# Tcadart/pyLatticeDSO

Measured on AMD Instinct MI355X. Metric: beams/s assembly+PCG-solve, higher is better.
Workload: dtype f64

## Files before the change

include/pylattice_hip.h:

```cpp
#ifndef PYLATTICE_HIP_H
#define PYLATTICE_HIP_H

#include <stdint.h>

#ifdef __cplusplus
extern "C" {
#endif

typedef struct pl_context *pl_handle;

typedef enum {
  PL_OK = 0,
  PL_ERR_ARG = -1,
  PL_ERR_HIP = -2,
  PL_ERR_STATE = -3,
  PL_ERR_NOCONV = -4,
  PL_ERR_NAN = -5,
  PL_ERR_NODEVICE = -6
} pl_status;

typedef struct {
  int64_t n_nodes;
  int64_t n_beams;
  const double *node_xyz;
// ... 60 lines not shown
  double cg_form_used;
  double kp_form;
  double comm_world;
  double comm_rank;
  double short_iteration_used;
  double reserved[2];
} pl_stats_t;

int pl_default_opts(pl_opts_t *o, uint32_t struct_size);
uint32_t pl_opts_size(void);
uint32_t pl_stats_size(void);
uint32_t pl_abi_version(void);
const char *pl_last_error(void);
const char *pl_version(void);

int pl_lzone(int device, int64_t n_nodes, int64_t n_beams, const double *node_xyz, const int32_t *beam_conn,
             const double *beam_radius, double *lzone);

int pl_create(const pl_mesh_t *mesh, const pl_opts_t *opts, pl_handle *out);
void pl_destroy(pl_handle h);

int pl_create_ddm(int64_t n_nodes, int64_t n_cells, int32_t nb, const int32_t *cell_nodes, int32_t n_S, const double *S,
                  const int32_t *cell_S, const pl_opts_t *opts, pl_handle *out);

#define PL_DDM_DENSE_MAX 16384
int pl_ddm_set_preconditioner(pl_handle h, int32_t n_S, const double *S ,
                              const int32_t *cell_S );

int pl_ddm_update_matrices(pl_handle h, int32_t n_S, const double *S , const int32_t *cell_S );

int pl_ddm_set_geometry(pl_handle h, const double *node_xyz );

int pl_set_bc(pl_handle h, const uint8_t *fixed, const double *ubar, const double *f);

int pl_set_periodic(pl_handle h, const int32_t *master );

int pl_update_radii(pl_handle h, const double *beam_radius);
int pl_set_multiplicity(pl_handle h, const double *beam_mult );
int pl_update_segments(pl_handle h, const double *seg_len, const int32_t *seg_nsub);

int pl_assemble(pl_handle h);

int pl_assemble_bsr(pl_handle h, int with_bc, int64_t *n_block_rows, int64_t *n_blocks);
int pl_get_bsr(pl_handle h, int64_t *rowptr , int32_t *colidx , double *vals );

int pl_spmv(pl_handle h, const double *x, double *y);
int pl_spmv_free(pl_handle h, const double *x, double *y);
int pl_spmv_bsr(pl_handle h, const double *x, double *y);

int pl_solve(pl_handle h, double rtol, int32_t max_iter, double *u, pl_stats_t *stats);

int pl_reactions(pl_handle h, const double *u, double *R);

int pl_sens(pl_handle h, const double *u, const double *lam, double *dCdr);

#define PL_SENS_GRAM_MAX 8
int pl_sens_gram(pl_handle h, int32_t n_rhs, const double *x, double *gram);

int pl_node_mod(pl_handle h, const double *u, double *out);

int pl_stress(pl_handle h, const double *u , int32_t where,
              double *station ,
              double *peak );
int pl_stress_pnorm(pl_handle h, const double *u , int32_t where, double p, double *phi, double *sigma_max,
                    double *dphi_du , double *dphi_dr );

int pl_buckling(pl_handle h, const double *u , int32_t length, double k_eff, int32_t shear,
                double *util , double *n_axial , double *n_crit );
int pl_buckling_pnorm(pl_handle h, const double *u , int32_t length, double k_eff, int32_t shear, double p,
                      double *bp, double *util_max, double *dbp_du , double *dbp_dr );

int pl_energy(pl_handle h, const double *u, double *energy);

int pl_schur(pl_handle h, const int32_t *boundary_nodes, int32_t nb, double rtol, int32_t max_iter, double *S);

#define PL_MULTI_MAX 64
int pl_spmv_multi(pl_handle h, int32_t n_rhs, int masked, const double *x, double *y);
int pl_solve_multi(pl_handle h, int32_t n_rhs, const double *ubar, const double *f, double rtol, int32_t max_iter,
                   double *u, pl_stats_t *stats);
int pl_schur_block(pl_handle h, const int32_t *boundary_nodes, int32_t nb, double rtol, int32_t max_iter,
                   int32_t block, double *S);

int pl_geom_spmv_multi(pl_handle h, const double *u, int32_t n_rhs, int masked, const double *x, double *y);
int pl_buckling_modes(pl_handle h, const double *u , int32_t n_modes, int32_t n_sub,
                      double rtol, int32_t max_iter,
                      double tol, int32_t max_outer,
                      double *load_factor , double *modes ,
                      double *residual ,
                      int32_t *n_found, int32_t *outer_iterations);
int pl_buckling_modes_sens(pl_handle h, const double *u , int32_t n_modes,
                           const double *load_factor , const double *modes ,
                           double rtol, int32_t max_iter,
                           const double *weights ,
                           double *dlam_dr  ,
                           double *dsum_dr  ,
                           double *adj_load );

int pl_set_mass(pl_handle h, double density, int32_t rotary, const double *node_mass );
int pl_mass_spmv_multi(pl_handle h, int32_t n_rhs, int masked, const double *x, double *y);
int pl_vibration_modes(pl_handle h, int32_t n_modes, int32_t n_sub, double rtol, int32_t max_iter, double tol,
                       int32_t max_outer, double *omega2 , double *modes ,
                       double *residual ,
                       int32_t *n_found, int32_t *outer_iterations);
int pl_vibration_modes_sens(pl_handle h, int32_t n_modes, const double *omega2 ,
                            const double *modes , const double *weights ,
                            double *domega2_dr ,
                            double *dsum_dr );

int pl_dyn_spmv_multi(pl_handle h, double c_K, double c_M, int32_t n_rhs, int masked, const double *x, double *y);
int pl_transient(pl_handle h, int32_t n_steps, double dt, double beta, double gamma, double ray_m, double ray_k,
                 int32_t n_pat, const double *pattern , const double *amp ,
                 const double *u0, const double *v0 , double rtol, int32_t max_iter,
                 int32_t n_probe, const int32_t *probe_nodes, double *probe ,
                 double *energy ,
                 int32_t snap_every, double *snaps ,
                 double *state , int32_t *iters );

#define PL_TRANSIENT_SENS_CHUNK 32
int pl_transient_sens(pl_handle h, int32_t n_steps, double dt, double beta, double gamma, double ray_m, double ray_k,
                      int32_t n_pat, const double *pattern , const double *amp ,
                      const double *base_dir , const double *base_acc ,
                      const double *u0, const double *v0 , double rtol, int32_t max_iter,
                      const double *out_vec , int32_t kind, double p, const double *weight ,
                      double *J, double *y , double *dJ_dr ,
                      int32_t *iters );

int pl_schur_cells(const pl_opts_t *o, int32_t n_inst, int32_t n_nodes, int32_t n_beams,
                   const int32_t *beam_conn , int32_t nb,
                   const int32_t *boundary_nodes ,
                   const double *node_xyz , const double *beam_radius ,
                   const double *seg_len , const int32_t *seg_nsub ,
                   double *S , int32_t *info );

int pl_cells_recover(const pl_opts_t *o, int32_t n_inst, int32_t n_nodes, int32_t n_beams,
                     const int32_t *beam_conn , int32_t nb,
                     const int32_t *boundary_nodes ,
                     const double *node_xyz , const double *beam_radius ,
                     const double *seg_len , const int32_t *seg_nsub ,
                     const double *u_b ,
                     const double *lam_b ,
                     double *u_full ,
                     double *lam_full ,
                     double *sens ,
                     int32_t *info );

int pl_get_records(pl_handle h, double *rec);

int pl_debug_partition(pl_handle h, int32_t *tile_of_node, int32_t *agg_of_node, int32_t *local_agg_of_node,
                       uint8_t *eliminated);

int pl_time_kernel(pl_handle h, int which, int reps, double *avg_ms);
int pl_algorithmic_bytes(pl_handle h, double *out3);
int pl_node_words_info(pl_handle h, int *classes_on, int *n_classes, int *bytes_on, int *byte_exp);
int pl_forget_history(pl_handle h);

int pl_debug_spd_solve(int device, int32_t n, const double *A, const double *b, double *x, double *quad,
                       int32_t fp32_factor);

int pl_dist_unique_id_bytes(void);
int pl_dist_unique_id(void *id_out);
int pl_dist_loopback_id(void *id_out);
int pl_dist_abort(pl_handle h);
int pl_dist_init(pl_handle h, int rank, int world, const void *unique_id, const int32_t *shared_local,
                 const int32_t *shared_global, int32_t n_shared, int32_t n_shared_global);

typedef struct pl_lattice pl_lattice;
typedef struct {
  int64_t n_nodes, n_beams, n_cell_beam, n_cell_node, n_created;
} pl_lattice_info_t;
int pl_generate_lattice(int64_t n_cells, const double *cell_coord, const double *cell_size, const double *cell_radii,
                        int32_t n_geom, int32_t n_tmpl, const double *tmpl, const int32_t *tmpl_type,
                        pl_lattice **out, pl_lattice_info_t *info);
int pl_lattice_fetch(const pl_lattice *L, double *node_xyz, int32_t *beam_conn, double *beam_radius, int32_t *beam_type,
                     int32_t *beam_cell0, int64_t *cell_beam_ptr , int64_t *cell_beam_idx,
                     int64_t *cell_node_ptr , int64_t *cell_node_idx, int32_t *created_nodes,
                     int32_t *created_beam);
void pl_lattice_free(pl_lattice *L);

int pl_penalize(int64_t n_beams, const double *node_xyz, const int32_t *beam_conn, const double *lzone ,
                double mesh_size, double *seg_len , int32_t *seg_nsub , double *pen_xyz );

int pl_boundary_index(int64_t n_cells, const int64_t *cell_node_ptr, const int64_t *cell_node_idx, int64_t n_nodes,
                      const double *node_xyz, const double *cell_coord, const double *cell_size, int64_t *index_boundary,
                      int64_t *visit, int64_t *n_visit);

int pl_boundary_index_rows(int64_t n_cells, const int64_t *cell_node_ptr, const int64_t *cell_node_idx, int64_t n_nodes,
                           const double *node_xyz, const double *cell_coord, const double *cell_size,
                           int64_t *index_boundary, int64_t *visit, int64_t *n_visit);

int pl_dist_set_peers(pl_handle h, const int32_t *shared_peer );

#ifdef __cplusplus
}
#endif
#endif
```

pylatticedso_amd/_capi.py:

```python
from __future__ import annotations

import ctypes as C
import os

import numpy as np

from .timing import timing as _timing

_HERE = os.path.dirname(os.path.abspath(__file__))
LIB_PATH = os.environ.get("PYLATTICE_HIP_LIB") or os.path.join(_HERE, "libpylattice_hip.so")

PL_OK, PL_ERR_ARG, PL_ERR_HIP, PL_ERR_STATE, PL_ERR_NOCONV, PL_ERR_NAN, PL_ERR_NODEVICE = 0, -1, -2, -3, -4, -5, -6

EXPORTS = ["pl_default_opts", "pl_opts_size", "pl_stats_size", "pl_abi_version", "pl_last_error", "pl_version", "pl_lzone", "pl_create", "pl_create_ddm",
           "pl_ddm_set_preconditioner", "pl_ddm_set_geometry", "pl_ddm_update_matrices", "pl_destroy", "pl_set_bc", "pl_set_periodic",
           "pl_update_radii", "pl_set_multiplicity", "pl_update_segments", "pl_assemble", "pl_assemble_bsr", "pl_get_bsr", "pl_spmv",
           "pl_spmv_free", "pl_spmv_bsr", "pl_solve", "pl_reactions", "pl_sens", "pl_sens_gram", "pl_energy", "pl_node_mod", "pl_schur",
           "pl_stress", "pl_stress_pnorm", "pl_buckling", "pl_buckling_pnorm",
           "pl_spmv_multi", "pl_solve_multi", "pl_schur_block", "pl_geom_spmv_multi", "pl_buckling_modes", "pl_buckling_modes_sens",
           "pl_set_mass", "pl_mass_spmv_multi", "pl_vibration_modes", "pl_vibration_modes_sens",
           "pl_dyn_spmv_multi", "pl_transient", "pl_transient_sens",
           "pl_schur_cells", "pl_cells_recover", "pl_get_records", "pl_debug_partition", "pl_time_kernel", "pl_algorithmic_bytes", "pl_node_words_info", "pl_forget_history", "pl_debug_spd_solve", "pl_dist_unique_id_bytes",
           "pl_dist_unique_id", "pl_dist_loopback_id", "pl_dist_abort", "pl_dist_init", "pl_dist_set_peers", "pl_generate_lattice", "pl_lattice_fetch",
           "pl_lattice_free", "pl_penalize", "pl_boundary_index", "pl_boundary_index_rows"]


class PlMesh(C.Structure):
    _fields_ = [("n_nodes", C.c_int64), ("n_beams", C.c_int64), ("node_xyz", C.c_void_p),
                ("beam_conn", C.c_void_p), ("beam_radius", C.c_void_p), ("seg_len", C.c_void_p),
                ("seg_nsub", C.c_void_p)]


class PlOpts(C.Structure):
    _fields_ = [("struct_size", C.c_uint32), ("abi_version", C.c_uint32),
                ("young", C.c_double), ("poisson", C.c_double), ("kappa", C.c_double), ("pen_coef", C.c_double),
                ("device", C.c_int32), ("spmv_kernel", C.c_int32), ("precond", C.c_int32), ("reorder", C.c_int32),
                ("check_every", C.c_int32), ("lanes_per_node", C.c_int32),
                ("tile_nodes", C.c_int32), ("coarse_max_dofs", C.c_int32), ("palette", C.c_int32),
                ("local_max_dofs", C.c_int32), ("precision", C.c_int32), ("restart_every", C.c_int32),
                ("alpha_max", C.c_double), ("grid_lo", C.c_double * 3), ("grid_hi", C.c_double * 3),
                ("grid_nodes", C.c_int64), ("mintol", C.c_double), ("compact_records", C.c_int32),
                ("condense", C.c_int32), ("chol_persistent", C.c_int32), ("cg_form", C.c_int32),
                ("tile_modes", C.c_int32), ("coarse_modes", C.c_int32), ("overlap", C.c_int32),
                ("coarse_storage", C.c_int32), ("warm_start", C.c_int32), ("short_iteration", C.c_int32)]


class PlStats(C.Structure):
    _fields_ = [("struct_size", C.c_uint32), ("iterations", C.c_int32), ("converged", C.c_int32),
                ("reserved_i", C.c_int32), ("rel_residual", C.c_double),
                ("b_norm", C.c_double), ("ms_assembly", C.c_double), ("ms_solve", C.c_double),
                ("ms_spmv_avg", C.c_double), ("precond_used", C.c_double), ("restarts", C.c_double),
                ("precision_used", C.c_double), ("info", C.c_double), ("stop_reason", C.c_double),
                ("condensed_nodes", C.c_double), ("cg_form_used", C.c_double), ("kp_form", C.c_double),
                ("comm_world", C.c_double), ("comm_rank", C.c_double), ("short_iteration_used", C.c_double),
                ("reserved", C.c_double * 2)]


class PlError(RuntimeError):
    def __init__(self, code, msg):
        super().__init__(f"libpylattice_hip error {code}: {msg}")
        self.code = code


_lib = None


def load_library(path: str | None = None):
    global _lib
    if _lib is not None and path is None:
        return _lib
    p = path or LIB_PATH
    if not os.path.exists(p):
        raise FileNotFoundError(f"{p} not found - build it with `make -C pylatticedso_amd/csrc` "
                                "(the HIP path has no CPU fallback)")
    lib = C.CDLL(p)
    lib.pl_last_error.restype = C.c_char_p
    lib.pl_version.restype = C.c_char_p
    lib.pl_destroy.restype = None
    for name in ("pl_opts_size", "pl_stats_size", "pl_abi_version"):
        getattr(lib, name).restype = C.c_uint32
    lib.pl_lattice_free.restype = None
    V, I32, I64, D = C.c_void_p, C.c_int32, C.c_int64, C.c_double
    sig = {"pl_default_opts": [V, C.c_uint32], "pl_opts_size": [], "pl_stats_size": [], "pl_abi_version": [], "pl_lzone": [I32, I64, I64, V, V, V, V], "pl_create": [V, V, V], "pl_create_ddm": [I64, I64, I32, V, I32, V, V, V, V],
           "pl_ddm_set_preconditioner": [V, I32, V, V], "pl_ddm_set_geometry": [V, V], "pl_ddm_update_matrices": [V, I32, V, V], "pl_destroy": [V], "pl_set_bc": [V, V, V, V], "pl_set_periodic": [V, V],
           "pl_update_radii": [V, V], "pl_set_multiplicity": [V, V], "pl_update_segments": [V, V, V], "pl_assemble": [V],
           "pl_assemble_bsr": [V, I32, V, V], "pl_get_bsr": [V, V, V, V], "pl_spmv": [V, V, V],
           "pl_spmv_free": [V, V, V], "pl_spmv_bsr": [V, V, V], "pl_solve": [V, D, I32, V, V],
           "pl_reactions": [V, V, V], "pl_sens": [V, V, V, V], "pl_sens_gram": [V, I32, V, V], "pl_energy": [V, V, V], "pl_node_mod": [V, V, V],
           "pl_stress": [V, V, I32, V, V], "pl_stress_pnorm": [V, V, I32, D, V, V, V, V],
           "pl_buckling": [V, V, I32, D, I32, V, V, V], "pl_buckling_pnorm": [V, V, I32, D, I32, D, V, V, V, V],
           "pl_schur": [V, V, I32, D, I32, V], "pl_spmv_multi": [V, I32, I32, V, V],
           "pl_solve_multi": [V, I32, V, V, D, I32, V, V], "pl_schur_block": [V, V, I32, D, I32, I32, V],
           "pl_geom_spmv_multi": [V, V, I32, I32, V, V],
           "pl_buckling_modes": [V, V, I32, I32, D, I32, D, I32, V, V, V, V, V],
           "pl_buckling_modes_sens": [V, V, I32, V, V, D, I32, V, V, V, V],
           "pl_set_mass": [V, D, I32, V], "pl_mass_spmv_multi": [V, I32, I32, V, V],
           "pl_vibration_modes": [V, I32, I32, D, I32, D, I32, V, V, V, V, V],
           "pl_vibration_modes_sens": [V, I32, V, V, V, V, V],
           "pl_dyn_spmv_multi": [V, D, D, I32, I32, V, V],
           "pl_transient": [V, I32, D, D, D, D, D, I32, V, V, V, V, D, I32, I32, V, V, V, I32, V, V, V],
           "pl_transient_sens": [V, I32, D, D, D, D, D, I32, V, V, V, V, V, V, D, I32, V, I32, D, V, V, V, V, V],
           "pl_schur_cells": [V, I32, I32, I32, V, I32, V, V, V, V, V, V, V],
           "pl_cells_recover": [V, I32, I32, I32, V, I32, V, V, V, V, V, V, V, V, V, V, V],
           "pl_get_records": [V, V], "pl_debug_partition": [V, V, V, V, V], "pl_time_kernel": [V, I32, I32, V],
           "pl_algorithmic_bytes": [V, V], "pl_node_words_info": [V, V, V, V, V], "pl_forget_history": [V], "pl_debug_spd_solve": [I32, I32, V, V, V, V, I32], "pl_dist_unique_id_bytes": [], "pl_dist_unique_id": [V], "pl_dist_loopback_id": [V], "pl_dist_abort": [V],
           "pl_dist_init": [V, I32, I32, V, V, V, I32, I32], "pl_dist_set_peers": [V, V],
           "pl_generate_lattice": [I64, V, V, V, I32, I32, V, V, V, V], "pl_lattice_fetch": [V] * 12,
           "pl_lattice_free": [V], "pl_penalize": [I64, V, V, V, D, V, V, V],
           "pl_boundary_index": [I64, V, V, I64, V, V, V, V, V, V],
           "pl_boundary_index_rows": [I64, V, V, I64, V, V, V, V, V, V]}
    for name, args in sig.items():
        getattr(lib, name).argtypes = args
    if lib.pl_opts_size() != C.sizeof(PlOpts) or lib.pl_stats_size() != C.sizeof(PlStats):
        raise ImportError(f"{p}: pl_opts_t / pl_stats_t are {lib.pl_opts_size()} / {lib.pl_stats_size()} bytes in the "
                          f"library, {C.sizeof(PlOpts)} / {C.sizeof(PlStats)} in this binding (ABI version "
                          f"{lib.pl_abi_version()}): rebuild libpylattice_hip.so")
    _lib = lib
    return lib


def default_opts(lib=None) -> "PlOpts":
    lib = lib or load_library()
    opts = PlOpts()
    _check(lib, lib.pl_default_opts(C.byref(opts), C.sizeof(PlOpts)))
    return opts


def _ptr(a):
    return None if a is None else a.ctypes.data_as(C.c_void_p)


def _f64(a, n=None):
    a = np.ascontiguousarray(a, dtype=np.float64)
    if n is not None and a.size != n:
        raise ValueError(f"expected {n} values, got {a.size}")
    return a


def _check(lib, rc, allow=()):
    if rc != PL_OK and rc not in allow:
        raise PlError(rc, lib.pl_last_error().decode())
    return rc


def lzone(node_xyz, beam_conn, beam_radius, device=0):
    lib = load_library()
    xyz = _f64(np.asarray(node_xyz).reshape(-1))
    conn = np.ascontiguousarray(beam_conn, dtype=np.int32).reshape(-1)
    rad = _f64(np.asarray(beam_radius).reshape(-1), len(conn) // 2)
    out = np.empty(len(conn), np.float64)
    _check(lib, lib.pl_lzone(int(device), len(xyz) // 3, len(conn) // 2, _ptr(xyz), _ptr(conn), _ptr(rad), _ptr(out)))
    return out.reshape(-1, 2)


def debug_spd_solve(A, b, device=0, fp32_factor=False):
    lib = load_library()
    A = np.ascontiguousarray(A, np.float64)
    b = np.ascontiguousarray(b, np.float64)
    x = np.empty_like(b)
    q = C.c_double()
    _check(lib, lib.pl_debug_spd_solve(device, len(b), _ptr(A), _ptr(b), _ptr(x), C.byref(q), int(bool(fp32_factor))))
    return x, q.value


MULTI_MAX = 64
SENS_GRAM_MAX = 8
TRANSIENT_SENS_CHUNK = 32

SCHUR_CELLS_MAX_BOUNDARY, SCHUR_CELLS_MAX_INTERIOR, SCHUR_CELLS_MAX_BEAMS = 32, 16, 512


def schur_cells_fits(n_nodes, n_beams, n_boundary):
    return (0 < n_boundary <= SCHUR_CELLS_MAX_BOUNDARY and n_nodes - n_boundary <= SCHUR_CELLS_MAX_INTERIOR
            and 0 < n_beams <= SCHUR_CELLS_MAX_BEAMS)


def _per_instance(name, a, tail, n_inst):
    if a.shape == tail:
        a = np.broadcast_to(a, (n_inst,) + tail)
    elif a.shape != (n_inst,) + tail:
        raise ValueError(f"{name} must have shape {tail} or {(n_inst,) + tail}, got {a.shape}")
    return np.ascontiguousarray(a)


def schur_cells(node_xyz, beam_conn, boundary_nodes, beam_radius, seg_len, seg_nsub, young, poisson, kappa=0.9,
                pen_coef=1.5, device=0, n_inst=None):
    xyz, conn, bn, rad, slen, nsub, n_inst = _cell_batch_arrays(node_xyz, beam_conn, boundary_nodes, beam_radius, seg_len,
                                                                seg_nsub, n_inst)
    B, N = len(conn), xyz.shape[1]
    lib = load_library()
    opts = default_opts(lib)
    opts.young, opts.poisson, opts.kappa, opts.pen_coef, opts.device = young, poisson, kappa, pen_coef, device
    m = 6 * len(bn)
    S = np.empty((n_inst, m, m), np.float64)
    info = np.empty(n_inst, np.int32)
    _check(lib, lib.pl_schur_cells(C.byref(opts), n_inst, N, B, _ptr(conn), len(bn), _ptr(bn), _ptr(xyz), _ptr(rad),
                                   _ptr(slen), _ptr(nsub), _ptr(S), _ptr(info)))
    return S, info


def _cell_batch_arrays(node_xyz, beam_conn, boundary_nodes, beam_radius, seg_len, seg_nsub, n_inst, extra_lead=()):
    conn = np.asarray(beam_conn)
    bn = np.asarray(boundary_nodes)
    if conn.ndim != 2 or conn.shape[1] != 2 or not np.issubdtype(conn.dtype, np.integer):
        raise ValueError("beam_conn must be an integer (B, 2) array")
    if bn.ndim != 1 or not np.issubdtype(bn.dtype, np.integer):
        raise ValueError("boundary_nodes must be a 1-D integer array")
    xyz, rad = np.asarray(node_xyz, dtype=np.float64), np.asarray(beam_radius, dtype=np.float64)
    slen, nsub = np.asarray(seg_len, dtype=np.float64), np.asarray(seg_nsub)
    if not np.issubdtype(nsub.dtype, np.integer):
        raise ValueError("seg_nsub must be an integer array")
    if xyz.ndim not in (2, 3) or xyz.shape[-1] != 3:
        raise ValueError("node_xyz must be (N, 3) or (n_inst, N, 3)")
    B, N = len(conn), xyz.shape[-2]
    lead = [a.shape[0] for a, nd in ((xyz, 3), (rad, 2), (slen, 3), (nsub, 3)) if a.ndim == nd] + list(extra_lead)
    if n_inst is None:
        n_inst = max(lead) if lead else 1
    n_inst = int(n_inst)
    if n_inst < 1:
        raise ValueError("n_inst must be >= 1")
    xyz = _per_instance("node_xyz", xyz, (N, 3), n_inst)
    rad = _per_instance("beam_radius", rad, (B,), n_inst)
    slen = _per_instance("seg_len", slen, (B, 3), n_inst)
    nsub = _per_instance("seg_nsub", nsub.astype(np.int32, copy=False), (B, 3), n_inst)
    conn = np.ascontiguousarray(conn, dtype=np.int32)
    bn = np.ascontiguousarray(bn, dtype=np.int32)
    return xyz, conn, bn, rad, slen, nsub, n_inst


def cells_recover(node_xyz, beam_conn, boundary_nodes, beam_radius, seg_len, seg_nsub, u_b, young, poisson, lam_b=None,
                  want=("u", "lam", "sens"), kappa=0.9, pen_coef=1.5, device=0):
    want = (want,) if isinstance(want, str) else tuple(want)
    if not want or any(w not in ("u", "lam", "sens") for w in want):
        raise ValueError('want must be a non-empty subset of ("u", "lam", "sens")')
    bn = np.asarray(boundary_nodes)
    m = 6 * (len(bn) if bn.ndim == 1 else 0)

    def boundary_values(name, v):
        v = np.asarray(v, dtype=np.float64)
        if v.ndim >= 2 and v.shape[-2:] == (m // 6, 6):
            v = v.reshape(v.shape[:-2] + (m,))
        if v.ndim not in (1, 2) or v.shape[-1] != m:
            raise ValueError(f"{name} must have {m} values per instance, got shape {v.shape}")
        return v

    ub = boundary_values("u_b", u_b)
    lb = None if lam_b is None else boundary_values("lam_b", lam_b)
    lead = [v.shape[0] for v in (ub, lb) if v is not None and v.ndim == 2]
    xyz, conn, bn, rad, slen, nsub, n_inst = _cell_batch_arrays(node_xyz, beam_conn, boundary_nodes, beam_radius, seg_len,
                                                                seg_nsub, None, lead)
    ub = _per_instance("u_b", ub, (m,), n_inst)
    lb = None if lb is None else _per_instance("lam_b", lb, (m,), n_inst)
    B, N = len(conn), xyz.shape[1]
    lib = load_library()
    opts = default_opts(lib)
    opts.young, opts.poisson, opts.kappa, opts.pen_coef, opts.device = young, poisson, kappa, pen_coef, device
    out = {"info": np.empty(n_inst, np.int32)}
    if "u" in want:
# ... 526 lines not shown
            out["dsum_dr"] = dsum
        return out

    def _mass_model(self):
        if getattr(self, "_mass", None) is None:
            raise ValueError("call set_mass first")
        return self._mass

    def mass_spmv_multi_host(self, X, masked=False, fixed=None):
        from . import mass_host as MH
        if masked and fixed is None:
            raise ValueError("the masked product needs the mask given to set_bc")
        rho, rotary, nm = self._mass_model()
        x = self._columns("X", X).reshape(-1, self.n_nodes, 6)
        return MH.mass_apply(self.node_xyz, self.beam_conn, self._radius, rho, x, self._mult, rotary, nm,
                             fixed if masked else None)

    def mass_matrix_host(self):
        from . import mass_host as MH
        rho, rotary, nm = self._mass_model()
        return MH.mass_matrix(self.node_xyz, self.beam_conn, self._radius, rho, self._mult, rotary, nm)

    def vibration_modes_host(self, fixed, n_modes=4, n_sub=0, tol=1e-9, max_outer=200, dense=False):
        from . import geometric_host as GH
        from . import mass_host as MH
        K = GH.elastic_matrix(self.records(), self.beam_conn, self.n_nodes)
        M = self.mass_matrix_host()
        if dense:
            return MH.vibration_modes_dense(K, M, fixed, n_modes)
        return MH.vibration_modes_subspace(K, M, fixed, n_modes, n_sub, tol, max_outer)

    def vibration_modes_sens_host(self, omega2, modes, fixed):
        from . import mass_host as MH
        from . import stress_host as SH
        rho, rotary, nm = self._mass_model()
        E, nu, kappa, pen = self._material
        drec = SH.drecords_dr(self.node_xyz, self.beam_conn, self._radius, self._seg_len, self._seg_nsub, E, nu, kappa, pen,
                              self._mult)
        return MH.vibration_sensitivity(self.node_xyz, self.beam_conn, self._radius, rho, drec, fixed, omega2, modes,
                                        self._mult, rotary, nm)

    def dyn_spmv_multi(self, c_K, c_M, X, masked=False):
        x = self._columns("X", X)
        y = np.empty_like(x)
        _check(self._lib, self._lib.pl_dyn_spmv_multi(self._h, float(c_K), float(c_M), x.shape[0], int(bool(masked)), _ptr(x),
                                                      _ptr(y)))
        return y.reshape(x.shape[0], self.n_nodes, 6)

    def transient(self, dt, n_steps, patterns=None, amp=None, u0=None, v0=None, beta=0.25, gamma=0.5, ray_m=0.0, ray_k=0.0,
                  rtol=1e-10, max_iter=100000, probes=None, snap_every=0, want_state=True):
        n_steps, n6 = int(n_steps), 6 * self.n_nodes
        rows = max(n_steps, 0) + 1
        pat = am = None
        n_pat = 0
        if patterns is not None:
            pat = np.ascontiguousarray(np.asarray(patterns, dtype=np.float64)).reshape(-1, n6)
            n_pat = pat.shape[0]
            am = np.ascontiguousarray(np.asarray(amp, dtype=np.float64).reshape(-1))
            if am.size != rows * n_pat:
                raise ValueError(f"amp must have shape ({rows}, {n_pat})")
        uu = self._opt_vec6(u0)
        vv = self._opt_vec6(v0)
        pr = np.zeros(0, np.int32) if probes is None else np.ascontiguousarray(np.asarray(probes).reshape(-1), dtype=np.int32)
        probe = np.zeros((rows, 3, pr.size, 6), np.float64)
        energy = np.zeros((rows, 3), np.float64)
        iters = np.zeros(rows, np.int32)
        snap_every = int(snap_every)
        snaps = np.zeros((n_steps // snap_every, self.n_nodes, 6), np.float64) if snap_every > 0 and n_steps > 0 else None
        state = np.zeros((3, self.n_nodes, 6), np.float64) if want_state else None
        _check(self._lib, self._lib.pl_transient(self._h, n_steps, float(dt), float(beta), float(gamma), float(ray_m),
                                                 float(ray_k), n_pat, _ptr(pat), _ptr(am), _ptr(uu), _ptr(vv), float(rtol),
                                                 int(max_iter), pr.size, _ptr(pr) if pr.size else None,
                                                 _ptr(probe) if pr.size else None, _ptr(energy), snap_every, _ptr(snaps),
                                                 _ptr(state), _ptr(iters)))
        out = {"time": float(dt) * np.arange(rows), "probe": probe, "energy": energy, "iters": iters}
        if want_state:
            out["state"] = state
        if snaps is not None:
            out["snaps"] = snaps
        return out

    def transient_host(self, fixed, dt, n_steps, patterns=None, amp=None, u0=None, v0=None, beta=0.25, gamma=0.5, ray_m=0.0,
                       ray_k=0.0, solve=None, probes=None, snap_every=0):
        import scipy.sparse as sp
        from . import dynamics_host as DH
        self.assemble_bsr(False)
        rowptr, col, vals = self.get_bsr()
        K = sp.bsr_matrix((vals, col, rowptr), shape=(6 * self.n_nodes, 6 * self.n_nodes)).tocsr()
        K.sum_duplicates()
        return DH.newmark(K, self.mass_matrix_host(), fixed, dt, n_steps, patterns, amp, u0, v0, beta, gamma, ray_m, ray_k,
                          solve, probes, snap_every)

    def transient_sens(self, dt, n_steps, out_vec, kind=2, p=8.0, weight=None, patterns=None, amp=None, base_dir=None,
                       base_acc=None, u0=None, v0=None, beta=0.25, gamma=0.5, ray_m=0.0, ray_k=0.0, rtol=1e-10,
                       max_iter=100000):
        n_steps, n6 = int(n_steps), 6 * self.n_nodes
        rows = max(n_steps, 0) + 1
        pat = am = None
        n_pat = 0
        if patterns is not None:
            pat = np.ascontiguousarray(np.asarray(patterns, dtype=np.float64)).reshape(-1, n6)
            n_pat = pat.shape[0]
            am = np.ascontiguousarray(np.asarray(amp, dtype=np.float64).reshape(-1))
            if am.size != rows * n_pat:
                raise ValueError(f"amp must have shape ({rows}, {n_pat})")
        bd = None if base_dir is None else _f64(np.asarray(base_dir).reshape(-1), 3)
        ba = None if base_acc is None else _f64(np.asarray(base_acc).reshape(-1), rows)
        uu = self._opt_vec6(u0)
        vv = self._opt_vec6(v0)
        lv = _f64(np.asarray(out_vec).reshape(-1), n6)
        wt = None if weight is None else _f64(np.asarray(weight).reshape(-1), rows)
        J = C.c_double()
        y = np.zeros(rows, np.float64)
        grad = np.zeros(self.n_beams, np.float64)
        iters = np.zeros((2, rows), np.int32)
        _check(self._lib, self._lib.pl_transient_sens(self._h, n_steps, float(dt), float(beta), float(gamma), float(ray_m),
                                                      float(ray_k), n_pat, _ptr(pat), _ptr(am), _ptr(bd), _ptr(ba), _ptr(uu),
                                                      _ptr(vv), float(rtol), int(max_iter), _ptr(lv), int(kind), float(p),
                                                      _ptr(wt), C.byref(J), _ptr(y), _ptr(grad), _ptr(iters)))
        return {"J": J.value, "y": y, "dJ_dr": grad, "iters": iters}

    def transient_sens_host(self, fixed, dt, n_steps, out_vec, kind=2, p=8.0, weight=None, patterns=None, amp=None,
                            base_dir=None, base_acc=None, u0=None, v0=None, beta=0.25, gamma=0.5, ray_m=0.0, ray_k=0.0,
                            solve=None):
        import scipy.sparse as sp
        from . import dynamics_host as DH
        from . import mass_host as MH
        from . import stress_host as SH
        self.assemble_bsr(False)
        rowptr, col, vals = self.get_bsr()
        K = sp.bsr_matrix((vals, col, rowptr), shape=(6 * self.n_nodes, 6 * self.n_nodes)).tocsr()
        K.sum_duplicates()
        rho, rotary, nm = self._mass_model()
        E, nu, kappa, pen = self._material
        drec = SH.drecords_dr(self.node_xyz, self.beam_conn, self._radius, self._seg_len, self._seg_nsub, E, nu, kappa, pen,
                              self._mult)
        conn = np.asarray(self.beam_conn).reshape(-1, 2)
        xyz = np.asarray(self.node_xyz, dtype=np.float64).reshape(-1, 3)
        dM = MH.delement_matrix_dr(xyz[conn[:, 1]] - xyz[conn[:, 0]], np.asarray(self._radius, dtype=np.float64).reshape(-1),
                                   rho, self._mult, rotary)
        return DH.newmark_sensitivity(K, self.mass_matrix_host(), fixed, conn, drec, dM, dt, n_steps, out_vec, kind, p, weight,
                                      patterns, amp, base_dir, base_acc, u0, v0, beta, gamma, ray_m, ray_k, solve)

    def time_kernel(self, which, reps=20):
        ms = C.c_double()
        _check(self._lib, self._lib.pl_time_kernel(self._h, int(which), int(reps), C.byref(ms)))
        return ms.value

    def node_words_info(self):
        v = [C.c_int() for _ in range(4)]
        _check(self._lib, self._lib.pl_node_words_info(self._h, *[C.byref(x) for x in v]))
        return {"classes": bool(v[0].value), "n_classes": v[1].value, "bytes": bool(v[2].value), "byte_exp": v[3].value}

    def algorithmic_bytes(self):
        out = (C.c_double * 3)()
        _check(self._lib, self._lib.pl_algorithmic_bytes(self._h, out))
        return {"spmv": out[0], "pcg_iter": out[1], "bsr": out[2]}

    def set_periodic(self, master):
        m = None if master is None else np.ascontiguousarray(master, dtype=np.int32)
        if m is not None and m.size != self.n_nodes:
            raise ValueError(f"expected {self.n_nodes} entries, got {m.size}")
        _check(self._lib, self._lib.pl_set_periodic(self._h, _ptr(m)))

    def forget_history(self):
        _check(self._lib, self._lib.pl_forget_history(self._h))

    @staticmethod
    def dist_unique_id() -> bytes:
        lib = load_library()
        n = lib.pl_dist_unique_id_bytes()
        buf = C.create_string_buffer(n)
        _check(lib, lib.pl_dist_unique_id(buf))
        return buf.raw

    @staticmethod
    def dist_loopback_id() -> bytes:
        lib = load_library()
        buf = C.create_string_buffer(lib.pl_dist_unique_id_bytes())
        _check(lib, lib.pl_dist_loopback_id(buf))
        return buf.raw

    def dist_abort(self):
        if getattr(self, "_h", None) is not None and self._h.value:
            self._lib.pl_dist_abort(self._h)

    def dist_init(self, rank, world, unique_id: bytes, shared_local, shared_global, n_shared_global, shared_peer=None):
        sl = np.ascontiguousarray(shared_local, dtype=np.int32)
        sg = np.ascontiguousarray(shared_global, dtype=np.int32)
        buf = C.create_string_buffer(unique_id, len(unique_id))
        _check(self._lib, self._lib.pl_dist_init(self._h, int(rank), int(world), buf, _ptr(sl), _ptr(sg),
                                                 int(len(sl)), int(n_shared_global)))
        if shared_peer is not None:
            sp = np.ascontiguousarray(shared_peer, dtype=np.int32)
            if sp.shape != sl.shape:
                raise ValueError("one peer rank per shared entry expected")
            _check(self._lib, self._lib.pl_dist_set_peers(self._h, _ptr(sp)))


for _name in ("assemble", "assemble_bsr", "get_bsr", "solve", "set_bc", "spmv", "spmv_free", "spmv_bsr", "reactions",
              "sens", "stress", "stress_pnorm", "buckling", "buckling_pnorm", "energy", "schur", "spmv_multi", "solve_multi", "geom_spmv_multi", "buckling_modes", "buckling_modes_sens", "mass_spmv_multi", "vibration_modes", "vibration_modes_sens", "dyn_spmv_multi", "transient", "update_radii", "update_segments", "records"):
    _f = getattr(HipLattice, _name, None)
    if _f is not None:
        _f._timing_category = "hip"
        setattr(HipLattice, _name, _timing.timeit(_f))
```

pylatticedso_amd/csrc/pl_api.hip:

```cpp
#include <functional>

#include "pl_solver.h"
#include "pl_condense.h"
#include "pl_multi.h"
#include "pl_stress.h"
#include "pl_buckling.h"
#include "pl_geom.h"
#include "pl_mass.h"
#include "pl_dyn.h"
#include "pl_dyn_sens.h"
#include "pl_sensgram.h"


namespace {
template <typename WT>
int debug_spd_solve_t(int device, int32_t n, const double *A, const double *b, double *x, double *quad) {
  if (n <= 0 || !A || !b || !x) return fail(PL_ERR_ARG, "pl_debug_spd_solve: bad argument");
  int ndev = 0;
  if (hipGetDeviceCount(&ndev) != hipSuccess || ndev <= 0) return fail(PL_ERR_NODEVICE, "no HIP device visible");
  PL_HIP(hipSetDevice(device));
  const int np = (n + pl::kNB - 1) / pl::kNB * pl::kNB;
  std::vector<double> Ap((size_t)np * np, 0.0), bp(np, 0.0);
  for (int i = 0; i < np; ++i) {
    if (i < n) {
// ... 24 lines not shown
  PL_HIP(hipMemset(dinfo.p, 0, 2 * sizeof(int)));
  pl::dense_factor_inverse(dA.p, dL.p, dW.p, dWt.p, dD.p, np, np, dinfo.p, 0, nullptr);
  pl::dense_apply(dW.p, dWt.p, np, np, db.p, dt.p, dy.p, dq.p, nullptr, nullptr);
  PL_HIP(hipGetLastError());
  PL_HIP(hipDeviceSynchronize());
  int info[2];
  PL_HIP(hipMemcpy(info, dinfo.p, sizeof(info), hipMemcpyDeviceToHost));
  if (info[0] != 0) return fail(PL_ERR_ARG, "pl_debug_spd_solve: matrix is not positive definite");
  std::vector<double> y(np), q(pl::kSlots);
  PL_HIP(hipMemcpy(y.data(), dy.p, np * sizeof(double), hipMemcpyDeviceToHost));
  PL_HIP(hipMemcpy(q.data(), dq.p, pl::kSlots * sizeof(double), hipMemcpyDeviceToHost));
  std::memcpy(x, y.data(), n * sizeof(double));
  if (quad) {
    *quad = 0.0;
    for (double v : q) *quad += v;
  }
  return PL_OK;
}

}

extern "C" {

const char *pl_last_error(void) { return g_err.c_str(); }
#ifndef PL_KP_HASH
#define PL_KP_HASH "unknown"
#endif
const char *pl_version(void) { return "pylattice_hip 0.2 (gfx950) kp=" PL_KP_HASH; }

uint32_t pl_opts_size(void) { return (uint32_t)sizeof(pl_opts_t); }
uint32_t pl_stats_size(void) { return (uint32_t)sizeof(pl_stats_t); }
uint32_t pl_abi_version(void) { return PL_ABI_VERSION; }

int pl_default_opts(pl_opts_t *o, uint32_t struct_size) {
  if (!o) return fail(PL_ERR_ARG, "pl_default_opts: null argument");
  if (struct_size != sizeof(pl_opts_t))
    return fail(PL_ERR_ARG, "pl_default_opts: the caller's pl_opts_t has " + std::to_string(struct_size) +
                                " bytes, this library's " + std::to_string(sizeof(pl_opts_t)) +
                                " (ABI version " + std::to_string(PL_ABI_VERSION) + "): rebuild the binding against include/pylattice_hip.h");
  std::memset(o, 0, sizeof(*o));
  o->struct_size = (uint32_t)sizeof(pl_opts_t);
  o->abi_version = PL_ABI_VERSION;
  o->young = 1013.0;
  o->poisson = 0.3;
  o->kappa = 0.9;
  o->pen_coef = 1.5;
  o->device = 0;
  o->spmv_kernel = 0;
  o->precond = 1;
  o->reorder = 1;
  o->check_every = 0;
  return PL_OK;
}

namespace {
int check_opts_abi(const pl_opts_t *o, const char *who) {
  if (o->struct_size != sizeof(pl_opts_t) || o->abi_version != PL_ABI_VERSION)
    return fail(PL_ERR_ARG, std::string(who) + ": pl_opts_t was not initialised by pl_default_opts of this library (struct_size " +
                                std::to_string(o->struct_size) + " / abi " + std::to_string(o->abi_version) + ", expected " +
                                std::to_string(sizeof(pl_opts_t)) + " / " + std::to_string(PL_ABI_VERSION) + ")");
  return PL_OK;
}
inline bool multi_rank_handle(const pl_opts_t *o) { return o->grid_nodes > 0; }
inline int coarse_modes_of(const pl_opts_t *o, int64_t N = -1) {
  const bool tile12 = o->precond == 3 && o->tile_modes != 6;
  if (!tile12 || o->coarse_modes == 6) return 6;
  if (multi_rank_handle(o)) N = o->grid_nodes;
  return (o->coarse_modes == 12 || N < 0 || N >= 250000) ? 12 : 6;
}
inline int coarse_budget(const pl_opts_t *o, int64_t N) {
  const bool multi_rank = o->grid_nodes > 0;
  if (o->coarse_max_dofs > 0) return o->coarse_max_dofs;
  if (multi_rank) return (coarse_modes_of(o, N) == 12 && o->grid_nodes >= 2000000) ? 6144 : 3072;
  if (coarse_modes_of(o, N) == 12) return N >= 2000000 ? 6144 : (N >= 1000000 ? 3072 : (N >= 250000 ? 1536 : 768));
  return N >= 1000000 ? 3072 : 2100;
}
}

int pl_create(const pl_mesh_t *m, const pl_opts_t *o, pl_handle *out) {
  if (!m || !o || !out) return fail(PL_ERR_ARG, "pl_create: null argument");
  if (int rc_abi = check_opts_abi(o, "pl_create")) return rc_abi;
  StageTimer stage("pl_create");
  if (m->n_nodes <= 0 || m->n_beams <= 0) return fail(PL_ERR_ARG, "pl_create: empty mesh");
  if (m->n_nodes >= (1LL << 31) - 64 || m->n_beams >= (1LL << 31) - 64)
    return fail(PL_ERR_ARG, "pl_create: more than 2^31 nodes/struts per handle");
  if (!m->node_xyz || !m->beam_conn || !m->beam_radius || !m->seg_len || !m->seg_nsub)
    return fail(PL_ERR_ARG, "pl_create: null mesh array");
  int ndev = 0;
  if (hipGetDeviceCount(&ndev) != hipSuccess || ndev <= 0)
    return fail(PL_ERR_NODEVICE, "pl_create: no HIP device visible (libpylattice_hip has no CPU fallback)");
  if (o->device < 0 || o->device >= ndev) return fail(PL_ERR_ARG, "pl_create: bad device ordinal");
  if (o->precond == 5 && 6 * m->n_nodes > PL_DDM_DENSE_MAX)
    return fail(PL_ERR_ARG, "pl_create: precond = 5 (dense factorisation) serves at most PL_DDM_DENSE_MAX dofs");
  const int64_t N = m->n_nodes, B = m->n_beams;
  {
    std::atomic<int64_t> bad_ends{-1}, bad_radius{-1}, bad_len{-1}, bad_seg{-1};
    pl::parallel_for(B, [&](int64_t b0, int64_t b1, unsigned) {
      for (int64_t b = b0; b < b1; ++b) {
        const int32_t a = m->beam_conn[2 * b], d = m->beam_conn[2 * b + 1];
        if (a < 0 || d < 0 || a >= N || d >= N || a == d) bad_ends = b;
        if (!(m->beam_radius[b] > 0.0)) bad_radius = b;
        const double L = m->seg_len[3 * b] + m->seg_len[3 * b + 1] + m->seg_len[3 * b + 2];
        if (!(L > 0.0)) bad_len = b;
        for (int k = 0; k < 3; ++k)
          if (m->seg_len[3 * b + k] < 0.0 || (m->seg_len[3 * b + k] > 0.0 && m->seg_nsub[3 * b + k] < 1)) bad_seg = b;
      }
    });
    if (bad_ends >= 0)
      return fail(PL_ERR_ARG, "pl_create: strut " + std::to_string(bad_ends.load()) + " has invalid end nodes");
    if (bad_radius >= 0) return fail(PL_ERR_ARG, "pl_create: non-positive radius");
    if (bad_len >= 0) return fail(PL_ERR_ARG, "pl_create: strut with zero length");
    if (bad_seg >= 0) return fail(PL_ERR_ARG, "pl_create: bad segment data on strut " + std::to_string(bad_seg.load()));
  }
  stage.mark("validate");
  PL_HIP(hipSetDevice(o->device));
  pl_context *c = new pl_context();
  c->opt = *o;
  c->N = N;
  c->B = B;
  c->mat = {o->young, o->young / (2.0 * (1.0 + o->poisson)), o->kappa, o->pen_coef};
  c->lpn = o->lanes_per_node > 0 ? o->lanes_per_node : pl::kDefaultLPN;
  if (c->lpn != 1 && c->lpn != 2 && c->lpn != 4 && c->lpn != 8 && c->lpn != 16) {
    delete c;
    return fail(PL_ERR_ARG, "pl_create: lanes_per_node must be 0 (default), 1, 2, 4, 8 or 16");
  }
  auto bail = [&](int rc) {
    delete c;
    return rc;
  };
#define PL_TRY(expr)              \
  do {                            \
    int _rc = (expr);             \
    if (_rc) return bail(_rc);    \
  } while (0)
#define PL_HIPC(expr)                                                                  \
  do {                                                                                 \
    hipError_t _e = (expr);                                                            \
    if (_e != hipSuccess)                                                              \
      return bail(fail(PL_ERR_HIP, std::string(#expr) + ": " + hipGetErrorString(_e))); \
  } while (0)
  {
    int prio_low = 0, prio_high = 0;
    PL_HIPC(hipDeviceGetStreamPriorityRange(&prio_low, &prio_high));
    PL_HIPC(hipStreamCreateWithPriority(&c->stream, hipStreamNonBlocking, prio_high));
    PL_HIPC(hipStreamCreateWithPriority(&c->side, hipStreamNonBlocking, prio_low));
  }
  PL_HIPC(hipEventCreate(&c->ev0));
  PL_HIPC(hipEventCreate(&c->ev1));
  PL_HIPC(hipEventCreateWithFlags(&c->ev_fork, hipEventDisableTiming));
  PL_HIPC(hipEventCreateWithFlags(&c->ev_join, hipEventDisableTiming));
  PL_HIPC(hipEventCreateWithFlags(&c->ev_chol, hipEventDisableTiming));
  PL_HIPC(hipEventCreateWithFlags(&c->ev_t0, hipEventDisableTiming));
  PL_HIPC(hipEventCreateWithFlags(&c->ev_t1, hipEventDisableTiming));
  PL_HIPC(hipEventCreateWithFlags(&c->ev_p0, hipEventDisableTiming));
  PL_HIPC(hipEventCreateWithFlags(&c->ev_p1, hipEventDisableTiming));
  PL_HIPC(hipEventCreateWithFlags(&c->ev_fill1, hipEventDisableTiming));
  PL_HIPC(hipStreamCreateWithFlags(&c->side2, hipStreamNonBlocking));
  {
    const char *e = std::getenv("PL_BSR_CUMASK");
    const int k = e ? std::atoi(e) : 4;
    hipDeviceProp_t prop;
    const bool tuned_layout = hipGetDeviceProperties(&prop, o->device) == hipSuccess && prop.multiProcessorCount == 256;
    if (k > 0 && k < 8 && tuned_layout) {
      uint32_t mask[8];
      for (int w = 0; w < 8; ++w) {
        mask[w] = 0u;
        for (int b = 0; b < 32; ++b) {
          const int i = 32 * w + b;
          if ((i / 8 + i) % 8 >= k) mask[w] |= 1u << b;
        }
      }
      if (hipExtStreamCreateWithCUMask(&c->side_cu, 8, mask) != hipSuccess) {
        (void)hipGetLastError();
        c->side_cu = nullptr;
      }
    }
  }

  const double global_grid[7] = {o->grid_lo[0], o->grid_lo[1], o->grid_lo[2], o->grid_hi[0], o->grid_hi[1],
                                 o->grid_hi[2], (double)o->grid_nodes};
  c->perm.resize(N);
  std::iota(c->perm.begin(), c->perm.end(), 0);
  std::vector<int32_t> tile_start, tile_of;
  std::vector<int64_t> tile_brick;
  pl::BrickGrid grid;
  if (o->reorder == 1) {
    pl::spatial_order(m->node_xyz, N, c->perm, tile_start,
                      (double)(o->tile_nodes > 0 ? std::min(o->tile_nodes, pl::kTileMaxNodes) : 256), tile_brick,
                      grid, o->grid_nodes > 0 ? global_grid : nullptr,
                      (o->precond >= 2 && o->precond <= 4) ? coarse_budget(o, N) * 6 / coarse_modes_of(o, N) : 0);
    c->reordered = true;
    {
      std::vector<uint64_t> kind((size_t)N, 0);
      pl::parallel_for(B, [&](int64_t b0, int64_t b1, unsigned) {
        for (int64_t b = b0; b < b1; ++b) {
          const int32_t u = m->beam_conn[2 * b], v = m->beam_conn[2 * b + 1];
          uint64_t d = 0;
          for (int k = 0; k < 3; ++k) {
            const int64_t q = (int64_t)std::llround((m->node_xyz[3 * (size_t)v + k] - m->node_xyz[3 * (size_t)u + k]) * 4096.0);
            d = d * 0x9E3779B97F4A7C15ull + (uint64_t)(q + (1 << 20));
          }
          auto mix = [](uint64_t h) { h ^= h >> 33; h *= 0xFF51AFD7ED558CCDull; h ^= h >> 33; return h; };
          __atomic_fetch_add(&kind[u], mix(d), __ATOMIC_RELAXED);
          __atomic_fetch_add(&kind[v], mix(~d), __ATOMIC_RELAXED);
        }
      }, 1 << 16);
      const int64_t T = (int64_t)tile_start.size() - 1;
      pl::parallel_for(T, [&](int64_t t0, int64_t t1, unsigned) {
        for (int64_t t = t0; t < t1; ++t)
          std::stable_sort(c->perm.begin() + tile_start[t], c->perm.begin() + tile_start[t + 1],
                           [&](int32_t l, int32_t r) { return kind[l] < kind[r]; });
      }, 16);
    }
  } else {
    pl::chunk_tiles(N, tile_start);
  }
  stage.mark("spatial order");
  c->iperm.resize(N);
  pl::parallel_for(N, [&](int64_t i0, int64_t i1, unsigned) {
    for (int64_t i = i0; i < i1; ++i) c->iperm[c->perm[i]] = (int32_t)i;
  }, 1 << 16);
  if (o->condense >= 0 && o->precond >= 2 && o->precond <= 4 && o->precision != 2 && o->reorder == 1) {
    std::vector<int64_t> aptr((size_t)N + 1, 0);
    pl::parallel_for(2 * B, [&](int64_t k0, int64_t k1, unsigned) {
      for (int64_t k = k0; k < k1; ++k)
        __atomic_fetch_add(&aptr[c->iperm[m->beam_conn[k]] + 1], (int64_t)1, __ATOMIC_RELAXED);
    }, 1 << 16);
    for (int64_t i = 0; i < N; ++i) aptr[i + 1] += aptr[i];
    std::vector<int32_t> adj((size_t)2 * B);
    {
      std::vector<int64_t> fill(aptr.begin(), aptr.end() - 1);
      pl::parallel_for(B, [&](int64_t b0, int64_t b1, unsigned) {
        for (int64_t b = b0; b < b1; ++b) {
          const int32_t u = c->iperm[m->beam_conn[2 * b]], v = c->iperm[m->beam_conn[2 * b + 1]];
          adj[__atomic_fetch_add(&fill[u], (int64_t)1, __ATOMIC_RELAXED)] = v;
          adj[__atomic_fetch_add(&fill[v], (int64_t)1, __ATOMIC_RELAXED)] = u;
        }
      }, 1 << 16);
    }
    double lo[3] = {1e300, 1e300, 1e300}, hi[3] = {-1e300, -1e300, -1e300};
    for (int64_t i = 0; i < N; ++i)
      for (int k = 0; k < 3; ++k) {
        lo[k] = std::min(lo[k], m->node_xyz[3 * i + k]);
        hi[k] = std::max(hi[k], m->node_xyz[3 * i + k]);
      }
    std::vector<uint8_t> state((size_t)N, 0);
    for (int pass = 0; pass < 2; ++pass)
      for (int64_t i = 0; i < N; ++i) {
        if (state[i] || aptr[i + 1] - aptr[i] < 3) continue;
        const double *q3 = m->node_xyz + 3 * (size_t)c->perm[i];
        const bool on_box = q3[0] <= lo[0] || q3[0] >= hi[0] || q3[1] <= lo[1] || q3[1] >= hi[1] || q3[2] <= lo[2] ||
                            q3[2] >= hi[2];
        if (on_box != (pass == 1)) continue;
        state[i] = 1;
        for (int64_t q = aptr[i]; q < aptr[i + 1]; ++q)
          if (!state[adj[q]]) state[adj[q]] = 2;
      }
    int64_t n_cand = 0;
    for (int64_t i = 0; i < N; ++i) n_cand += state[i] == 1;
    const bool use = o->condense > 0 || (double)n_cand >= 0.45 * (double)N;
    const int64_t T = use ? (int64_t)tile_start.size() - 1 : 0;
    std::vector<int32_t> np(c->perm.size());
    if (use) c->h_cand.assign((size_t)N, 0);
    for (int64_t t = 0; t < T; ++t) {
      int64_t w = tile_start[t];
      for (int pass = 0; pass < 2; ++pass)
        for (int64_t i = tile_start[t]; i < tile_start[t + 1]; ++i)
          if ((state[i] == 1) == (pass == 1)) {
            c->h_cand[w] = (uint8_t)pass;
            np[w++] = c->perm[i];
          }
    }
    if (use) {
      c->perm.swap(np);
      for (int64_t i = 0; i < N; ++i) c->iperm[c->perm[i]] = (int32_t)i;
    }
  }

  stage.mark("candidates");
  std::vector<double> xyz((size_t)N * 3);
  pl::parallel_for(N, [&](int64_t i0, int64_t i1, unsigned) {
    for (int64_t i = i0; i < i1; ++i)
      std::memcpy(&xyz[3 * i], m->node_xyz + 3 * (size_t)c->perm[i], 3 * sizeof(double));
  });
  std::vector<int32_t> conn((size_t)B * 2);
  {
    std::vector<int32_t> conn0((size_t)B * 2);
    pl::parallel_for(2 * B, [&](int64_t k0, int64_t k1, unsigned) {
      for (int64_t k = k0; k < k1; ++k) conn0[k] = c->iperm[m->beam_conn[k]];
    });
    pl::tile_strut_order(conn0, N, B, tile_start, tile_of, c->bperm, xyz.data());
    pl::parallel_for(B, [&](int64_t b0, int64_t b1, unsigned) {
      for (int64_t b = b0; b < b1; ++b) {
        conn[2 * b] = conn0[2 * (size_t)c->bperm[b]];
        conn[2 * b + 1] = conn0[2 * (size_t)c->bperm[b] + 1];
      }
    });
  }
  stage.mark("strut order");
  std::vector<double> radius(B), seg_len((size_t)B * 3);
  std::vector<int32_t> seg_nsub((size_t)B * 3);
  pl::parallel_for(B, [&](int64_t b0, int64_t b1, unsigned) {
    for (int64_t b = b0; b < b1; ++b) {
      const size_t ob = (size_t)c->bperm[b];
      radius[b] = m->beam_radius[ob];
      for (int k = 0; k < 3; ++k) {
// ... 64 lines not shown
  PL_HIPC(c->f.alloc(n6));
  const size_t vpad = o->precond == 5 ? (size_t)pl::kNB : 0;
  for (DevBuf<double> *v : {&c->diag, &c->dinv, &c->x, &c->r, &c->z, &c->p, &c->Ap, &c->tmp, &c->tmp2}) {
    PL_HIPC(v->alloc(n6 + vpad));
    if (vpad) PL_HIPC(hipMemset(v->p, 0, (n6 + vpad) * sizeof(double)));
  }
  PL_HIPC(c->scal.alloc(2 * pl::S_COUNT * pl::kSlots));
  PL_HIPC(hipMemset(c->fixed.p, 0, n6));
  PL_HIPC(hipMemset(c->fixedbits.p, 0, N));
  PL_HIPC(hipMemset(c->ubar.p, 0, n6 * sizeof(double)));
  PL_HIPC(hipMemset(c->f.p, 0, n6 * sizeof(double)));
  PL_HIPC(hipDeviceSynchronize());
#undef PL_TRY
#undef PL_HIPC
  stage.mark("vector buffers");
  *out = c;
  return PL_OK;
}

static int ddm_build_classes(pl_context *c) {
  const int64_t n_cells = c->ddm_cells;
  const int nb = c->ddm_nb, m = 6 * nb;
  const int32_t *cell_S = c->h_ddm_cell_S.data(), *cell_nodes = c->h_ddm_cell_nodes.data();
  std::vector<int32_t> order((size_t)n_cells);
  std::iota(order.begin(), order.end(), 0);
  std::stable_sort(order.begin(), order.end(), [&](int32_t l, int32_t r) { return cell_S[l] < cell_S[r]; });
  PL_HIP(c->ddm_order.alloc(order.size()));
  PL_HIP(hipMemcpy(c->ddm_order.p, order.data(), order.size() * sizeof(int32_t), hipMemcpyHostToDevice));
  std::vector<int32_t> tiles, tile_S;
  for (size_t q = 0; q < order.size();) {
    const int32_t id = cell_S[order[q]];
    size_t e = q;
    while (e < order.size() && cell_S[order[e]] == id) ++e;
    for (size_t a = q; a < e; a += 16) {
      for (size_t k = 0; k < 16; ++k) tiles.push_back(a + k < e ? order[a + k] : -1);
      tile_S.push_back(id);
    }
    q = e;
  }
  c->ddm_n_tiles = (int64_t)tile_S.size();
  if (m <= 192) {
    const int KS = pl::ddm_mfma_ks(m);
    std::vector<int32_t> gidx((size_t)c->ddm_n_tiles * KS * 64, -1);
    for (int64_t t = 0; t < c->ddm_n_tiles; ++t)
      for (int kk = 0; kk < KS; ++kk)
        for (int lane = 0; lane < 64; ++lane) {
          const int32_t cell = tiles[16 * t + (lane & 15)];
          const int k = 4 * kk + (lane >> 4);
          if (cell >= 0 && k < m)
            gidx[((size_t)t * KS + kk) * 64 + lane] = 6 * cell_nodes[(int64_t)cell * nb + k / 6] + k % 6;
        }
    PL_HIP(c->ddm_tile_gidx.alloc(std::max<size_t>(1, gidx.size())));
    if (!gidx.empty())
      PL_HIP(hipMemcpy(c->ddm_tile_gidx.p, gidx.data(), gidx.size() * sizeof(int32_t), hipMemcpyHostToDevice));
  }
  PL_HIP(c->ddm_tiles.alloc(std::max<size_t>(1, tiles.size())));
  PL_HIP(c->ddm_tile_S.alloc(std::max<size_t>(1, tile_S.size())));
  if (!tiles.empty()) {
    PL_HIP(hipMemcpy(c->ddm_tiles.p, tiles.data(), tiles.size() * sizeof(int32_t), hipMemcpyHostToDevice));
    PL_HIP(hipMemcpy(c->ddm_tile_S.p, tile_S.data(), tile_S.size() * sizeof(int32_t), hipMemcpyHostToDevice));
  }
  return PL_OK;
}

int pl_ddm_update_matrices(pl_handle h, int32_t n_S, const double *S, const int32_t *cell_S) {
  if (!valid(h) || !S || !cell_S || n_S <= 0) return fail(PL_ERR_ARG, "pl_ddm_update_matrices: bad argument");
  if (h->opkind != 1) return fail(PL_ERR_STATE, "pl_ddm_update_matrices: not a DDM handle");
  for (int64_t c = 0; c < h->ddm_cells; ++c)
    if (cell_S[c] < 0 || cell_S[c] >= n_S) return fail(PL_ERR_ARG, "pl_ddm_update_matrices: matrix id out of range");
  PL_HIP(hipSetDevice(h->opt.device));
  PL_HIP(hipStreamSynchronize(h->stream));
  const int m = 6 * h->ddm_nb;
  const size_t cnt = (size_t)n_S * m * m;
  if (h->ddm_St.n != cnt) PL_HIP(h->ddm_St.alloc(cnt));
  if (h->ddm_Sraw.n < cnt) PL_HIP(h->ddm_Sraw.alloc(cnt));
  PL_HIP(hipMemcpyAsync(h->ddm_Sraw.p, S, cnt * sizeof(double), hipMemcpyHostToDevice, h->stream));
  hipLaunchKernelGGL(pl::k_ddm_transpose_palette, dim3(grid_for((int64_t)cnt)), dim3(pl::kBlock), 0, h->stream, (int64_t)n_S, m,
                     (const double *)h->ddm_Sraw.p, h->ddm_St.p);
  PL_HIP(hipStreamSynchronize(h->stream));
  PL_HIP(hipGetLastError());
  h->ddm_n_S = n_S;
  if (!std::equal(h->h_ddm_cell_S.begin(), h->h_ddm_cell_S.end(), cell_S)) {
    h->h_ddm_cell_S.assign(cell_S, cell_S + h->ddm_cells);
    PL_HIP(hipMemcpy(h->ddm_cell_S.p, cell_S, h->ddm_cells * sizeof(int32_t), hipMemcpyHostToDevice));
    int rc = ddm_build_classes(h);
    if (rc) return rc;
  }
  h->assembled = false;
  h->dd_ready = false;
  h->dd_blocks = false;
  h->dd2_ready = false;
  return PL_OK;
}

int pl_create_ddm(int64_t n_nodes, int64_t n_cells, int32_t nb, const int32_t *cell_nodes, int32_t n_S,
                  const double *S, const int32_t *cell_S, const pl_opts_t *o, pl_handle *out) {
  if (!cell_nodes || !S || !cell_S || !o || !out) return fail(PL_ERR_ARG, "pl_create_ddm: null argument");
  if (int rc_abi = check_opts_abi(o, "pl_create_ddm")) return rc_abi;
  if (n_nodes <= 0 || n_cells <= 0 || nb <= 0 || n_S <= 0) return fail(PL_ERR_ARG, "pl_create_ddm: empty problem");
  if (6 * nb > pl::kDdmMaxM) return fail(PL_ERR_ARG, "pl_create_ddm: more than 27 boundary nodes per cell");
  int ndev = 0;
  if (hipGetDeviceCount(&ndev) != hipSuccess || ndev <= 0)
    return fail(PL_ERR_NODEVICE, "pl_create_ddm: no HIP device visible (libpylattice_hip has no CPU fallback)");
  if (o->device < 0 || o->device >= ndev) return fail(PL_ERR_ARG, "pl_create_ddm: bad device ordinal");
  for (int64_t k = 0; k < n_cells * nb; ++k)
    if (cell_nodes[k] < 0 || cell_nodes[k] >= n_nodes) return fail(PL_ERR_ARG, "pl_create_ddm: node id out of range");
  for (int64_t c = 0; c < n_cells; ++c)
    if (cell_S[c] < 0 || cell_S[c] >= n_S) return fail(PL_ERR_ARG, "pl_create_ddm: matrix id out of range");
  PL_HIP(hipSetDevice(o->device));
  pl_context *c = new pl_context();
  c->opt = *o;
  c->opt.precond = (o->precond >= 1 && o->precond <= 4) ? o->precond : 0;
  if (c->opt.precond == 2 && 6 * n_nodes > PL_DDM_DENSE_MAX) {
    delete c;
    return fail(PL_ERR_ARG, "pl_create_ddm: precond = 2 factorises a dense (6 n_nodes)^2 matrix; limit is " +
                                std::to_string(PL_DDM_DENSE_MAX) + " dofs (use precond = 3 or 1)");
  }
  c->opkind = 1;
  c->N = n_nodes;
  c->B = 0;
  c->ddm_cells = n_cells;
  c->ddm_nb = nb;
  {
    int64_t span = 0;
    for (int64_t cc = 0; cc < n_cells; ++cc) {
      const int32_t *nd = cell_nodes + cc * nb;
      span = std::max<int64_t>(span, *std::max_element(nd, nd + nb) - *std::min_element(nd, nd + nb));
    }
    c->dd_bw = (int)((6 * span + 5) / pl::kNB + 1);
  }
  auto bail = [&](int rc) {
    delete c;
    return rc;
  };
#define PL_HIPC(expr)                                                                  \
  do {                                                                                 \
    hipError_t _e = (expr);                                                            \
    if (_e != hipSuccess)                                                              \
      return bail(fail(PL_ERR_HIP, std::string(#expr) + ": " + hipGetErrorString(_e))); \
  } while (0)
  {
    int prio_low = 0, prio_high = 0;
    PL_HIPC(hipDeviceGetStreamPriorityRange(&prio_low, &prio_high));
    PL_HIPC(hipStreamCreateWithPriority(&c->stream, hipStreamNonBlocking, prio_high));
    PL_HIPC(hipStreamCreateWithPriority(&c->side, hipStreamNonBlocking, prio_low));
  }
  PL_HIPC(hipEventCreate(&c->ev0));
  PL_HIPC(hipEventCreate(&c->ev1));
  PL_HIPC(hipEventCreateWithFlags(&c->ev_fork, hipEventDisableTiming));
  PL_HIPC(hipEventCreateWithFlags(&c->ev_join, hipEventDisableTiming));
  PL_HIPC(hipEventCreateWithFlags(&c->ev_chol, hipEventDisableTiming));
  PL_HIPC(hipEventCreateWithFlags(&c->ev_t0, hipEventDisableTiming));
  PL_HIPC(hipEventCreateWithFlags(&c->ev_t1, hipEventDisableTiming));
  PL_HIPC(hipStreamCreateWithFlags(&c->side2, hipStreamNonBlocking));
  c->perm.resize(n_nodes);
  std::iota(c->perm.begin(), c->perm.end(), 0);
  c->iperm = c->perm;
  const int m = 6 * nb;
  std::vector<double> St((size_t)n_S * m * m);
  for (int s = 0; s < n_S; ++s)
    for (int i = 0; i < m; ++i)
      for (int j = 0; j < m; ++j) St[((size_t)s * m + j) * m + i] = S[((size_t)s * m + i) * m + j];
  PL_HIPC(c->ddm_cell_nodes.alloc((size_t)n_cells * nb));
  PL_HIPC(c->ddm_cell_S.alloc(n_cells));
  PL_HIPC(c->ddm_St.alloc(St.size()));
  PL_HIPC(hipMemcpy(c->ddm_cell_nodes.p, cell_nodes, (size_t)n_cells * nb * sizeof(int32_t), hipMemcpyHostToDevice));
  PL_HIPC(hipMemcpy(c->ddm_cell_S.p, cell_S, n_cells * sizeof(int32_t), hipMemcpyHostToDevice));
  PL_HIPC(hipMemcpy(c->ddm_St.p, St.data(), St.size() * sizeof(double), hipMemcpyHostToDevice));
  {
    if (n_cells * nb >= (1LL << 31)) return bail(fail(PL_ERR_ARG, "pl_create_ddm: more than 2^31 cell-node entries"));
    std::vector<int64_t> nptr((size_t)n_nodes + 1, 0);
    for (int64_t k = 0; k < n_cells * nb; ++k) nptr[cell_nodes[k] + 1]++;
    for (int64_t i = 0; i < n_nodes; ++i) nptr[i + 1] += nptr[i];
    std::vector<int32_t> nent((size_t)n_cells * nb);
    std::vector<int64_t> fill(nptr.begin(), nptr.end() - 1);
    for (int64_t k = 0; k < n_cells * nb; ++k) nent[fill[cell_nodes[k]]++] = (int32_t)k;
    PL_HIPC(c->ddm_node_ptr.alloc(nptr.size()));
    PL_HIPC(c->ddm_node_ent.alloc(nent.size()));
    PL_HIPC(c->ddm_stage.alloc((size_t)n_cells * m));
    PL_HIPC(hipMemcpy(c->ddm_node_ptr.p, nptr.data(), nptr.size() * sizeof(int64_t), hipMemcpyHostToDevice));
    PL_HIPC(hipMemcpy(c->ddm_node_ent.p, nent.data(), nent.size() * sizeof(int32_t), hipMemcpyHostToDevice));
    c->h_ddm_cell_nodes.assign(cell_nodes, cell_nodes + n_cells * nb);
    c->h_ddm_cell_S.assign(cell_S, cell_S + n_cells);
    c->ddm_n_S = n_S;
    {
      int rcc = ddm_build_classes(c);
      if (rcc) return bail(rcc);
    }
  }
  const size_t n6 = (size_t)n_nodes * 6;
  PL_HIPC(c->fixed.alloc(n6));
  PL_HIPC(c->fixedbits.alloc(n_nodes));
  PL_HIPC(c->ubar.alloc(n6));
  PL_HIPC(c->f.alloc(n6));
  for (DevBuf<double> *v : {&c->diag, &c->dinv, &c->x, &c->r, &c->z, &c->p, &c->Ap, &c->tmp, &c->tmp2}) {
    PL_HIPC(v->alloc(n6 + pl::kNB));
    PL_HIPC(hipMemset(v->p, 0, (n6 + pl::kNB) * sizeof(double)));
  }
  PL_HIPC(c->scal.alloc(2 * pl::S_COUNT * pl::kSlots));
  PL_HIPC(hipMemset(c->fixed.p, 0, n6));
  PL_HIPC(hipMemset(c->fixedbits.p, 0, n_nodes));
  PL_HIPC(hipMemset(c->ubar.p, 0, n6 * sizeof(double)));
  PL_HIPC(hipMemset(c->f.p, 0, n6 * sizeof(double)));
  PL_HIPC(hipDeviceSynchronize());
#undef PL_HIPC
  *out = c;
  return PL_OK;
}

int pl_ddm_set_geometry(pl_handle h, const double *node_xyz) {
  if (!valid(h) || !node_xyz) return fail(PL_ERR_ARG, "pl_ddm_set_geometry: null argument");
  if (h->opkind != 1) return fail(PL_ERR_STATE, "pl_ddm_set_geometry: not a DDM handle");
  PL_HIP(hipSetDevice(h->opt.device));
  const int64_t N = h->N;
  h->dd2_plan = false;
  h->dd2_ready = false;
  h->assembled = false;
  double lo[3], hi[3];
  for (int k = 0; k < 3; ++k) lo[k] = hi[k] = node_xyz[k];
  for (int64_t i = 0; i < N; ++i)
    for (int k = 0; k < 3; ++k) {
      const double v = node_xyz[3 * i + k];
      if (!std::isfinite(v)) return fail(PL_ERR_ARG, "pl_ddm_set_geometry: non-finite coordinate");
      lo[k] = std::min(lo[k], v);
      hi[k] = std::max(hi[k], v);
    }
  const int budget = h->opt.coarse_max_dofs > 0 ? h->opt.coarse_max_dofs : 1536;
  const int64_t n_target = std::max<int64_t>(1, std::min<int64_t>(budget / pl::kDdmModes, N / 27));
  double ext[3];
  for (int k = 0; k < 3; ++k) ext[k] = hi[k] - lo[k];
  const double emax = std::max(ext[0], std::max(ext[1], ext[2]));
  int64_t na[3] = {1, 1, 1};
  if (emax > 0.0) {
    double side = emax;
    for (int it = 0; it < 200; ++it) {
      int64_t t[3];
      for (int k = 0; k < 3; ++k) t[k] = std::max<int64_t>(1, (int64_t)std::floor(ext[k] / (side * 0.96) + 0.5));
      if (t[0] * t[1] * t[2] > n_target) break;
      for (int k = 0; k < 3; ++k) na[k] = t[k];
      side *= 0.96;
    }
  }
  const int n_agg = (int)(na[0] * na[1] * na[2]);
  int ax[3] = {0, 1, 2};
  std::stable_sort(ax, ax + 3, [&](int l, int r) { return na[l] > na[r]; });
  std::vector<int32_t> agg((size_t)N), ptr((size_t)n_agg + 1, 0), nodes((size_t)N);
  for (int64_t i = 0; i < N; ++i) {
    int64_t b[3];
    for (int k = 0; k < 3; ++k) {
      b[k] = ext[k] > 0.0 ? (int64_t)std::floor((node_xyz[3 * i + k] - lo[k]) / ext[k] * (double)na[k]) : 0;
      b[k] = std::min<int64_t>(std::max<int64_t>(b[k], 0), na[k] - 1);
    }
    agg[(size_t)i] = (int32_t)((b[ax[0]] * na[ax[1]] + b[ax[1]]) * na[ax[2]] + b[ax[2]]);
    ptr[(size_t)agg[(size_t)i] + 1]++;
  }
  for (int a = 0; a < n_agg; ++a) ptr[(size_t)a + 1] += ptr[(size_t)a];
  {
    std::vector<int32_t> fill(ptr.begin(), ptr.end() - 1);
    for (int64_t i = 0; i < N; ++i) nodes[(size_t)fill[(size_t)agg[(size_t)i]]++] = (int32_t)i;
  }
  std::vector<double> cen((size_t)n_agg * 3);
  for (int a = 0; a < n_agg; ++a) {
    int64_t b[3];
    b[ax[0]] = a / (na[ax[1]] * na[ax[2]]);
    b[ax[1]] = (a / na[ax[2]]) % na[ax[1]];
    b[ax[2]] = a % na[ax[2]];
    for (int k = 0; k < 3; ++k) cen[3 * (size_t)a + k] = lo[k] + ((double)b[k] + 0.5) * ext[k] / (double)na[k];
  }
  std::vector<int32_t> cn((size_t)h->ddm_cells * h->ddm_nb);
  PL_HIP(hipMemcpy(cn.data(), h->ddm_cell_nodes.p, cn.size() * sizeof(int32_t), hipMemcpyDeviceToHost));
  int64_t max_diff = 0;
  for (int64_t c = 0; c < h->ddm_cells; ++c) {
    int32_t amin = n_agg, amax = -1;
    for (int i = 0; i < h->ddm_nb; ++i) {
      const int32_t a = agg[(size_t)cn[(size_t)c * h->ddm_nb + i]];
      amin = std::min(amin, a);
      amax = std::max(amax, a);
    }
    max_diff = std::max<int64_t>(max_diff, amax - amin);
  }
  pl::Coarse &cs = h->dd2;
  const int nc = pl::kDdmModes * n_agg, ncp = (nc + pl::kNB - 1) / pl::kNB * pl::kNB;
  if (cs.ncp != ncp) {
    for (void **q : {(void **)&cs.Ac, (void **)&cs.Lf, (void **)&cs.W, (void **)&cs.Wt, (void **)&cs.Dinv, (void **)&cs.rc,
                     (void **)&cs.yc, (void **)&cs.tv, (void **)&cs.info, (void **)&cs.bar, (void **)&cs.Ainv})
      if (*q) {
        (void)hipFree(*q);
        *q = nullptr;
      }
    const size_t n2 = (size_t)ncp * ncp;
    PL_HIP(hipMalloc((void **)&cs.Ac, n2 * sizeof(double)));
    PL_HIP(hipMalloc((void **)&cs.Lf, n2 * sizeof(double)));
    PL_HIP(hipMalloc((void **)&cs.W, n2 * sizeof(float)));
    PL_HIP(hipMalloc((void **)&cs.Wt, n2 * sizeof(float)));
    PL_HIP(hipMalloc((void **)&cs.Dinv, (size_t)ncp * pl::kNB * sizeof(double)));
    PL_HIP(hipMalloc((void **)&cs.rc, (size_t)(ncp + 2 * pl::kSlots) * sizeof(double)));
    PL_HIP(hipMalloc((void **)&cs.yc, (size_t)ncp * sizeof(double)));
    PL_HIP(hipMalloc((void **)&cs.tv, (size_t)ncp * sizeof(double)));
    PL_HIP(hipMalloc((void **)&cs.info, 2 * sizeof(int)));
    PL_HIP(hipMalloc((void **)&cs.bar, sizeof(unsigned)));
    if (ncp <= pl::kOneGemvMaxDofs) PL_HIP(hipMalloc((void **)&cs.Ainv, n2 * sizeof(float)));
    PL_HIP(hipMemset(cs.Lf, 0, n2 * sizeof(double)));
    PL_HIP(hipMemset(cs.W, 0, n2 * sizeof(float)));
    PL_HIP(hipMemset(cs.Wt, 0, n2 * sizeof(float)));
    PL_HIP(hipMemset(cs.rc, 0, (size_t)(ncp + 2 * pl::kSlots) * sizeof(double)));
    PL_HIP(hipMemset(cs.yc, 0, (size_t)ncp * sizeof(double)));
// ... 2142 lines not shown
  if (!valid(h)) return fail(PL_ERR_ARG, "pl_debug_partition: null handle");
  PL_HIP(hipSetDevice(h->opt.device));
  const int64_t N = h->N;
  std::vector<int32_t> tmp((size_t)N);
  auto fetch = [&](const int32_t *dev, int32_t *out) -> int {
    if (!out) return PL_OK;
    if (!dev) {
      std::fill(out, out + N, -1);
      return PL_OK;
    }
    PL_HIP(hipMemcpy(tmp.data(), dev, (size_t)N * sizeof(int32_t), hipMemcpyDeviceToHost));
    for (int64_t i = 0; i < N; ++i) out[h->perm[i]] = tmp[(size_t)i];
    return PL_OK;
  };
  if (tile_of_node) {
    std::fill(tile_of_node, tile_of_node + N, -1);
    if (h->opkind == 0)
      for (size_t t = 0; t + 1 < h->h_tile_start.size(); ++t)
        for (int32_t i = h->h_tile_start[t]; i < h->h_tile_start[t + 1]; ++i) tile_of_node[h->perm[i]] = (int32_t)t;
  }
  int rc = fetch(h->opkind == 1 ? (h->dd2_plan ? (const int32_t *)h->dd2_agg.p : (const int32_t *)nullptr)
                                : (h->coarse.enabled ? (const int32_t *)h->coarse.agg_of_node.p : (const int32_t *)nullptr),
                 agg_of_node);
  if (rc) return rc;
  rc = fetch(h->coarseL.enabled ? (const int32_t *)h->coarseL.agg_of_node.p : (const int32_t *)nullptr, local_agg_of_node);
  if (rc) return rc;
  if (eliminated) {
    std::fill(eliminated, eliminated + N, (uint8_t)0);
    if (h->n_cond > 0 && h->cond_ready && h->cflag.p) {
      std::vector<uint8_t> flag((size_t)N);
      PL_HIP(hipMemcpy(flag.data(), h->cflag.p, (size_t)N, hipMemcpyDeviceToHost));
      for (int64_t i = 0; i < N; ++i) eliminated[h->perm[i]] = flag[(size_t)i];
    }
  }
  return PL_OK;
}

int pl_algorithmic_bytes(pl_handle h, double *out3) {
  if (!valid(h) || !out3) return fail(PL_ERR_ARG, "pl_algorithmic_bytes: null argument");
  const double w = 8.0, B = (double)h->B, N = (double)h->N;
  const bool mp = h->assembled && mp_applies(h);
  const double wv = mp ? 4.0 : 8.0;
  const double wx = (mp && h->opt.precision == 1) ? 4.0 : 8.0;
  out3[0] = B * (8.0 + 8.0 * w) + N * 6.0 * wv * 2.0;
  out3[1] = out3[0] + 10.0 * (6.0 * N * wx);
  out3[2] = B * (8.0 + 8.0 * w) + (N + 2.0 * B) * (36.0 * w + 4.0);
  return PL_OK;
}

int pl_forget_history(pl_handle h) {
  if (!valid(h)) return fail(PL_ERR_ARG, "pl_forget_history: null handle");
  h->last_iterations = 0;
  h->xprev_valid = false;
  h->xprev2_valid = false;
  h->xprev3_valid = false;
  h->gh_count = 0;
  return PL_OK;
}

int pl_time_kernel(pl_handle h, int which, int reps, double *avg_ms) {
  if (!valid(h) || !avg_ms || reps <= 0) return fail(PL_ERR_ARG, "pl_time_kernel: bad argument");
  if (h->opkind != 0 && which != 0 && which != 3 && which != 10 && which != 11) return fail(PL_ERR_STATE, "pl_time_kernel: DDM handles time K*p / PCG only");
  if (!h->assembled) return fail(PL_ERR_STATE, "pl_time_kernel: call pl_assemble first");
  if ((which == 0 || which == 3 || which == 10 || which == 11) && !h->have_bc) return fail(PL_ERR_STATE, "pl_time_kernel: call pl_set_bc first");
  if ((which == 2 || which == 4) && !h->have_bsr) return fail(PL_ERR_STATE, "pl_time_kernel: needs pl_assemble_bsr");
  PL_HIP(hipSetDevice(h->opt.device));
  const int64_t n6 = h->N * 6;
  int rc = ensure_hist(h, reps + 1);
  if (rc) return rc;
  solver_plan(h);
  h->stop_use = false;
  if (h->small_use && (which == 3 || which == 11)) {
    rc = small_prepare(h);
    if (rc) return rc;
  }
  PL_HIP(hipMemcpyAsync(h->p.p, h->dinv.p, n6 * sizeof(double), hipMemcpyDeviceToDevice, h->stream));
  if (which >= 7 && which <= 11) {
    hipLaunchKernelGGL(pl::k_to_float, dim3(grid_for(n6)), dim3(pl::kBlock), 0, h->stream, n6, h->dinv.p,
                       reinterpret_cast<float *>(h->z.p));
    PL_HIP(hipMemsetAsync(h->tmp.p, 0, n6 * sizeof(double), h->stream));
  }
  float *p32 = reinterpret_cast<float *>(h->z.p), *Ap32 = p32 + n6;
  float *x32 = reinterpret_cast<float *>(h->tmp.p), *r32 = x32 + n6;
  auto one = [&](int k) -> int {
    switch (which) {
      case 0: return launch_spmv(h, h->p.p, h->Ap.p, true, h->scal.p + pl::S_PAP * pl::kSlots);
      case 1: {
        int r1 = launch_records(h);
        return r1 ? r1 : build_palette(h);
      }
      case 2: return launch_bsr_fill(h, 0, h->stream);
      case 3: return pcg_iteration(h, k);
      case 4:
        hipLaunchKernelGGL(pl::k_bsr_spmv, dim3(grid_for(h->N)), dim3(pl::kBlock), 0, h->stream, h->N,
                           h->bsr_rowptr.p, h->bsr_col.p, h->bsr_vals.p, h->p.p, h->Ap.p);
        return PL_OK;
      case 5:
        if (!h->dist.active) return fail(PL_ERR_STATE, "pl_time_kernel: 5/6 need pl_dist_init");
        return pl::dist_sum_shared(h->dist, h->Ap.p, h->stream, h->scal.p + pl::S_PAP * pl::kSlots, pl::kSlots)
                   ? fail(PL_ERR_HIP, "RCCL all-reduce failed") : PL_OK;
      case 6:
        if (!h->dist.active || !h->coarse.ready) return fail(PL_ERR_STATE, "pl_time_kernel: 6 needs a coarse level");
        return pl::dist_sum_scalars(h->dist, h->coarse.tv, h->coarse.ncp, h->stream)
                   ? fail(PL_ERR_HIP, "RCCL all-reduce failed") : PL_OK;
      case 7:
      case 8:
      case 9:
        if (!(h->coarse.ready && h->tile.ready && choose_kernel(h) == 3))
          return fail(PL_ERR_STATE, "pl_time_kernel: 7/8/9 need the multi-level PCG on the tile kernel");
        if (which == 7) return launch_spmv_f32(h, p32, Ap32, true, h->scal.p + pl::S_PAP * pl::kSlots);
        return which == 8 ? mp_iteration<float>(h, k, k, p32, Ap32, x32, r32)
                          : mp_iteration<double>(h, k, k, p32, Ap32, h->x.p, h->r.p);
      case 10:
        return mp_applies(h) ? apply_operator<float>(h, p32, Ap32, h->scal.p + pl::S_PAP * pl::kSlots)
                             : apply_operator<double>(h, h->p.p, h->Ap.p, h->scal.p + pl::S_PAP * pl::kSlots);
      case 11:
        return mp_applies(h) && h->opt.precision == 1 ? mp_iteration<float>(h, k, k, p32, Ap32, x32, r32) : pcg_iteration(h, k);
      case 12:
        if (h->gram_cols < 1) return fail(PL_ERR_STATE, "pl_time_kernel: 12 needs a pl_sens_gram call on this handle first");
        return launch_sens_gram(h, h->gram_cols, h->gram_x.p, h->gram_out.p);
      default: return fail(PL_ERR_ARG, "pl_time_kernel: unknown kernel id");
    }
  };
  for (int k = 0; k < 3; ++k) {
    rc = one(0);
    if (rc) return rc;
  }
  PL_HIP(hipEventRecord(h->ev0, h->stream));
  for (int k = 0; k < reps; ++k) {
    rc = one(k);
    if (rc) return rc;
  }
  PL_HIP(hipEventRecord(h->ev1, h->stream));
  PL_HIP(hipStreamSynchronize(h->stream));
  float ms = 0.f;
  PL_HIP(hipEventElapsedTime(&ms, h->ev0, h->ev1));
  *avg_ms = (double)ms / reps;
  return PL_OK;
}

int pl_node_words_info(pl_handle h, int *classes_on, int *n_classes, int *bytes_on, int *byte_exp) {
  if (!valid(h)) return fail(PL_ERR_ARG, "pl_node_words_info: null handle");
  const pl::Coarse &cs = h->coarse;
  const bool words = node_words_apply(h);
  const bool cls = words && h->assembled && cs.dcl_ready;
  const bool bytes = words && cs.rel_e >= 0;
  if (classes_on) *classes_on = cls ? 1 : 0;
  if (n_classes) *n_classes = h->assembled ? cs.dcl_classes : 0;
  if (bytes_on) *bytes_on = bytes ? 1 : 0;
  if (byte_exp) *byte_exp = bytes ? cs.rel_e : -1;
  return PL_OK;
}

int pl_debug_spd_solve(int device, int32_t n, const double *A, const double *b, double *x, double *quad,
                       int32_t fp32_factor) {
  return fp32_factor ? debug_spd_solve_t<float>(device, n, A, b, x, quad)
                     : debug_spd_solve_t<double>(device, n, A, b, x, quad);
}

int pl_lzone(int device, int64_t n_nodes, int64_t n_beams, const double *node_xyz, const int32_t *beam_conn,
             const double *beam_radius, double *lzone) {
  if (n_nodes <= 0 || n_beams <= 0 || !node_xyz || !beam_conn || !beam_radius || !lzone)
    return fail(PL_ERR_ARG, "pl_lzone: bad argument");
  int ndev = 0;
  if (hipGetDeviceCount(&ndev) != hipSuccess || ndev <= 0)
    return fail(PL_ERR_NODEVICE, "pl_lzone: no HIP device visible (libpylattice_hip has no CPU fallback)");
  if (device < 0 || device >= ndev) return fail(PL_ERR_ARG, "pl_lzone: bad device ordinal");
  const int64_t nh = 2 * n_beams;
  std::vector<int64_t> ptr((size_t)n_nodes + 1, 0);
  for (int64_t h = 0; h < nh; ++h) {
    const int32_t v = beam_conn[h];
    if (v < 0 || v >= n_nodes) return fail(PL_ERR_ARG, "pl_lzone: node id out of range");
    ptr[(size_t)v + 1]++;
  }
  for (int64_t i = 0; i < n_nodes; ++i) ptr[i + 1] += ptr[i];
  std::vector<int32_t> half((size_t)nh);
  {
    std::vector<int64_t> fill(ptr.begin(), ptr.end() - 1);
    for (int64_t h = 0; h < nh; ++h) half[(size_t)fill[beam_conn[h]]++] = (int32_t)h;
  }
  PL_HIP(hipSetDevice(device));
  DevBuf<double> dx, dr, dl;
  DevBuf<int32_t> dc, dh;
  DevBuf<int64_t> dp;
  PL_HIP(dx.alloc((size_t)n_nodes * 3));
  PL_HIP(dr.alloc(n_beams));
  PL_HIP(dl.alloc(nh));
  PL_HIP(dc.alloc(nh));
  PL_HIP(dh.alloc(nh));
  PL_HIP(dp.alloc(n_nodes + 1));
  PL_HIP(hipMemcpy(dx.p, node_xyz, (size_t)n_nodes * 3 * sizeof(double), hipMemcpyHostToDevice));
  PL_HIP(hipMemcpy(dr.p, beam_radius, n_beams * sizeof(double), hipMemcpyHostToDevice));
  PL_HIP(hipMemcpy(dc.p, beam_conn, nh * sizeof(int32_t), hipMemcpyHostToDevice));
  PL_HIP(hipMemcpy(dh.p, half.data(), nh * sizeof(int32_t), hipMemcpyHostToDevice));
  PL_HIP(hipMemcpy(dp.p, ptr.data(), (n_nodes + 1) * sizeof(int64_t), hipMemcpyHostToDevice));
  hipLaunchKernelGGL(pl::k_lzone, dim3(grid_for(nh)), dim3(pl::kBlock), 0, nullptr, nh, dx.p, dc.p, dr.p, dp.p, dh.p,
                     dl.p);
  PL_HIP(hipGetLastError());
  PL_HIP(hipMemcpy(lzone, dl.p, nh * sizeof(double), hipMemcpyDeviceToHost));
  return PL_OK;
}

#ifdef PL_TILE_STAMPS
int pl_debug_tile_stamps(unsigned long long *out) {
  return hipMemcpyFromSymbol(out, HIP_SYMBOL(pl::g_tile_stamps), sizeof(unsigned long long) * 8 * 4096) == hipSuccess ? 0 : -2;
}
#endif

int pl_dist_unique_id_bytes(void) { return pl::dist_unique_id_bytes(); }
int pl_dist_unique_id(void *id_out) {
  if (!id_out) return fail(PL_ERR_ARG, "pl_dist_unique_id: null argument");
  return pl::dist_unique_id(id_out) ? fail(PL_ERR_HIP, "ncclGetUniqueId failed") : PL_OK;
}
int pl_dist_loopback_id(void *id_out) {
  if (!id_out) return fail(PL_ERR_ARG, "pl_dist_loopback_id: null argument");
  pl::dist_loopback_id(id_out);
  return PL_OK;
}
int pl_dist_init(pl_handle h, int rank, int world, const void *unique_id, const int32_t *shared_local,
                 const int32_t *shared_global, int32_t n_shared, int32_t n_shared_global) {
  if (!valid(h) || !unique_id || world < 1 || rank < 0 || rank >= world || n_shared < 0)
    return fail(PL_ERR_ARG, "pl_dist_init: bad argument");
  if (n_shared > 0 && (!shared_local || !shared_global)) return fail(PL_ERR_ARG, "pl_dist_init: null index array");
  PL_HIP(hipSetDevice(h->opt.device));
  std::vector<int32_t> loc(n_shared);
  for (int i = 0; i < n_shared; ++i) {
    if (shared_local[i] < 0 || shared_local[i] >= h->N || shared_global[i] < 0 || shared_global[i] >= n_shared_global)
      return fail(PL_ERR_ARG, "pl_dist_init: shared node index out of range");
    loc[i] = h->iperm[shared_local[i]];
  }
  int rc = pl::dist_init(h->dist, rank, world, unique_id, loc.data(), shared_global, n_shared, n_shared_global, h->N,
                         h->stream);
  if (rc == 6)
    return fail(PL_ERR_ARG, "pl_dist_init: loopback group mismatch (all ranks of a loopback id must share one device and one "
                            "world size <= " + std::to_string(pl::kLoopMaxWorld) + ", each rank attaches once)");
  if (rc) return fail(PL_ERR_HIP, "pl_dist_init: communicator setup failed (" + std::to_string(rc) + ")");
  h->h_shared.assign((size_t)h->N, 0);
  for (int i = 0; i < n_shared; ++i) h->h_shared[loc[i]] = 1;
  h->ov_ready = false;
  if (h->coarse.enabled) {
    h->cond_ready = false;
    h->n_cond = 0;
    h->cond_agree = -1;
    PL_HIP(hipMemcpy(h->sharedbits.p, h->h_shared.data(), h->h_shared.size(), hipMemcpyHostToDevice));
    h->coarseL.n_fix = -1;
  }
  h->assembled = false;
  return PL_OK;
}

int pl_dist_abort(pl_handle h) {
  if (!valid(h)) return fail(PL_ERR_ARG, "pl_dist_abort: null handle");
  if (h->dist.loop) {
    std::lock_guard<std::mutex> lk(h->dist.loop->m);
    h->dist.loop->broken = true;
    h->dist.loop->cv.notify_all();
  }
  return PL_OK;
}

int pl_dist_set_peers(pl_handle h, const int32_t *shared_peer) {
  if (!valid(h) || !shared_peer) return fail(PL_ERR_ARG, "pl_dist_set_peers: null argument");
  if (!h->dist.active) return fail(PL_ERR_STATE, "pl_dist_set_peers: call pl_dist_init first");
  PL_HIP(hipSetDevice(h->opt.device));
  int rc = pl::dist_set_peers(h->dist, shared_peer);
  if (rc) return fail(rc == 2 ? PL_ERR_ARG : PL_ERR_HIP, "pl_dist_set_peers: setup failed (" + std::to_string(rc) + ")");
  h->assembled = false;
  h->ov_ready = false;
  if (h->opt.overlap >= 0 && h->tile.ready && h->opkind == 0 && !h->h_tile_start.empty()) {
    const int64_t T = (int64_t)h->h_tile_start.size() - 1;
    std::vector<int32_t> iface, inner;
    for (int64_t t = 0; t < T; ++t) {
      bool has = false;
      for (int32_t i = h->h_tile_start[t]; i < h->h_tile_start[t + 1] && !has; ++i) has = h->h_shared[i] != 0;
      (has ? iface : inner).push_back((int32_t)t);
    }
    if (!iface.empty() && !inner.empty()) {
      PL_HIP(h->ov_iface.alloc(iface.size()));
      PL_HIP(h->ov_inner.alloc(inner.size()));
      PL_HIP(hipMemcpy(h->ov_iface.p, iface.data(), iface.size() * sizeof(int32_t), hipMemcpyHostToDevice));
      PL_HIP(hipMemcpy(h->ov_inner.p, inner.data(), inner.size() * sizeof(int32_t), hipMemcpyHostToDevice));
      h->n_ov_iface = (int64_t)iface.size();
      h->n_ov_inner = (int64_t)inner.size();
      if (!h->comm_stream) {
        int prio_low = 0, prio_high = 0;
        PL_HIP(hipDeviceGetStreamPriorityRange(&prio_low, &prio_high));
        PL_HIP(hipStreamCreateWithPriority(&h->comm_stream, hipStreamNonBlocking, prio_high));
        PL_HIP(hipEventCreateWithFlags(&h->ev_ov_a, hipEventDisableTiming));
        PL_HIP(hipEventCreateWithFlags(&h->ev_ov_x, hipEventDisableTiming));
      }
      h->ov_ready = true;
    }
  }
  return PL_OK;
}

}
```

pylatticedso_amd/csrc/pl_assembly.h:

```cpp
#pragma once
#include "pl_ops.h"

namespace {

inline bool small_wanted(const pl_context *c) {
  const pl::Coarse &cs = c->coarse;
  if (c->opt.short_iteration < 0 || c->opkind != 0 || c->dist.active || c->coarseL.enabled || c->opt.precision != 0 ||
      c->opt.cg_form == 1 || !cs.enabled || !c->tile.ready || choose_kernel(c) != 3 || c->opt.mintol > 0.0 ||
      c->opt.restart_every > 0)
    return false;
  if (c->opt.short_iteration == 1) return true;
  static const double auto_mb = [] { const char *e = std::getenv("PL_SHORT_ITERATION_MB"); return e ? std::atof(e) : 16.0; }();
  return (double)cs.n_tiles * cs.cm * cs.ncp * 4.0 <= auto_mb * 1048576.0;
}


int launch_records(pl_context *c) {
  hipLaunchKernelGGL(pl::k_build_records, dim3(grid_for(c->B)), dim3(pl::kBlock), 0, c->stream, c->B, c->xyz.p,
                     c->conn.p, c->radius.p, c->seg_len.p, c->seg_nsub.p, c->mult.p, c->mat, c->rec.p, c->rec5.p);
  PL_HIP(hipGetLastError());
  return PL_OK;
}

void refresh_visit_words(pl_context *c, hipStream_t st) {
// ... 58 lines not shown
  const dim3 g(grid_for(c->B)), blk(pl::kBlock);
  hipLaunchKernelGGL(pl::k_pal_insert, g, blk, 0, st, c->B, c->rec.p, c->pal_keys.p, c->pal_owner.p, c->pal_id.p,
                     c->pal_flags.p);
  hipLaunchKernelGGL(pl::k_pal_publish, g, blk, 0, st, c->B, c->rec.p, c->pal_owner.p, c->pal_id.p, c->palette.p);
  hipLaunchKernelGGL(pl::k_pal_verify, g, blk, 0, st, c->B, c->rec.p, c->pal_id.p, c->palette.p, c->pal_owner.p,
                     c->pal_flags.p, c->pal_dense_of_slot.p, c->pal_dense.p, pl::kPalDenseMax);
  refresh_visit_words(c, st);
  if (c->pal_dense2.p)
    hipLaunchKernelGGL(pl::k_pal_orient, dim3(1), dim3(pl::kPalDenseMax), 0, st, pl::kPalDenseMax, c->pal_dense.p,
                       c->pal_dense2.p);
  PL_HIP(hipGetLastError());
  PL_HIP(hipMemcpyAsync(c->pal_host_flags, c->pal_flags.p, 2 * sizeof(int), hipMemcpyDeviceToHost, st));
  return PL_OK;
}
void finish_palette(pl_context *c) {
  if (!c->opt.palette) return;
  if (c->pal_skipped) {
    c->pal_entries = 0;
    c->pal_ready = false;
    c->pal_lds = false;
    c->pal_rows = false;
    return;
  }
  c->pal_entries = c->pal_host_flags[1];
  c->pal_ready = (c->pal_host_flags[0] == 0);
  static const bool lds_off = [] { const char *e = std::getenv("PL_TILE_LDS"); return e && e[0] == '0'; }();
  c->pal_lds = c->pal_ready && c->vword.p && c->pal_entries > 0 && c->pal_entries <= pl::kPalDenseMax && !lds_off;
  if (c->pal_ready && !c->pal_lds && !lds_off && small_wanted(c) && c->rec5.p && c->vword_dir.p && c->tile.n_dir > 0 &&
      c->tile.n_dir <= pl::kPalDenseMax)
    c->pal_ready = false;
  if (c->pal_ready) {
    c->pal_fail_streak = 0;
  } else {
    c->pal_fail_streak = std::min(c->pal_fail_streak + 1, 4);
    c->pal_skip_left = (1 << c->pal_fail_streak) - 1;
  }
  const char *re = std::getenv("PL_ROWS");
  c->pal_rows = c->pal_lds && c->rword.p && c->pal_dense2.p && re && re[0] == '1';
}
int build_palette(pl_context *c) {
  int rc = launch_palette(c, c->stream);
  if (rc) return rc;
  PL_HIP(hipStreamSynchronize(c->stream));
  finish_palette(c);
  return PL_OK;
}

int launch_diag(pl_context *c, hipStream_t st) {
  const unsigned g = grid_for(c->n_slices, pl::kBlock / pl::kWave);
  const uint8_t *fb = c->have_bc ? c->fixedbits.p : (const uint8_t *)nullptr;
#define PL_D(L)                                                                                                  \
  hipLaunchKernelGGL((pl::k_diag_gather<L>), dim3(g), dim3(pl::kBlock), 0, st, c->N, c->slice_ptr.p, c->ent.p, \
                     c->rec.p, fb, c->diag.p, c->dinv.p)
  switch (c->lpn) { case 1: PL_D(1); break; case 2: PL_D(2); break; case 4: PL_D(4); break; case 8: PL_D(8); break;
                    default: PL_D(16); }
#undef PL_D
  PL_HIP(hipGetLastError());
  return PL_OK;
}
int finish_diag_dist(pl_context *c) {
  if (!c->dist.active) return PL_OK;
  int rc = pl::dist_sum_shared(c->dist, c->diag.p, c->stream);
  if (rc) return fail(PL_ERR_HIP, "RCCL all-reduce of the Jacobi diagonal failed");
  pl::launch_invert_diag(c->N * 6, c->diag.p, c->have_bc ? c->fixed.p : nullptr, c->dinv.p, c->stream);
  return PL_OK;
}

__global__ void k_local_mask(int64_t N, const uint8_t *__restrict__ fixedbits, const uint8_t *__restrict__ shared,
                             uint8_t *__restrict__ mask) {
  const int64_t i = (int64_t)blockIdx.x * blockDim.x + threadIdx.x;
  if (i < N) mask[i] = (uint8_t)(fixedbits[i] | (shared[i] ? 0x3f : 0));
}

int launch_dinv32(pl_context *c) {
  if (!c->coarse.enabled) return PL_OK;
  hipLaunchKernelGGL(pl::k_to_float, dim3(grid_for(c->N * 6)), dim3(pl::kBlock), 0, c->stream, c->N * 6, c->dinv.p,
                     c->coarse.dinv32);
  PL_HIP(hipGetLastError());
  return PL_OK;
}

inline bool node_words_apply(const pl_context *c) {
  return c->coarse.enabled && c->coarse.nword.p && !c->dist.active && !c->coarseL.ready;
}
int launch_node_classes(pl_context *c, hipStream_t st, bool convert) {
  pl::Coarse &cs = c->coarse;
  cs.dcl_ready = false;
  cs.dcl_classes = 0;
  c->dcl_pending = false;
  if (!cs.enabled || !cs.nword.p || !cs.dcl_table || !c->have_bc || c->dist.active || c->coarseL.enabled)
    return PL_OK;
  if (c->dcl_skip_left > 0) {
    c->dcl_skip_left--;
    return PL_OK;
  }
  if (!c->dcl_keys.p) {
    PL_HIP(c->dcl_keys.alloc(pl::kDclSlots));
    PL_HIP(c->dcl_owner.alloc(pl::kDclSlots));
    PL_HIP(c->dcl_dense_of_slot.alloc(pl::kDclSlots));
    PL_HIP(c->dcl_flags.alloc(2));
    PL_HIP(c->dcl_slot.alloc((size_t)c->N));
    void *pinned = nullptr;
    PL_HIP(hipHostMalloc(&pinned, 2 * sizeof(int), hipHostMallocDefault));
    c->dcl_host_flags = static_cast<int *>(pinned);
  }
  c->dcl_host_flags[0] = 1;
  c->dcl_host_flags[1] = 0;
  PL_HIP(hipMemsetAsync(c->dcl_keys.p, 0xFF, pl::kDclSlots * sizeof(unsigned long long), st));
  PL_HIP(hipMemsetAsync(c->dcl_owner.p, 0x7F, pl::kDclSlots * sizeof(int), st));
  PL_HIP(hipMemsetAsync(c->dcl_dense_of_slot.p, 0xFF, pl::kDclSlots * sizeof(int), st));
  PL_HIP(hipMemsetAsync(c->dcl_flags.p, 0, 2 * sizeof(int), st));
  const dim3 g(grid_for(c->N)), blk(pl::kBlock);
  if (convert)
    hipLaunchKernelGGL(pl::k_to_float, dim3(grid_for(c->N * 6)), blk, 0, st, c->N * 6, c->dinv.p, cs.dinv32);
  hipLaunchKernelGGL(pl::k_dcl_insert, g, blk, 0, st, c->N, (const float *)cs.dinv32, (const uint8_t *)c->fixedbits.p,
                     c->dcl_keys.p, c->dcl_owner.p, c->dcl_slot.p, c->dcl_flags.p);
  hipLaunchKernelGGL(pl::k_dcl_publish, g, blk, 0, st, c->N, (const float *)cs.dinv32, (const uint8_t *)c->fixedbits.p,
                     (const int *)c->dcl_owner.p, (const uint16_t *)c->dcl_slot.p, c->dcl_dense_of_slot.p, cs.dcl_table,
                     c->dcl_flags.p);
  hipLaunchKernelGGL(pl::k_dcl_verify, g, blk, 0, st, c->N, (const float *)cs.dinv32, (const uint8_t *)c->fixedbits.p,
                     (const uint16_t *)c->dcl_slot.p, (const int *)c->dcl_dense_of_slot.p, (const uint32_t *)cs.dcl_table,
                     cs.nword.p, c->dcl_flags.p);
  PL_HIP(hipGetLastError());
  PL_HIP(hipMemcpyAsync(c->dcl_host_flags, c->dcl_flags.p, 2 * sizeof(int), hipMemcpyDeviceToHost, st));
  c->dcl_pending = true;
  return PL_OK;
}
void finish_node_classes(pl_context *c) {
  if (!c->dcl_pending) return;
  c->dcl_pending = false;
  pl::Coarse &cs = c->coarse;
  cs.dcl_classes = c->dcl_host_flags[1];
  cs.dcl_ready = c->dcl_host_flags[0] == 0 && cs.dcl_classes > 0 && cs.dcl_classes <= pl::kDclMax;
  if (cs.dcl_ready) {
    c->dcl_fail_streak = 0;
  } else {
    c->dcl_fail_streak = std::min(c->dcl_fail_streak + 1, 4);
    c->dcl_skip_left = (1 << c->dcl_fail_streak) - 1;
  }
}

int launch_local_mask(pl_context *c) {
  if (!c->coarse.enabled || !(c->dist.active || c->coarseL.enabled)) return PL_OK;
  hipLaunchKernelGGL(k_local_mask, dim3(grid_for(c->N)), dim3(pl::kBlock), 0, c->stream, c->N, c->fixedbits.p,
                     c->sharedbits.p, c->maskL.p);
  PL_HIP(hipGetLastError());
  return PL_OK;
}

inline int tile_modes_now(const pl_context *c) {
  return (c->coarse.tile_level && c->coarse.tile_modes == 12 && !c->coarseL.enabled) ? 12 : 6;
}

int launch_tile_blocks(pl_context *c, hipStream_t st) {
  pl::Coarse &cs = c->coarse;
  if (!cs.enabled || !c->have_bc || !cs.tile_level) return PL_OK;
  if (cs.cm == 12) return PL_OK;
  const uint8_t *fb = c->dist.active ? c->maskL.p : c->fixedbits.p;
  const bool twelve = tile_modes_now(c) == 12;
  if (!twelve)
    hipLaunchKernelGGL(pl::k_tile_blocks, dim3((unsigned)cs.n_tiles), dim3(pl::kBlock), 0, st, c->tile.tile_start.p,
                       c->tile.home_ptr.p, c->tile.foreign_ptr.p, c->tile.foreign_idx.p,
                       reinterpret_cast<const int2 *>(c->conn.p), c->rec.p, cs.agg_of_tile.p, cs.cen.p, c->xyz.p,
                       fb, cs.Bt_inv, (double *)nullptr);
  if (twelve) {
    hipLaunchKernelGGL(pl::k_tile_blocks_strain<true>, dim3((unsigned)cs.n_tiles), dim3(pl::kBlock), 0, st,
                       c->tile.tile_start.p, c->tile.home_ptr.p, c->tile.foreign_ptr.p, c->tile.foreign_idx.p,
                       reinterpret_cast<const int2 *>(c->conn.p), c->rec.p, cs.agg_of_tile.p, cs.cen.p, c->xyz.p, fb,
                       cs.Bt_raw);
    hipLaunchKernelGGL(pl::k_tile_blocks_strain<false>, dim3((unsigned)cs.n_tiles), dim3(pl::kBlock), 0, st,
                       c->tile.tile_start.p, c->tile.home_ptr.p, c->tile.foreign_ptr.p, c->tile.foreign_idx.p,
                       reinterpret_cast<const int2 *>(c->conn.p), c->rec.p, cs.agg_of_tile.p, cs.cen.p, c->xyz.p, fb,
                       cs.Bt_raw);
    hipLaunchKernelGGL(pl::k_tile_invert12, dim3((unsigned)cs.n_tiles), dim3(pl::kInv12Block), 0, st, cs.n_tiles,
                       (const double *)cs.Bt_raw, cs.Bt_inv);
  }
  PL_HIP(hipGetLastError());
  return PL_OK;
}

int build_coarse_level(pl_context *c, pl::Coarse &cs, const uint8_t *mask, bool reduce,
                       const std::function<void(int)> &after_chol = nullptr) {
  cs.ready = false;
  if (!cs.enabled || !c->have_bc) {
    if (after_chol) after_chol(1);
    return PL_OK;
  }
  bool tile_invert_pending = false;
  const int n = cs.ncp;
  if (!cs.ac_clean) PL_HIP(hipMemsetAsync(cs.Ac, 0, (size_t)n * n * sizeof(double), c->stream));
  cs.ac_clean = false;
  PL_HIP(hipMemsetAsync(cs.info, 0, 2 * sizeof(int), c->stream));
  if (cs.cm == 12) {
    const dim3 gt((unsigned)cs.n_tiles), blk(pl::kBlock);
    const int2 *conn2 = reinterpret_cast<const int2 *>(c->conn.p);
    const bool two_sets = c->dist.active;
    if (two_sets) {
      if (!cs.Bt_rawA && hipMalloc((void **)&cs.Bt_rawA, (size_t)cs.n_tiles * 144 * sizeof(double)) != hipSuccess)
        return fail(PL_ERR_HIP, "pl_assemble: out of device memory for the tile blocks");
      hipLaunchKernelGGL(pl::k_tile_blocks_strain<true>, gt, blk, 0, c->stream, c->tile.tile_start.p, c->tile.home_ptr.p,
                         c->tile.foreign_ptr.p, c->tile.foreign_idx.p, conn2, c->rec.p, cs.agg_of_tile.p, cs.cen.p,
                         c->xyz.p, (const uint8_t *)c->maskL.p, cs.Bt_raw);
      hipLaunchKernelGGL(pl::k_tile_blocks_strain<false>, gt, blk, 0, c->stream, c->tile.tile_start.p, c->tile.home_ptr.p,
                         c->tile.foreign_ptr.p, c->tile.foreign_idx.p, conn2, c->rec.p, cs.agg_of_tile.p, cs.cen.p,
                         c->xyz.p, (const uint8_t *)c->maskL.p, cs.Bt_raw);
    }
    double *rawA = two_sets ? cs.Bt_rawA : cs.Bt_raw;
    PL_HIP(hipEventRecord(c->ev_t0, c->stream));
    PL_HIP(hipStreamWaitEvent(c->side2, c->ev_t0, 0));
    hipLaunchKernelGGL(pl::k_tile_blocks_strain<true>, gt, blk, 0, c->side2, c->tile.tile_start.p, c->tile.home_ptr.p,
                       c->tile.foreign_ptr.p, c->tile.foreign_idx.p, conn2, c->rec.p, cs.agg_of_tile.p, cs.cen.p, c->xyz.p,
                       mask, rawA);
    if (cs.n_cross > 0)
      hipLaunchKernelGGL(pl::k_coarse_cross12, dim3(grid_for(cs.n_cross)), blk, 0, c->side2, cs.n_cross,
                         cs.cross_idx.p, c->conn.p, c->rec.p, cs.agg_of_node.p, cs.cen.p, c->xyz.p, mask, n, cs.Ac);
    PL_HIP(hipEventRecord(c->ev_t1, c->side2));
    hipLaunchKernelGGL(pl::k_tile_blocks_strain<false>, gt, blk, 0, c->stream, c->tile.tile_start.p, c->tile.home_ptr.p,
                       c->tile.foreign_ptr.p, c->tile.foreign_idx.p, conn2, c->rec.p, cs.agg_of_tile.p, cs.cen.p, c->xyz.p,
                       mask, rawA);
    PL_HIP(hipStreamWaitEvent(c->stream, c->ev_t1, 0));
    hipLaunchKernelGGL(pl::k_agg_add_tiles, dim3(grid_for(cs.n_tiles * 144)), blk, 0, c->stream, cs.n_tiles,
                       cs.agg_of_tile.p, (const double *)rawA, n, cs.Ac);
    PL_HIP(hipEventRecord(c->ev_t0, c->stream));
    PL_HIP(hipStreamWaitEvent(c->side2, c->ev_t0, 0));
    hipLaunchKernelGGL(pl::k_tile_invert12, dim3((unsigned)cs.n_tiles), dim3(pl::kInv12Block), 0,
                       c->side2, cs.n_tiles, (const double *)cs.Bt_raw, cs.Bt_inv);
    PL_HIP(hipEventRecord(c->ev_t1, c->side2));
    tile_invert_pending = true;
  } else {
  if (cs.n_fix < 0) {
    if (!cs.fix_count) PL_HIP(hipMalloc((void **)&cs.fix_count, sizeof(int)));
    int cnt = 0;
    DevBuf<int64_t> keys;
    for (int pass = 0; pass < 2; ++pass) {
      PL_HIP(hipMemsetAsync(cs.fix_count, 0, sizeof(int), c->stream));
      hipLaunchKernelGGL(pl::k_list_fixed_struts, dim3(grid_for(c->B)), dim3(pl::kBlock), 0, c->stream, c->B,
                         c->conn.p, cs.agg_of_node.p, mask, pass ? keys.p : (int64_t *)nullptr, cs.fix_count);
      if (pass == 0) {
        PL_HIP(hipMemcpyAsync(&cnt, cs.fix_count, sizeof(int), hipMemcpyDeviceToHost, c->stream));
        PL_HIP(hipStreamSynchronize(c->stream));
        if (cnt == 0) break;
        PL_HIP(keys.alloc((size_t)cnt));
      }
    }
    std::vector<int32_t> list;
    if (cnt > 0) {
      std::vector<int64_t> hk((size_t)cnt);
      PL_HIP(hipMemcpyAsync(hk.data(), keys.p, hk.size() * sizeof(int64_t), hipMemcpyDeviceToHost, c->stream));
      PL_HIP(hipStreamSynchronize(c->stream));
      std::sort(hk.begin(), hk.end());
      list.reserve(hk.size() + hk.size() / 4 + pl::kWave);
      for (size_t q = 0; q < hk.size(); ++q) {
        if (q > 0 && (hk[q] >> 32) != (hk[q - 1] >> 32))
          while (list.size() % pl::kWave) list.push_back(-1);
        list.push_back((int32_t)(hk[q] & 0xffffffffLL));
      }
      while (list.size() % pl::kWave) list.push_back(-1);
      PL_HIP(cs.fix_list.upload(list));
    }
    cs.n_fix = (int64_t)list.size();
  }
  if (cs.n_fix > 0)
    hipLaunchKernelGGL(pl::k_coarse_assemble, dim3(grid_for(cs.n_fix)), dim3(pl::kBlock), 0, c->stream, cs.n_fix,
                       cs.fix_list.p, c->conn.p, c->rec.p, cs.agg_of_node.p, cs.cen.p, c->xyz.p, mask, n,
                       cs.Ac);
  if (cs.n_cross > 0)
    hipLaunchKernelGGL(pl::k_coarse_assemble_cross, dim3(grid_for(cs.n_cross)), dim3(pl::kBlock), 0, c->stream,
                       cs.n_cross, cs.cross_idx.p, c->conn.p, c->rec.p, cs.agg_of_node.p, cs.cen.p, c->xyz.p,
                       mask, n, cs.Ac);
  }
  if (reduce && c->dist.active) {
    const int nb = n / pl::kNB;
    if (cs.bw_blocks > 0 && cs.bw_blocks + 1 < nb) {
      const int64_t cnt = (int64_t)n * (cs.bw_blocks + 1) * pl::kNB;
      hipLaunchKernelGGL(pl::k_band_pack, dim3((unsigned)((cnt + 255) / 256)), dim3(256), 0, c->stream, n, n,
                         cs.bw_blocks, cs.Ac, cs.Lf);
      if (pl::dist_sum_scalars(c->dist, cs.Lf, (int)cnt, c->stream))
        return fail(PL_ERR_HIP, "RCCL all-reduce of the coarse operator failed");
      hipLaunchKernelGGL(pl::k_band_unpack, dim3((unsigned)((cnt + 255) / 256)), dim3(256), 0, c->stream, n, n,
                         cs.bw_blocks, cs.Lf, cs.Ac);
    } else if (pl::dist_sum_scalars(c->dist, cs.Ac, n * n, c->stream)) {
      return fail(PL_ERR_HIP, "RCCL all-reduce of the coarse operator failed");
    }
  }
  hipLaunchKernelGGL(pl::k_coarse_regularize, dim3((n + 255) / 256), dim3(256), 0, c->stream, n, cs.Ac);
  pl::TrtriPhases ph;
  {
    const char *e = std::getenv("PL_TRTRI_ROWS");
    ph.rows = e ? std::atoi(e) : 3;
    ph.stream = c->side2;
    ph.ev_go = c->ev_p0;
    ph.ev_done = c->ev_p1;
  }
  pl::coarse_factor(cs, n, c->stream, after_chol, c->opt.chol_persistent ? cs.bar : (unsigned *)nullptr, ph);
  cs.ainv_ready = false;
  if (&cs == &c->coarse && (small_wanted(c) || (n <= pl::kOneGemvMaxDofs && c->opkind == 0))) {
    if (!cs.Ainv && hipMalloc((void **)&cs.Ainv, (size_t)n * n * sizeof(float)) != hipSuccess)
      return fail(PL_ERR_HIP, "pl_assemble: out of device memory for the explicit inverse of the dense level");
    const long tiles = (long)(n / 32) * (n / 32 + 1) / 2;
    if (cs.w16)
      hipLaunchKernelGGL(pl::k_dense_explicit_inverse<pl::bf16_t>, dim3((unsigned)((tiles + 3) / 4)), dim3(256), 0, c->stream, n,
                         reinterpret_cast<const pl::bf16_t *>(cs.W), n, cs.Ainv);
    else
      hipLaunchKernelGGL(pl::k_dense_explicit_inverse<float>, dim3((unsigned)((tiles + 3) / 4)), dim3(256), 0, c->stream, n,
                         (const float *)cs.W, n, cs.Ainv);
    cs.ainv_ready = true;
  }
  if (tile_invert_pending) PL_HIP(hipStreamWaitEvent(c->stream, c->ev_t1, 0));
  PL_HIP(hipGetLastError());
  int info[2] = {0, 0};
  PL_HIP(hipMemcpyAsync(info, cs.info, sizeof(info), hipMemcpyDeviceToHost, c->stream));
  PL_HIP(hipStreamSynchronize(c->stream));
  if (&cs == &c->coarse) c->coarse_info = info[0];
  cs.ready = (info[0] == 0);
  return PL_OK;
}

int build_coarse(pl_context *c, const std::function<void(int)> &after_chol = nullptr) {
  int rc = build_coarse_level(c, c->coarse, c->fixedbits.p, true, after_chol);
  if (rc || !c->coarseL.enabled) return rc;
  return build_coarse_level(c, c->coarseL, c->maskL.p, false);
}

inline const double *cinv(const pl_context *c) { return c->cls_ready ? c->cls_table.p : c->kcc_inv.p; }
inline const uint16_t *ccls(const pl_context *c) { return c->cls_ready ? c->cls_id.p : (const uint16_t *)nullptr; }

int select_condensed(pl_context *c, const std::vector<uint8_t> &bits) {
  c->cond_ready = false;
  c->n_cond = 0;
  c->cond_agree = -1;
  const bool wanted = c->opt.condense >= 0 && c->opkind == 0 && c->coarse.enabled && c->opt.precision != 2 &&
                      !c->h_cand.empty();
  if (!wanted) return PL_OK;
  const int64_t N = c->N;
  std::vector<int32_t> picked;
  for (int64_t i = 0; i < N; ++i)
    if (c->h_cand[i] && !bits[i] && (c->h_shared.empty() || !c->h_shared[i])) picked.push_back((int32_t)i);
  if (picked.empty()) return PL_OK;
  std::vector<uint8_t> flag((size_t)N, 0), mask(bits);
  for (int32_t i : picked) {
    flag[i] = 1;
    mask[i] = 0x3f;
  }
  PL_HIP(c->cnodes.alloc(picked.size()));
  PL_HIP(c->kcc_inv.alloc(picked.size() * 36));
  if (!c->maskC.p) {
    PL_HIP(c->maskC.alloc(N));
    PL_HIP(c->cflag.alloc(N));
  }
  PL_HIP(hipMemcpy(c->cnodes.p, picked.data(), picked.size() * sizeof(int32_t), hipMemcpyHostToDevice));
  {
    std::vector<int32_t> keep;
    keep.reserve((size_t)N - picked.size());
    for (int64_t i = 0; i < N; ++i)
      if (!flag[i]) keep.push_back((int32_t)i);
    PL_HIP(c->ckeep.alloc(std::max<size_t>(1, keep.size())));
    if (!keep.empty()) PL_HIP(hipMemcpy(c->ckeep.p, keep.data(), keep.size() * sizeof(int32_t), hipMemcpyHostToDevice));
  }
  if (!c->cbase.p) PL_HIP(c->cbase.alloc(N));
  c->cbase_state = -1;
  PL_HIP(hipMemcpy(c->maskC.p, mask.data(), N, hipMemcpyHostToDevice));
  PL_HIP(hipMemcpy(c->cflag.p, flag.data(), N, hipMemcpyHostToDevice));
  if (!c->cend.p) PL_HIP(c->cend.alloc(c->B));
  hipLaunchKernelGGL(k_cond_ends, dim3(grid_for(c->B)), dim3(pl::kBlock), 0, c->stream, c->B,
                     reinterpret_cast<const int2 *>(c->conn.p), (const uint8_t *)c->cflag.p, c->cend.p);
  refresh_visit_words(c, c->stream);
  if (refresh_visit_words_dir(c, c->stream)) return PL_ERR_HIP;
  PL_HIP(hipGetLastError());
  c->n_cond = (int64_t)picked.size();
  return PL_OK;
}
int agree_condensed(pl_context *c) {
// ... 175 lines not shown
```

pylatticedso_amd/csrc/pl_coarse.h:

```cpp
#pragma once
#include <hip/hip_runtime.h>

#include <algorithm>
#include <cstdint>
#include <cstdlib>
#include <vector>

#include "pl_dense.h"
#include "pl_kernels.h"
#include "pl_nodeword.h"
#include "pl_tile.h"

namespace pl {

constexpr int kDclMax = 256;
constexpr int kDclSlots = 4096;
inline bool node_words_enabled() {
  const char *e = std::getenv("PL_NODE_WORDS");
  return !(e && e[0] == '0');
}

struct Coarse {
  bool enabled = false;
  bool ready = false;
  int n_agg = 0, nc = 0, ncp = 0;
  int cm = 6;
  int bw_blocks = 0;
  int64_t n_tiles = 0;
  int vblock = kBlock;
  TBuf<int32_t> agg_of_node, agg_of_tile;
  TBuf<int32_t> tile_of_node;
  TBuf<double> cen;
  TBuf<int32_t> cross_idx;
  int64_t n_cross = 0;
  float *Ainv = nullptr;
  bool ainv_ready = false;
  float *W = nullptr, *Wt = nullptr;
  bool w16 = false;
  double *Ac = nullptr, *Lf = nullptr, *Dinv = nullptr, *rc = nullptr, *yc = nullptr, *tv = nullptr;
  int *info = nullptr;
  unsigned *bar = nullptr;
  bool ac_clean = false;
  bool tile_level = true;
  std::vector<int32_t> h_tile_start;
  double *Bt_inv = nullptr, *yt = nullptr;
  int tile_modes = 6;
  double *Bt_raw = nullptr;
  double *Bt_rawA = nullptr;
  float *dinv32 = nullptr;
  TBuf<float> rel32;
  bool rel_exact = false;
  TBuf<uint32_t> nword;
  int rel_e = -1;
  bool dcl_ready = false;
  int dcl_classes = 0;
  uint32_t *dcl_table = nullptr;
  TBuf<int32_t> fix_list;
  int *fix_count = nullptr;
  int64_t n_fix = -1;
  ~Coarse() {
    for (void *q : {(void *)Ac, (void *)Lf, (void *)W, (void *)Wt, (void *)Dinv, (void *)rc, (void *)yc, (void *)tv,
                    (void *)info, (void *)Bt_inv, (void *)yt, (void *)fix_count, (void *)dinv32, (void *)bar,
                    (void *)Bt_raw, (void *)Bt_rawA, (void *)Ainv, (void *)dcl_table})
      if (q) (void)hipFree(q);
  }
};

inline int coarse_setup(Coarse &c, const std::vector<int32_t> &tile_start, const std::vector<int64_t> &tile_brick,
                        const BrickGrid &grid, const double *xyz_dev_order, int64_t N, int max_dofs,
                        const std::vector<int32_t> &conn, bool local = false, bool multi_rank = false, int modes = 6) {
  const int64_t T = (int64_t)tile_start.size() - 1;
  c.cm = modes;
  const int64_t *nbrick = grid.nb;
  int ax[3] = {0, 1, 2};
  std::stable_sort(ax, ax + 3, [&](int l, int r) { return nbrick[l] > nbrick[r]; });
  auto grid_agg = [&](int64_t key, int , const int64_t *na) {
    const int64_t b[3] = {key / (nbrick[2] * nbrick[1]), (key / nbrick[2]) % nbrick[1], key % nbrick[2]};
    const int64_t a0 = b[ax[0]] * na[ax[0]] / nbrick[ax[0]], a1 = b[ax[1]] * na[ax[1]] / nbrick[ax[1]],
                  a2 = b[ax[2]] * na[ax[2]] / nbrick[ax[2]];
    return (a0 * na[ax[1]] + a1) * na[ax[2]] + a2;
  };
  int g = 2;
  int64_t na[3];
  std::vector<int64_t> used;
  for (int step = 0;; ++step) {
    const double scale = 1.5 + 0.125 * step;
    for (int k = 0; k < 3; ++k) na[k] = std::max<int64_t>(1, (int64_t)std::floor((double)nbrick[k] / scale));
    if (!local && step == 0 && grid.na[0] > 0 && modes * grid.na[0] * grid.na[1] * grid.na[2] <= max_dofs)
      for (int k = 0; k < 3; ++k) na[k] = grid.na[k];
    int64_t count = na[0] * na[1] * na[2];
    if (local) {
      used.clear();
      for (int64_t t = 0; t < T; ++t) used.push_back(grid_agg(tile_brick[t], g, na));
      std::sort(used.begin(), used.end());
      used.erase(std::unique(used.begin(), used.end()), used.end());
      count = (int64_t)used.size();
    }
    if (count * modes <= max_dofs || scale > 64.0) break;
  }
  const int n_agg = local ? (int)used.size() : (int)(na[0] * na[1] * na[2]);
  std::vector<int32_t> agg_of_tile(T), agg_of_node(N);
  std::vector<double> cen((size_t)n_agg * 3, 0.0);
  for (int a = 0; a < n_agg; ++a) {
    const int64_t ga = local ? used[a] : a;
    int64_t ai[3];
    ai[ax[0]] = ga / (na[ax[1]] * na[ax[2]]);
    ai[ax[1]] = (ga / na[ax[2]]) % na[ax[1]];
    ai[ax[2]] = ga % na[ax[2]];
    for (int k = 0; k < 3; ++k) {
      const int64_t b_lo = (ai[k] * nbrick[k] + na[k] - 1) / na[k], b_hi = ((ai[k] + 1) * nbrick[k] + na[k] - 1) / na[k];
      cen[3 * a + k] = grid.lo[k] + 0.5 * (double)(b_lo + b_hi) * grid.side[k];
    }
  }
  for (int64_t t = 0; t < T; ++t) {
    const int64_t ga = grid_agg(tile_brick[t], g, na);
    const int a = local ? (int)(std::lower_bound(used.begin(), used.end(), ga) - used.begin()) : (int)ga;
    agg_of_tile[t] = a;
    for (int32_t i = tile_start[t]; i < tile_start[t + 1]; ++i) agg_of_node[i] = a;
  }
  {
    if (hipMalloc((void **)&c.dinv32, (size_t)N * 6 * sizeof(float)) != hipSuccess) return 2;
    c.rel_exact = false;
    if (!local && xyz_dev_order && !std::getenv("PL_NO_REL32")) {
      std::vector<float> rel((size_t)N * 3);
      bool exact = true;
      for (int64_t i = 0; i < N && exact; ++i)
        for (int k = 0; k < 3; ++k) {
          const double d = xyz_dev_order[3 * i + k] - cen[3 * (size_t)agg_of_node[i] + k];
          const float f = (float)d;
          if ((double)f != d) {
            exact = false;
            break;
          }
          rel[3 * (size_t)i + k] = f;
        }
      if (exact) {
        if (c.rel32.upload(rel) != hipSuccess) return 1;
        c.rel_exact = true;
      }
    }
    c.rel_e = -1;
    if (!local && xyz_dev_order && node_words_enabled()) {
      std::vector<double> d((size_t)N * 3);
      for (int64_t i = 0; i < N; ++i)
        for (int k = 0; k < 3; ++k) d[3 * (size_t)i + k] = xyz_dev_order[3 * i + k] - cen[3 * (size_t)agg_of_node[i] + k];
      std::vector<uint32_t> words;
      int e = -1;
      if (pack_rel_bytes(d.data(), (size_t)N, words, e)) c.rel_e = e;
      else words.assign((size_t)N, 0u);
      if (c.nword.upload(words) != hipSuccess) return 1;
      if (hipMalloc((void **)&c.dcl_table, (size_t)kDclMax * 8 * sizeof(uint32_t)) != hipSuccess) return 2;
    }
  }
  c.n_agg = n_agg;
  c.nc = modes * n_agg;
  c.n_tiles = T;
  {
    int longest = 1;
    for (int64_t t = 0; t < T; ++t) longest = std::max(longest, (int)(tile_start[t + 1] - tile_start[t]));
    c.vblock = std::min(kBlock, (longest + kWave - 1) / kWave * kWave);
  }
  {
    const int64_t B = (int64_t)conn.size() / 2;
    std::vector<std::pair<int64_t, int32_t>> cross;
    std::vector<int32_t> tile_of_node(N);
    for (int64_t t = 0; t < T; ++t)
      for (int32_t i = tile_start[t]; i < tile_start[t + 1]; ++i) tile_of_node[i] = (int32_t)t;
    if (c.tile_of_node.upload(tile_of_node) != hipSuccess) return 1;
    for (int64_t b = 0; b < B; ++b) {
      const int I = agg_of_node[conn[2 * b]], J = agg_of_node[conn[2 * b + 1]];
      if (I != J || (modes == 12 && tile_of_node[conn[2 * b]] != tile_of_node[conn[2 * b + 1]]))
        cross.push_back({(int64_t)I * n_agg + J, (int32_t)b});
    }
    int64_t max_diff = std::min<int64_t>(n_agg - 1, na[ax[1]] * na[ax[2]] + na[ax[2]] + 1);
    if (local) {
      max_diff = 0;
      for (const auto &pr : cross) max_diff = std::max<int64_t>(max_diff, std::abs(pr.first / n_agg - pr.first % n_agg));
    }
    c.bw_blocks = (int)((modes * (max_diff + 1) + kNB - 1) / kNB + 1);
    for (const auto &pr : cross)
      if (std::abs(pr.first / n_agg - pr.first % n_agg) > max_diff) {
        if (multi_rank && !local) return 4;
        c.bw_blocks = 0;
      }
    std::sort(cross.begin(), cross.end());
    std::vector<int32_t> idx2;
    idx2.reserve(cross.size() + cross.size() / 2);
    for (size_t q = 0; q < cross.size(); ++q) {
      if (q > 0 && cross[q].first != cross[q - 1].first)
        while (idx2.size() % kWave) idx2.push_back(-1);
      idx2.push_back(cross[q].second);
    }
    while (idx2.size() % kWave) idx2.push_back(-1);
    c.n_cross = (int64_t)idx2.size();
    if (c.cross_idx.upload(idx2) != hipSuccess) return 1;
  }
  if (c.agg_of_node.upload(agg_of_node) != hipSuccess || c.agg_of_tile.upload(agg_of_tile) != hipSuccess ||
      c.cen.upload(cen) != hipSuccess)
    return 1;
  c.ncp = (c.nc + kNB - 1) / kNB * kNB;
  const size_t n2 = (size_t)c.ncp * c.ncp;
  if (hipMalloc((void **)&c.Ac, n2 * sizeof(double)) != hipSuccess) return 2;
  c.ac_clean = false;
  if (hipMalloc((void **)&c.W, n2 * sizeof(float)) != hipSuccess) return 2;
  if (hipMalloc((void **)&c.Lf, n2 * sizeof(double)) != hipSuccess) return 2;
  if (hipMemset(c.Lf, 0, n2 * sizeof(double)) != hipSuccess) return 2;
  if (hipMalloc((void **)&c.Wt, n2 * sizeof(float)) != hipSuccess) return 2;
  if (hipMalloc((void **)&c.Dinv, (size_t)c.ncp * kNB * sizeof(double)) != hipSuccess) return 2;
  if (hipMalloc((void **)&c.rc, (size_t)(c.ncp + 2 * kSlots) * sizeof(double)) != hipSuccess) return 2;
  if (hipMalloc((void **)&c.yc, (size_t)c.ncp * sizeof(double)) != hipSuccess) return 2;
  if (hipMalloc((void **)&c.tv, (size_t)c.ncp * sizeof(double)) != hipSuccess) return 2;
  if (hipMalloc((void **)&c.info, 2 * sizeof(int)) != hipSuccess) return 2;
  if (hipMalloc((void **)&c.bar, sizeof(unsigned)) != hipSuccess) return 2;
  {
    c.h_tile_start = tile_start;
    if (hipMalloc((void **)&c.Bt_inv, (size_t)T * 144 * sizeof(double)) != hipSuccess) return 2;
    if (hipMalloc((void **)&c.Bt_raw, (size_t)T * 144 * sizeof(double)) != hipSuccess) return 2;
    if (hipMalloc((void **)&c.yt, (size_t)T * 12 * sizeof(double)) != hipSuccess) return 2;
    if (hipMemset(c.Bt_inv, 0, (size_t)T * 144 * sizeof(double)) != hipSuccess) return 2;
    if (hipMemset(c.Bt_raw, 0, (size_t)T * 144 * sizeof(double)) != hipSuccess) return 2;
    if (hipMemset(c.yt, 0, (size_t)T * 12 * sizeof(double)) != hipSuccess) return 2;
  }
  if (hipMemset(c.rc, 0, (size_t)(c.ncp + 2 * kSlots) * sizeof(double)) != hipSuccess) return 2;
  if (hipMemset(c.W, 0, n2 * sizeof(float)) != hipSuccess) return 2;
  if (hipMemset(c.Wt, 0, n2 * sizeof(float)) != hipSuccess) return 2;
  c.enabled = true;
  return 0;
}

__global__ __launch_bounds__(kBlock) void k_list_fixed_struts(int64_t B, const int32_t *__restrict__ conn,
                                                              const int32_t *__restrict__ agg,
                                                              const uint8_t *__restrict__ fixedbits,
                                                              int64_t *__restrict__ keys, int *__restrict__ count) {
  const int64_t b = (int64_t)blockIdx.x * kBlock + threadIdx.x;
  if (b >= B) return;
  const int ia = conn[2 * b], ib = conn[2 * b + 1];
  const int I = agg[ia];
  if (I != agg[ib]) return;
  if ((fixedbits[ia] | fixedbits[ib]) == 0u) return;
  const int slot = atomicAdd(count, 1);
  if (keys) keys[slot] = ((int64_t)I << 32) | (int64_t)b;
}

__device__ __forceinline__ void coarse_block(const double *K, unsigned frow, unsigned fcol, const double *relp,
                                             const double *relq, double *C) {
  double Km[36];
#pragma unroll
  for (int i = 0; i < 6; ++i)
#pragma unroll
    for (int j = 0; j < 6; ++j) Km[i * 6 + j] = (((frow >> i) & 1u) || ((fcol >> j) & 1u)) ? 0.0 : K[i * 6 + j];
  const double Sq[3][3] = {{0, -relq[2], relq[1]}, {relq[2], 0, -relq[0]}, {-relq[1], relq[0], 0}};
  const double Sp[3][3] = {{0, -relp[2], relp[1]}, {relp[2], 0, -relp[0]}, {-relp[1], relp[0], 0}};
  double M[36];
#pragma unroll
  for (int i = 0; i < 6; ++i) {
#pragma unroll
    for (int j = 0; j < 3; ++j) M[i * 6 + j] = Km[i * 6 + j];
#pragma unroll
    for (int j = 0; j < 3; ++j) {
      double acc = Km[i * 6 + 3 + j];
#pragma unroll
      for (int k = 0; k < 3; ++k) acc -= Km[i * 6 + k] * Sq[k][j];
      M[i * 6 + 3 + j] = acc;
    }
  }
#pragma unroll
  for (int j = 0; j < 6; ++j) {
#pragma unroll
    for (int i = 0; i < 3; ++i) C[i * 6 + j] = M[i * 6 + j];
#pragma unroll
    for (int i = 0; i < 3; ++i) {
      double acc = M[(3 + i) * 6 + j];
#pragma unroll
      for (int k = 0; k < 3; ++k) acc += Sp[i][k] * M[k * 6 + j];
      C[(3 + i) * 6 + j] = acc;
    }
  }
}

__global__ __launch_bounds__(kBlock) void k_coarse_assemble(int64_t n_list, const int32_t *__restrict__ list,
                                                            const int32_t *__restrict__ conn,
                                                            const Record *__restrict__ rec,
                                                            const int32_t *__restrict__ agg,
                                                            const double *__restrict__ cen,
                                                            const double *__restrict__ xyz,
                                                            const uint8_t *__restrict__ fixedbits, int nc,
                                                            double *__restrict__ Ac) {
  const int64_t q = (int64_t)blockIdx.x * kBlock + threadIdx.x;
  if ((q & ~(int64_t)(kWave - 1)) >= n_list) return;
  const bool live = list[q] >= 0;
  const int64_t b = live ? list[q] : list[q & ~(int64_t)(kWave - 1)];
  const int ia = conn[2 * b], ib = conn[2 * b + 1];
  const int I = agg[ia];
  const unsigned fa = fixedbits[ia], fb = fixedbits[ib];
  const Record r = load_record(rec, b);
  double rela[3], relb[3];
#pragma unroll
  for (int k = 0; k < 3; ++k) {
    rela[k] = xyz[3 * (int64_t)ia + k] - cen[3 * I + k];
    relb[k] = xyz[3 * (int64_t)ib + k] - cen[3 * I + k];
  }
  double Kss[36], Kso[36], C[36], T[36];
  tip_blocks(r, Kss, Kso);
  coarse_block(Kss, fb, fb, relb, relb, T);
  coarse_block(Kso, fb, fa, relb, rela, C);
#pragma unroll
  for (int e = 0; e < 36; ++e) T[e] += C[e];
  tip_blocks(reversed(r), Kss, Kso);
  coarse_block(Kss, fa, fa, rela, rela, C);
#pragma unroll
  for (int e = 0; e < 36; ++e) T[e] += C[e];
  coarse_block(Kso, fa, fb, rela, relb, C);
#pragma unroll
  for (int e = 0; e < 36; ++e) T[e] += C[e];
  double *dII = Ac + ((size_t)6 * I) * nc + 6 * I;
  const bool uniform = __all(I == __shfl(I, 0, 64));
  if (uniform) {
#pragma unroll
    for (int e = 0; e < 36; ++e) {
      const double v = wave_sum(live ? T[e] : 0.0);
      if ((threadIdx.x & 63) == 0) unsafeAtomicAdd(dII + (size_t)(e / 6) * nc + e % 6, v);
    }
  } else if (live) {
#pragma unroll
    for (int e = 0; e < 36; ++e) unsafeAtomicAdd(dII + (size_t)(e / 6) * nc + e % 6, T[e]);
  }
}

__global__ __launch_bounds__(kBlock) void k_coarse_assemble_cross(int64_t n_cross, const int32_t *__restrict__ cross,
                                                                  const int32_t *__restrict__ conn,
                                                                  const Record *__restrict__ rec,
                                                                  const int32_t *__restrict__ agg,
                                                                  const double *__restrict__ cen,
                                                                  const double *__restrict__ xyz,
                                                                  const uint8_t *__restrict__ fixedbits, int nc,
                                                                  double *__restrict__ Ac) {
  const int64_t q = (int64_t)blockIdx.x * kBlock + threadIdx.x;
  if ((q & ~(int64_t)(kWave - 1)) >= n_cross) return;
  const bool live = cross[q] >= 0;
  const int64_t b = live ? cross[q] : cross[q & ~(int64_t)(kWave - 1)];
  const int ia = conn[2 * b], ib = conn[2 * b + 1];
  const int I = agg[ia], J = agg[ib];
  const unsigned fa = fixedbits ? fixedbits[ia] : 0u, fb = fixedbits ? fixedbits[ib] : 0u;
  const Record r = load_record(rec, b);
  double rela[3], relb[3];
#pragma unroll
  for (int k = 0; k < 3; ++k) {
    rela[k] = xyz[3 * (int64_t)ia + k] - cen[3 * I + k];
    relb[k] = xyz[3 * (int64_t)ib + k] - cen[3 * J + k];
  }
  double Kss[36], Kso[36], Cjj[36], Cii[36], Cx[36];
  tip_blocks(r, Kss, Kso);
  coarse_block(Kss, fb, fb, relb, relb, Cjj);
  if (J > I) coarse_block(Kso, fb, fa, relb, rela, Cx);
  tip_blocks(reversed(r), Kss, Kso);
  coarse_block(Kss, fa, fa, rela, rela, Cii);
  if (I > J) coarse_block(Kso, fa, fb, rela, relb, Cx);
  const int hi = I > J ? I : J, lo = I > J ? J : I;
  double *dII = Ac + ((size_t)6 * I) * nc + 6 * I, *dJJ = Ac + ((size_t)6 * J) * nc + 6 * J;
  double *dX = Ac + ((size_t)6 * hi) * nc + 6 * lo;
  const int I0 = __shfl(I, 0, 64), J0 = __shfl(J, 0, 64);
  const bool uniform = __all(I == I0 && J == J0);
  if (uniform) {
#pragma unroll
    for (int e = 0; e < 36; ++e) {
      const double a = wave_sum(live ? Cii[e] : 0.0), c = wave_sum(live ? Cjj[e] : 0.0), x = wave_sum(live ? Cx[e] : 0.0);
      if ((threadIdx.x & 63) == 0) {
        const int i = e / 6, j = e - 6 * i;
        unsafeAtomicAdd(dII + (size_t)i * nc + j, a);
        unsafeAtomicAdd(dJJ + (size_t)i * nc + j, c);
        unsafeAtomicAdd(dX + (size_t)i * nc + j, x);
      }
    }
  } else if (live) {
#pragma unroll
    for (int e = 0; e < 36; ++e) {
      const int i = e / 6, j = e - 6 * i;
      unsafeAtomicAdd(dII + (size_t)i * nc + j, Cii[e]);
      unsafeAtomicAdd(dJJ + (size_t)i * nc + j, Cjj[e]);
      unsafeAtomicAdd(dX + (size_t)i * nc + j, Cx[e]);
    }
  }
}

__device__ __forceinline__ V3 strain_disp(int q, const double *r) {
  switch (q) {
    case 0: return {r[0], 0.0, 0.0};
    case 1: return {0.0, r[1], 0.0};
    case 2: return {0.0, 0.0, r[2]};
    case 3: return {0.5 * r[1], 0.5 * r[0], 0.0};
    case 4: return {0.0, 0.5 * r[2], 0.5 * r[1]};
    default: return {0.5 * r[2], 0.0, 0.5 * r[0]};
  }
}
__device__ __forceinline__ void strain_restrict(const V3 &F, const double *r, double *s6, double sign) {
  s6[0] += sign * r[0] * F.x;
  s6[1] += sign * r[1] * F.y;
  s6[2] += sign * r[2] * F.z;
  s6[3] += sign * 0.5 * (r[1] * F.x + r[0] * F.y);
  s6[4] += sign * 0.5 * (r[2] * F.y + r[1] * F.z);
  s6[5] += sign * 0.5 * (r[2] * F.x + r[0] * F.z);
}
__device__ __forceinline__ V3 mask3(V3 v, unsigned bits) {
  return {(bits & 1u) ? 0.0 : v.x, (bits & 2u) ? 0.0 : v.y, (bits & 4u) ? 0.0 : v.z};
}
__global__ __launch_bounds__(kBlock) void k_agg_add_tiles(int64_t T, const int32_t *__restrict__ agg_of_tile,
                                                          const double *__restrict__ raw, int nc,
                                                          double *__restrict__ Ac) {
  const int64_t q = (int64_t)blockIdx.x * kBlock + threadIdx.x;
  const int64_t t = q / 144;
  if (t >= T) return;
  const int e = (int)(q - 144 * t), i = e / 12, j = e - 12 * i;
  if (j > i) return;
  const int a = agg_of_tile[t];
  const double v = 0.5 * (raw[t * 144 + i * 12 + j] + raw[t * 144 + j * 12 + i]);
  if (v != 0.0) unsafeAtomicAdd(Ac + ((size_t)12 * a + i) * nc + 12 * a + j, v);
}
__device__ __forceinline__ void mode_disp(int n, const double *r, V3 &u, V3 &th) {
  th = {0.0, 0.0, 0.0};
  if (n >= 6) {
    u = strain_disp(n - 6, r);
    return;
  }
  switch (n) {
    case 0: u = {1.0, 0.0, 0.0}; break;
    case 1: u = {0.0, 1.0, 0.0}; break;
    case 2: u = {0.0, 0.0, 1.0}; break;
    case 3: u = {0.0, -r[2], r[1]}; th = {1.0, 0.0, 0.0}; break;
    case 4: u = {r[2], 0.0, -r[0]}; th = {0.0, 1.0, 0.0}; break;
    default: u = {-r[1], r[0], 0.0}; th = {0.0, 0.0, 1.0}; break;
  }
}
__global__ __launch_bounds__(kBlock) void k_coarse_cross12(int64_t n_cross, const int32_t *__restrict__ list,
                                                           const int32_t *__restrict__ conn,
                                                           const Record *__restrict__ rec,
                                                           const int32_t *__restrict__ agg,
                                                           const double *__restrict__ cen,
                                                           const double *__restrict__ xyz,
                                                           const uint8_t *__restrict__ fixedbits, int nc,
                                                           double *__restrict__ Ac) {
  const int64_t q = (int64_t)blockIdx.x * kBlock + threadIdx.x;
  if ((q & ~(int64_t)(kWave - 1)) >= n_cross) return;
  const bool live = list[q] >= 0;
  const int64_t b = live ? list[q] : list[q & ~(int64_t)(kWave - 1)];
  const int ia = conn[2 * b], ib = conn[2 * b + 1];
  const int I = agg[ia], J = agg[ib];
  const unsigned fa = fixedbits ? fixedbits[ia] : 0u, fb = fixedbits ? fixedbits[ib] : 0u;
  const Record r = load_record(rec, b);
  double rela[3], relb[3];
#pragma unroll
  for (int k = 0; k < 3; ++k) {
    rela[k] = xyz[3 * (int64_t)ia + k] - cen[3 * I + k];
    relb[k] = xyz[3 * (int64_t)ib + k] - cen[3 * J + k];
  }
  const V3 d = {r.dx, r.dy, r.dz}, zero = {0.0, 0.0, 0.0};
  const int lane = threadIdx.x & 63;
  for (int n = 0; n < 12; ++n) {
    V3 uB, tB;
    mode_disp(n, relb, uB, tB);
    uB = mask3(uB, fb);
    tB = mask3(tB, fb >> 3);
    V3 F, M;
    tip_force(r, zero, zero, uB, tB, F, M);
    const V3 FA = mask3((-1.0) * F, fa), MA = mask3((-1.0) * M - cross(d, F), fa >> 3);
    double x[12] = {FA.x, FA.y, FA.z,
                    MA.x + (rela[1] * FA.z - rela[2] * FA.y), MA.y + (rela[2] * FA.x - rela[0] * FA.z),
                    MA.z + (rela[0] * FA.y - rela[1] * FA.x), 0, 0, 0, 0, 0, 0};
    strain_restrict(FA, rela, x + 6, 1.0);
#pragma unroll
    for (int m = 0; m < 12; ++m) {
      const double v = wave_sum(live ? x[m] : 0.0);
      if (lane == 0 && v != 0.0) {
        const size_t ri = (size_t)12 * I + m, cj = (size_t)12 * J + n;
        if (ri > cj) unsafeAtomicAdd(Ac + ri * nc + cj, v);
        else if (cj > ri) unsafeAtomicAdd(Ac + cj * nc + ri, v);
        else unsafeAtomicAdd(Ac + ri * nc + cj, 2.0 * v);
      }
    }
  }
}

__global__ void k_coarse_regularize(int nc, double *__restrict__ Ac) {
  const int i = blockIdx.x * blockDim.x + threadIdx.x;
  if (i >= nc) return;
  if (!(Ac[(size_t)i * nc + i] > 0.0)) Ac[(size_t)i * nc + i] = 1.0;
}
__device__ __forceinline__ void spd6_inverse(double *A ) {
  double dmax = 0.0;
#pragma unroll
  for (int i = 0; i < 6; ++i) dmax = fmax(dmax, A[i * 6 + i]);
  double L[36];
  bool keep[6];
#pragma unroll
  for (int e = 0; e < 36; ++e) L[e] = 0.0;
#pragma unroll
  for (int j = 0; j < 6; ++j) {
    double s = A[j * 6 + j];
#pragma unroll
    for (int k = 0; k < 6; ++k)
      if (k < j) s -= L[j * 6 + k] * L[j * 6 + k];
    keep[j] = s > 1e-12 * dmax;
    if (!keep[j]) {
#pragma unroll
      for (int k = 0; k < 6; ++k) L[j * 6 + k] = 0.0;
      L[j * 6 + j] = 1.0;
      continue;
    }
    const double d = sqrt(s);
    L[j * 6 + j] = d;
#pragma unroll
    for (int i = 0; i < 6; ++i)
      if (i > j) {
        double v = 0.5 * (A[i * 6 + j] + A[j * 6 + i]);
#pragma unroll
        for (int k = 0; k < 6; ++k)
          if (k < j) v -= L[i * 6 + k] * L[j * 6 + k];
        L[i * 6 + j] = v / d;
      }
  }
  double W[36];
#pragma unroll
  for (int e = 0; e < 36; ++e) W[e] = 0.0;
#pragma unroll
  for (int j = 0; j < 6; ++j) {
    W[j * 6 + j] = 1.0 / L[j * 6 + j];
#pragma unroll
    for (int i = 0; i < 6; ++i)
      if (i > j) {
        double v = 0.0;
#pragma unroll
        for (int k = 0; k < 6; ++k)
          if (k >= j && k < i) v -= L[i * 6 + k] * W[k * 6 + j];
        W[i * 6 + j] = v / L[i * 6 + i];
      }
  }
#pragma unroll
  for (int i = 0; i < 6; ++i)
#pragma unroll
    for (int j = 0; j < 6; ++j) {
      double v = 0.0;
#pragma unroll
      for (int k = 0; k < 6; ++k)
        if (k >= i && k >= j) v += W[k * 6 + i] * W[k * 6 + j];
      A[i * 6 + j] = (keep[i] && keep[j]) ? v : 0.0;
    }
}

__global__ void k_band_pack(int n, int ld, int bwb, double *__restrict__ A, double *__restrict__ P) {
  const int W = (bwb + 1) * kNB;
  const int64_t e = (int64_t)blockIdx.x * blockDim.x + threadIdx.x;
  if (e >= (int64_t)n * W) return;
  const int i = (int)(e / W), j = (i / kNB - bwb) * kNB + (int)(e % W);
  double v = 0.0;
  if (j >= 0) {
    v = A[(size_t)i * ld + j];
    A[(size_t)i * ld + j] = 0.0;
  }
  P[e] = v;
}
__global__ void k_band_unpack(int n, int ld, int bwb, const double *__restrict__ P, double *__restrict__ A) {
  const int W = (bwb + 1) * kNB;
  const int64_t e = (int64_t)blockIdx.x * blockDim.x + threadIdx.x;
  if (e >= (int64_t)n * W) return;
  const int i = (int)(e / W), j = (i / kNB - bwb) * kNB + (int)(e % W);
  if (j >= 0) A[(size_t)i * ld + j] = P[e];
}

__global__ __launch_bounds__(kBlock) void k_tile_blocks(const int32_t *__restrict__ tile_start,
                                                        const int64_t *__restrict__ home_ptr,
                                                        const int64_t *__restrict__ foreign_ptr,
                                                        const int32_t *__restrict__ foreign_idx,
                                                        const int2 *__restrict__ conn2, const Record *__restrict__ rec,
                                                        const int32_t *__restrict__ agg_of_tile,
                                                        const double *__restrict__ cen, const double *__restrict__ xyz,
                                                        const uint8_t *__restrict__ fixedbits,
                                                        double *__restrict__ Bt_inv,
                                                        double *__restrict__ raw ) {
  __shared__ double red[36][kBlock / kWave];
  __shared__ double A[36];
  const int t = blockIdx.x;
  const int n0 = tile_start[t], n1 = tile_start[t + 1];
  const int a = agg_of_tile[t];
  const double c0 = cen[3 * a], c1 = cen[3 * a + 1], c2 = cen[3 * a + 2];
  double acc[36];
#pragma unroll
  for (int e = 0; e < 36; ++e) acc[e] = 0.0;
  const int64_t h0 = home_ptr[t], h1 = home_ptr[t + 1], f0 = foreign_ptr[t], f1 = foreign_ptr[t + 1];
  const int64_t total = (h1 - h0) + (f1 - f0);
  for (int64_t q = threadIdx.x; q < total; q += kBlock) {
    const int64_t b = q < (h1 - h0) ? h0 + q : (int64_t)foreign_idx[f0 + (q - (h1 - h0))];
    const int2 cn = conn2[b];
    const bool ina = cn.x >= n0 && cn.x < n1, inb = cn.y >= n0 && cn.y < n1;
    const unsigned fa = fixedbits ? fixedbits[cn.x] : 0u, fb = fixedbits ? fixedbits[cn.y] : 0u;
    if (ina && inb && fa == 0u && fb == 0u) continue;
    const Record r = load_record(rec, b);
    const double rela[3] = {xyz[3 * (int64_t)cn.x] - c0, xyz[3 * (int64_t)cn.x + 1] - c1, xyz[3 * (int64_t)cn.x + 2] - c2};
    const double relb[3] = {xyz[3 * (int64_t)cn.y] - c0, xyz[3 * (int64_t)cn.y + 1] - c1, xyz[3 * (int64_t)cn.y + 2] - c2};
    double Kss[36], Kso[36], C[36];
    if (inb) {
      tip_blocks(r, Kss, Kso);
      coarse_block(Kss, fb, fb, relb, relb, C);
#pragma unroll
      for (int e = 0; e < 36; ++e) acc[e] += C[e];
      if (ina) {
        coarse_block(Kso, fb, fa, relb, rela, C);
#pragma unroll
        for (int e = 0; e < 36; ++e) acc[e] += C[e];
      }
    }
    if (ina) {
      tip_blocks(reversed(r), Kss, Kso);
      coarse_block(Kss, fa, fa, rela, rela, C);
#pragma unroll
      for (int e = 0; e < 36; ++e) acc[e] += C[e];
      if (inb) {
        coarse_block(Kso, fa, fb, rela, relb, C);
#pragma unroll
        for (int e = 0; e < 36; ++e) acc[e] += C[e];
      }
    }
  }
  const int lane = threadIdx.x & 63, wv = threadIdx.x >> 6;
#pragma unroll
  for (int e = 0; e < 36; ++e) {
    const double s = wave_sum(acc[e]);
    if (lane == 0) red[e][wv] = s;
  }
  __syncthreads();
  if (threadIdx.x < 36) {
    double s = 0.0;
#pragma unroll
    for (int q = 0; q < kBlock / kWave; ++q) s += red[threadIdx.x][q];
    A[threadIdx.x] = s;
  }
  __syncthreads();
  if (raw) {
    if (threadIdx.x < 36) raw[(size_t)t * 144 + (threadIdx.x / 6) * 12 + threadIdx.x % 6] = A[threadIdx.x];
    return;
  }
  if (threadIdx.x == 0) {
    double M[36];
#pragma unroll
    for (int e = 0; e < 36; ++e) M[e] = A[e];
    spd6_inverse(M);
#pragma unroll
    for (int e = 0; e < 36; ++e) Bt_inv[(size_t)t * 36 + e] = M[e];
  }
}

template <bool RIGID>
__global__ __launch_bounds__(kBlock) void k_tile_blocks_strain(const int32_t *__restrict__ tile_start,
                                                               const int64_t *__restrict__ home_ptr,
                                                               const int64_t *__restrict__ foreign_ptr,
                                                               const int32_t *__restrict__ foreign_idx,
                                                               const int2 *__restrict__ conn2,
                                                               const Record *__restrict__ rec,
                                                               const int32_t *__restrict__ agg_of_tile,
                                                               const double *__restrict__ cen,
                                                               const double *__restrict__ xyz,
                                                               const uint8_t *__restrict__ fixedbits,
                                                               double *__restrict__ raw) {
  __shared__ double red[57][kBlock / kWave];
  const int t = blockIdx.x;
  const int n0 = tile_start[t], n1 = tile_start[t + 1];
  const int a = agg_of_tile[t];
  const double c0 = cen[3 * a], c1 = cen[3 * a + 1], c2 = cen[3 * a + 2];
  double SS[21], RS[RIGID ? 1 : 36];
  double RR[RIGID ? 21 : 1];
#pragma unroll
  for (int e = 0; e < (RIGID ? 21 : 1); ++e) RR[e] = 0.0;
#pragma unroll
  for (int e = 0; e < 21; ++e) SS[e] = 0.0;
#pragma unroll
  for (int e = 0; e < (RIGID ? 1 : 36); ++e) RS[e] = 0.0;
  const int64_t h0 = home_ptr[t], h1 = home_ptr[t + 1], f0 = foreign_ptr[t], f1 = foreign_ptr[t + 1];
  const int64_t total = (h1 - h0) + (f1 - f0);
  for (int64_t v = threadIdx.x; v < total; v += kBlock) {
    const int64_t b = v < (h1 - h0) ? h0 + v : (int64_t)foreign_idx[f0 + (v - (h1 - h0))];
    const int2 cn = conn2[b];
    const bool ina = cn.x >= n0 && cn.x < n1, inb = cn.y >= n0 && cn.y < n1;
    if (!ina && !inb) continue;
    const unsigned fa = fixedbits ? fixedbits[cn.x] : 0u, fb = fixedbits ? fixedbits[cn.y] : 0u;
    const bool free_inside = ina && inb && fa == 0u && fb == 0u;
    if (RIGID && free_inside) continue;
    const Record r = load_record(rec, b);
    const double rela[3] = {xyz[3 * (int64_t)cn.x] - c0, xyz[3 * (int64_t)cn.x + 1] - c1, xyz[3 * (int64_t)cn.x + 2] - c2};
    const double relb[3] = {xyz[3 * (int64_t)cn.y] - c0, xyz[3 * (int64_t)cn.y + 1] - c1, xyz[3 * (int64_t)cn.y + 2] - c2};
    const V3 d = {r.dx, r.dy, r.dz}, zero = {0.0, 0.0, 0.0};
#pragma unroll
    for (int q = 0; q < (RIGID ? 0 : 6); ++q) {
      const V3 uA = ina ? mask3(strain_disp(q, rela), fa) : zero, uB = inb ? mask3(strain_disp(q, relb), fb) : zero;
      V3 F, M;
      tip_force(r, uA, zero, uB, zero, F, M);
      const V3 FB = mask3(F, fb), MB = mask3(M, fb >> 3);
      const V3 FA = mask3((-1.0) * F, fa), MA = mask3((-1.0) * M - cross(d, F), fa >> 3);
      double s6[6] = {0, 0, 0, 0, 0, 0};
      if (inb) strain_restrict(FB, relb, s6, 1.0);
      if (ina) strain_restrict(FA, rela, s6, 1.0);
#pragma unroll
      for (int p = 0; p <= q; ++p) SS[q * (q + 1) / 2 + p] += s6[p];
      if (!free_inside) {
        if (inb) {
          RS[0 * 6 + q] += FB.x;
          RS[1 * 6 + q] += FB.y;
          RS[2 * 6 + q] += FB.z;
          RS[3 * 6 + q] += MB.x + (relb[1] * FB.z - relb[2] * FB.y);
          RS[4 * 6 + q] += MB.y + (relb[2] * FB.x - relb[0] * FB.z);
          RS[5 * 6 + q] += MB.z + (relb[0] * FB.y - relb[1] * FB.x);
        }
        if (ina) {
          RS[0 * 6 + q] += FA.x;
          RS[1 * 6 + q] += FA.y;
          RS[2 * 6 + q] += FA.z;
          RS[3 * 6 + q] += MA.x + (rela[1] * FA.z - rela[2] * FA.y);
          RS[4 * 6 + q] += MA.y + (rela[2] * FA.x - rela[0] * FA.z);
          RS[5 * 6 + q] += MA.z + (rela[0] * FA.y - rela[1] * FA.x);
        }
      }
    }
    if (RIGID && !free_inside) {
#pragma unroll
      for (int q = 0; q < 6; ++q) {
        V3 uA = zero, tA = zero, uB = zero, tB = zero;
        if (ina) {
          mode_disp(q, rela, uA, tA);
          uA = mask3(uA, fa);
          tA = mask3(tA, fa >> 3);
        }
        if (inb) {
          mode_disp(q, relb, uB, tB);
          uB = mask3(uB, fb);
          tB = mask3(tB, fb >> 3);
        }
        V3 F, M;
        tip_force(r, uA, tA, uB, tB, F, M);
        double x6[6] = {0, 0, 0, 0, 0, 0};
        if (inb) {
          const V3 FB = mask3(F, fb), MB = mask3(M, fb >> 3);
          x6[0] += FB.x;
          x6[1] += FB.y;
          x6[2] += FB.z;
          x6[3] += MB.x + (relb[1] * FB.z - relb[2] * FB.y);
          x6[4] += MB.y + (relb[2] * FB.x - relb[0] * FB.z);
          x6[5] += MB.z + (relb[0] * FB.y - relb[1] * FB.x);
        }
        if (ina) {
          const V3 FA = mask3((-1.0) * F, fa), MA = mask3((-1.0) * M - cross(d, F), fa >> 3);
          x6[0] += FA.x;
          x6[1] += FA.y;
          x6[2] += FA.z;
          x6[3] += MA.x + (rela[1] * FA.z - rela[2] * FA.y);
          x6[4] += MA.y + (rela[2] * FA.x - rela[0] * FA.z);
          x6[5] += MA.z + (rela[0] * FA.y - rela[1] * FA.x);
        }
#pragma unroll
        for (int p = 0; p <= q; ++p) RR[q * (q + 1) / 2 + p] += x6[p];
      }
    }
  }
  const int lane = threadIdx.x & 63, wv = threadIdx.x >> 6;
  double *B = raw + (size_t)t * 144;
  if (RIGID) {
#pragma unroll
    for (int e = 0; e < 21; ++e) {
      const double s0 = wave_sum(RR[e]);
      if (lane == 0) red[e][wv] = s0;
    }
    __syncthreads();
    if (threadIdx.x < 21) {
      double v = 0.0;
#pragma unroll
      for (int q = 0; q < kBlock / kWave; ++q) v += red[threadIdx.x][q];
      int q = 0;
      while ((q + 1) * (q + 2) / 2 <= (int)threadIdx.x) ++q;
      const int p = (int)threadIdx.x - q * (q + 1) / 2;
      B[p * 12 + q] = v;
      B[q * 12 + p] = v;
    }
    return;
  }
#pragma unroll
  for (int e = 0; e < 21; ++e) {
    const double s1 = wave_sum(SS[e]);
    if (lane == 0) red[e][wv] = s1;
  }
#pragma unroll
  for (int e = 0; e < (RIGID ? 1 : 36); ++e) {
    const double s2 = wave_sum(RS[e]);
    if (lane == 0) red[21 + e][wv] = s2;
  }
  __syncthreads();
  if (threadIdx.x < 57) {
    double v = 0.0;
#pragma unroll
    for (int q = 0; q < kBlock / kWave; ++q) v += red[threadIdx.x][q];
    if (threadIdx.x < 21) {
      int q = 0;
      while ((q + 1) * (q + 2) / 2 <= (int)threadIdx.x) ++q;
      const int p = (int)threadIdx.x - q * (q + 1) / 2;
      B[(6 + p) * 12 + 6 + q] = v;
      B[(6 + q) * 12 + 6 + p] = v;
    } else {
      const int e = (int)threadIdx.x - 21, p = e / 6, q = e % 6;
      B[p * 12 + 6 + q] = v;
      B[(6 + q) * 12 + p] = v;
    }
  }
}
constexpr int kInv12Block = 192;
__global__ __launch_bounds__(kInv12Block) void k_tile_invert12(int64_t T, const double *__restrict__ raw,
                                                              double *__restrict__ Bt_inv) {
  constexpr int n = 12;
  __shared__ double A[n][n + 1];
  __shared__ double diag0[n];
  const int64_t t = blockIdx.x;
  if (t >= T) return;
  const int e = threadIdx.x, i = e / n, j = e - n * i;
  const bool act = e < n * n;
  if (act) A[i][j] = 0.5 * (raw[t * 144 + i * n + j] + raw[t * 144 + j * n + i]);
  __syncthreads();
  if (e < n) diag0[e] = A[e][e];
  __syncthreads();
  unsigned dropped = 0u;
  for (int k = 0; k < n; ++k) {
    const double d = A[k][k];
    if (!(d > 1e-10 * diag0[k]) || !(diag0[k] > 0.0)) {
      dropped |= 1u << k;
      continue;
    }
    const double inv = 1.0 / d;
    double v = 0.0;
    if (act) {
      const bool di = (dropped >> i) & 1u, dj = (dropped >> j) & 1u;
      if (i == k && j == k) v = -inv;
      else if (i == k) v = A[k][j] * inv;
      else if (j == k) v = A[k][i] * inv;
      else if (di || dj) v = A[i][j];
      else v = A[i][j] - (A[i][k] * inv) * A[k][j];
    }
    __syncthreads();
    if (act) A[i][j] = v;
    __syncthreads();
  }
  if (act) {
    const bool out = ((dropped >> i) & 1u) || ((dropped >> j) & 1u);
    Bt_inv[t * 144 + i * n + j] = out ? 0.0 : -A[i][j];
  }
}
inline void coarse_factor(Coarse &cs, int n, hipStream_t s, const std::function<void(int)> &after_chol, unsigned *bar,
                          TrtriPhases ph = TrtriPhases()) {
  if (cs.w16)
    dense_factor_inverse(cs.Ac, cs.Lf, reinterpret_cast<bf16_t *>(cs.W), reinterpret_cast<bf16_t *>(cs.Wt), cs.Dinv, n, n,
                         cs.info, cs.bw_blocks, s, after_chol, bar, ph);
  else
    dense_factor_inverse(cs.Ac, cs.Lf, cs.W, cs.Wt, cs.Dinv, n, n, cs.info, cs.bw_blocks, s, after_chol, bar, ph);
}
constexpr int kOneGemvMaxDofs = 2048;
inline void coarse_apply(const Coarse &cs, const double *r, double *t, double *y, double *dot_out, const double *add0,
                         hipStream_t s) {
  static const bool one_off = [] { const char *e = std::getenv("PL_ONE_GEMV"); return e && e[0] == '0'; }();
  if (cs.ainv_ready && cs.Ainv && cs.ncp <= kOneGemvMaxDofs && !one_off) {
    hipLaunchKernelGGL(k_full_gemv, dim3((cs.ncp + 3) / 4), dim3(kBlock), 0, s, cs.ncp, (const float *)cs.Ainv, cs.ncp, r, y,
                       dot_out, add0);
    return;
  }
  if (cs.w16)
    dense_apply(reinterpret_cast<const bf16_t *>(cs.W), reinterpret_cast<const bf16_t *>(cs.Wt), cs.ncp, cs.ncp, r, t, y,
                dot_out, add0, s);
  else
    dense_apply(cs.W, cs.Wt, cs.ncp, cs.ncp, r, t, y, dot_out, add0, s);
}

__global__ __launch_bounds__(kBlock) void k_to_float(int64_t n, const double *__restrict__ x, float *__restrict__ y) {
  const int64_t i = (int64_t)blockIdx.x * kBlock + threadIdx.x;
  if (i < n) y[i] = (float)x[i];
}

__device__ __forceinline__ void nword_rel(uint32_t w, double rscale, double &rx, double &ry, double &rz) {
  rx = (double)((int)(w << 24) >> 24) * rscale;
  ry = (double)((int)(w << 16) >> 24) * rscale;
  rz = (double)((int)(w << 8) >> 24) * rscale;
}

template <typename PT, typename RT, int TM = 6, bool MULTI = true, bool LOCAL = true>
__global__ __launch_bounds__(kBlock) void k_pcg_update_tile(const int32_t *__restrict__ tile_start,
                                                            const int32_t *__restrict__ agg_of_tile,
                                                            const double *__restrict__ cen,
                                                            const double *__restrict__ xyz,
                                                            const PT *__restrict__ Ap,
                                                            const float *__restrict__ dinv32,
                                                            const double *__restrict__ w ,
                                                            RT *__restrict__ r,
                                                            double *__restrict__ scal, double *__restrict__ rc,
                                                            const double *__restrict__ Bt_inv ,
                                                            double *__restrict__ yt,
                                                            const int32_t *__restrict__ aggL_of_tile ,
                                                            const double *__restrict__ cenL,
                                                            const uint8_t *__restrict__ shared ,
                                                            double *__restrict__ rcL, int ncp,
                                                            const uint8_t *__restrict__ skip_rows ,
                                                            int cm = 6 ,
                                                            const float *__restrict__ rel32 = nullptr ,
                                                            const uint32_t *__restrict__ nword = nullptr ,
                                                            const uint32_t *__restrict__ dtab = nullptr ,
                                                            double rscale = 0.0 ) {
  __shared__ double red[32][4 * kBlock / kWave];
  if constexpr (!MULTI) {
    w = nullptr;
    shared = nullptr;
  }
  if constexpr (!MULTI || !LOCAL) aggL_of_tile = nullptr;
  double *rr_slot = rc + ncp + (blockIdx.x & (kSlots - 1)), *rdr_slot = rr_slot + kSlots;
  const int t = blockIdx.x;
  double pap, old_rz;
  scalar_read2(scal, S_PAP, S_RZ_OLD, pap, old_rz);
  const double alpha = (pap != 0.0) ? old_rz / pap : 0.0;
  const int n0 = tile_start[t], n1 = tile_start[t + 1];
  const int a = agg_of_tile[t];
  const double c0 = cen[3 * a], c1 = cen[3 * a + 1], c2 = cen[3 * a + 2];
  __shared__ double sbi[16][TM];
  double bi[TM];
#pragma unroll
  for (int j = 0; j < TM; ++j) bi[j] = 0.0;
  const int my_mode = (TM == 12) ? ((int)threadIdx.x < 6 ? (int)threadIdx.x : ((int)threadIdx.x >= 8 && (int)threadIdx.x < 14
                                                                                   ? (int)threadIdx.x - 2 : -1))
                                 : ((int)threadIdx.x < 6 ? (int)threadIdx.x : -1);
  if (Bt_inv && my_mode >= 0) {
#pragma unroll
    for (int j = 0; j < TM; ++j) bi[j] = Bt_inv[(size_t)t * (TM * TM) + TM * my_mode + j];
  }
  if (threadIdx.x < 16) {
#pragma unroll
    for (int j = 0; j < TM; ++j) sbi[threadIdx.x][j] = bi[j];
  }
  double accS[6] = {0, 0, 0, 0, 0, 0};
  double accD[6] = {0, 0, 0, 0, 0, 0};
  double acc[8] = {0, 0, 0, 0, 0, 0, 0, 0};
  const int aL = aggL_of_tile ? aggL_of_tile[t] : 0;
  double l0 = 0.0, l1 = 0.0, l2 = 0.0;
  if (aggL_of_tile) {
    l0 = cenL[3 * aL];
    l1 = cenL[3 * aL + 1];
    l2 = cenL[3 * aL + 2];
  }
  double accL[6] = {0, 0, 0, 0, 0, 0};
  double accT[6] = {0, 0, 0, 0, 0, 0};
  const bool own_t = Bt_inv && shared;
  for (int i = n0 + threadIdx.x; i < n1; i += blockDim.x) {
    if (skip_rows && skip_rows[i]) continue;
// ... 714 lines not shown
```

pylatticedso_amd/csrc/pl_context.h:

```cpp
#pragma once
#include <hip/hip_runtime.h>

#include <algorithm>
#include <atomic>
#include <chrono>
#include <cmath>
#include <cstdlib>
#include <cstdio>
#include <cstring>
#include <functional>
#include <memory>
#include <numeric>
#include <string>
#include <vector>

#include "../../include/pylattice_hip.h"
#include "pl_kernels.h"
#include "pl_parallel.h"
#include "pl_tile.h"
#include "pl_rows.h"
#include "pl_dist.h"
#include "pl_coarse.h"
#include "pl_cg1.h"
#include "pl_small.h"
#include "pl_persist.h"
#include "pl_palette.h"
#include "pl_ddm.h"
#include "pl_lzone.h"

namespace {

thread_local std::string g_err;

int fail(int code, const std::string &msg) {
  g_err = msg;
  return code;
}

#define PL_HIP(expr)                                                                                   \
  do {                                                                                                 \
    hipError_t _e = (expr);                                                                            \
    if (_e != hipSuccess)                                                                              \
      return fail(PL_ERR_HIP, std::string(#expr) + ": " + hipGetErrorString(_e));                     \
  } while (0)

template <typename T>
struct DevBuf {
  T *p = nullptr;
  size_t n = 0;
  ~DevBuf() { release(); }
  void release() {
    if (p) (void)hipFree(p);
    p = nullptr;
    n = 0;
  }
  hipError_t alloc(size_t count) {
    release();
    n = count;
    if (count == 0) return hipSuccess;
    return hipMalloc(reinterpret_cast<void **>(&p), count * sizeof(T));
  }
};

inline unsigned grid_for(int64_t n, int block = pl::kBlock) { return (unsigned)((n + block - 1) / block); }
inline unsigned grid_stream(int64_t n) {
  return (unsigned)std::max<int64_t>(1, std::min<int64_t>((n + pl::kBlock - 1) / pl::kBlock, 2048));
}

}

struct pl_context {
  pl_opts_t opt{};
  pl::Material mat{};
  int64_t N = 0, B = 0;
  hipStream_t stream = nullptr;
  hipEvent_t ev0 = nullptr, ev1 = nullptr;
  hipStream_t side = nullptr;
  hipEvent_t ev_fork = nullptr, ev_join = nullptr, ev_chol = nullptr, ev_t0 = nullptr, ev_t1 = nullptr;
  hipEvent_t ev_p0 = nullptr, ev_p1 = nullptr;
  hipEvent_t ev_fill1 = nullptr;
  hipStream_t side2 = nullptr;
  hipStream_t side_cu = nullptr;
  bool assembled = false, have_bc = false, have_bsr = false;
  int pal_fallback_flags[2] = {1, 0};
  int *pal_host_flags = pal_fallback_flags;
  bool want_bsr = false;
  int bsr_with_bc = 0;

  std::vector<int32_t> perm, iperm;
  bool reordered = false;
  std::vector<int32_t> bperm;

  DevBuf<double> xyz, radius, seg_len;
  DevBuf<double> mult;
  DevBuf<int32_t> conn, seg_nsub;
  DevBuf<pl::Record> rec;
  DevBuf<double> rec5;
  DevBuf<int64_t> slice_ptr;
  DevBuf<int2> ent;
  int64_t n_slices = 0, n_ent = 0;
  int lpn = pl::kDefaultLPN;
  DevBuf<int64_t> bsr_rowptr;
  DevBuf<int32_t> bsr_col, ent_slot, diag_slot;
  DevBuf<double> bsr_vals;
  int64_t nblk = 0;
  std::vector<int64_t> h_rowptr;
  std::vector<int32_t> h_col;
  DevBuf<uint8_t> fixed;
  DevBuf<uint8_t> fixedbits;
  std::vector<uint8_t> h_fixedbits;
  DevBuf<double> ubar, f;
  DevBuf<double> diag, dinv, x, r, z, p, Ap, tmp, tmp2, scal, hist;
  DevBuf<double> xprev;
  bool xprev_valid = false;
  int pal_fail_streak = 0, pal_skip_left = 0;
  bool pal_skipped = false;
  DevBuf<double> xprev2;
  bool xprev2_valid = false;
  DevBuf<double> xprev3;
  bool xprev3_valid = false;
  static constexpr int kWarmMax = 8;
  DevBuf<double> gh[kWarmMax - 1];
  int gh_head = 0, gh_count = 0;
  DevBuf<double> gw[kWarmMax];
  DevBuf<double> gw_dots;
  DevBuf<double> cg1;
  int hist_cap = 0;
  pl::TilePlan tile;
  int opkind = 0;
  int64_t ddm_cells = 0;
  int ddm_nb = 0;
  int ddm_n_S = 0;
  std::vector<int32_t> h_ddm_cell_nodes, h_ddm_cell_S;
  DevBuf<int32_t> ddm_cell_nodes, ddm_cell_S;
  DevBuf<double> ddm_St;
  DevBuf<double> ddm_Sraw;
  DevBuf<int64_t> ddm_node_ptr;
  DevBuf<int32_t> ddm_node_ent;
  DevBuf<double> ddm_stage;
  DevBuf<int32_t> ddm_order;
  DevBuf<int32_t> ddm_tiles, ddm_tile_S;
  int64_t ddm_n_tiles = 0;
  DevBuf<int32_t> ddm_tile_gidx;
  DevBuf<int32_t> ddm_cell_P;
  DevBuf<double> ddm_Pt;
  bool ddm_have_P = false;
  DevBuf<double> dd_A, dd_Lf, dd_W, dd_Wt, dd_Dinv, dd_tv;
  DevBuf<int> dd_info;
  int dd_n = 0;
  int dd_bw = 0;
  bool dd_ready = false;
  DevBuf<double> dd_B;
  bool dd_blocks = false;
  DevBuf<double> dd2_xyz, dd2_cen;
  DevBuf<int32_t> dd2_agg, dd2_ptr, dd2_nodes;
  pl::Coarse dd2;
  int dd2_n_agg = 0;
  bool dd2_plan = false, dd2_ready = false;
  DevBuf<int> stop_flag;
  bool stop_use = false;
  double stop_thresh = 0.0;
  DevBuf<unsigned long long> pal_keys;
  DevBuf<int> pal_owner, pal_flags;
  DevBuf<uint16_t> pal_id;
  DevBuf<int> pal_dense_of_slot;
  DevBuf<pl::Record> pal_dense;
  DevBuf<uint32_t> vword;
  DevBuf<uint32_t> vword_dir;
  bool vword_dir_fresh = false;
  bool pal_lds = false;
  pl::RowPlan rows;
  DevBuf<uint32_t> rword;
  DevBuf<pl::Record> pal_dense2;
  bool pal_rows = false;
  DevBuf<pl::Record> palette;
  bool pal_ready = false;
  int pal_entries = 0;
  pl::Coarse coarse;
  int coarse_info = 0;
  pl::Coarse coarseL;
  DevBuf<uint8_t> sharedbits, maskL;
  std::vector<uint8_t> h_cand;
  std::vector<uint8_t> h_shared;
  DevBuf<uint8_t> cend;
  DevBuf<int32_t> cnodes, cbase;
  DevBuf<int32_t> ckeep;
  int cbase_state = -1;
  DevBuf<double> kcc_inv;
  DevBuf<uint8_t> maskC, cflag;
  DevBuf<unsigned long long> cls_key, cls_keys;
  DevBuf<int> cls_owner, cls_flags;
  DevBuf<uint16_t> cls_id;
  DevBuf<double> cls_table;
  int *cls_host_flag = nullptr;
  bool cls_ready = false;
  DevBuf<unsigned long long> dcl_keys;
  DevBuf<int> dcl_owner, dcl_dense_of_slot, dcl_flags;
  DevBuf<uint16_t> dcl_slot;
  int *dcl_host_flags = nullptr;
  int dcl_fail_streak = 0, dcl_skip_left = 0;
  bool dcl_pending = false;
  DevBuf<double> p2, small_scal, small_rc;
  bool small_use = false;
  bool persist_use = false;
  DevBuf<double> ps_Ug, ps_red;
  DevBuf<unsigned> ps_flags;
  DevBuf<unsigned long long> ps_dbg;
  DevBuf<int32_t> ps_agg_ptr, ps_agg_idx;
  int ps_n_agg = 0;
  int last_iterations = 0;
  int64_t n_cond = 0;
  bool cond_ready = false;
  bool cond_use = false;
  int cond_agree = -1;
  pl::Dist dist;
  std::vector<int32_t> h_tile_start;
  DevBuf<int32_t> ov_iface, ov_inner;
  int64_t n_ov_iface = 0, n_ov_inner = 0;
  bool ov_ready = false;
  hipStream_t comm_stream = nullptr;
  hipEvent_t ev_ov_a = nullptr, ev_ov_x = nullptr;

  pl_stats_t last{};
  double ms_assembly = 0.0;
  double *pin6 = nullptr;
  size_t pin6_n = 0;
  DevBuf<int32_t> per_ptr, per_nodes;
  int64_t n_per_groups = 0;
  double *pinB = nullptr;
  DevBuf<double> sens_out;
  DevBuf<double> usol;
  bool usol_valid = false;
  DevBuf<double> gram_x, gram_out;
  double *pinG = nullptr;
  size_t pinG_n = 0;
  int gram_cols = 0;
  std::shared_ptr<void> multi_ws;
  std::shared_ptr<void> geom_ws;
  std::shared_ptr<void> mass_ws;
  std::shared_ptr<void> dyn_ws;
  std::shared_ptr<void> dyn_sens_ws;
  DevBuf<double> st_vm4, st_part, st_red, st_G, st_dr;

  ~pl_context() {
    if (ev0) (void)hipEventDestroy(ev0);
    if (ev1) (void)hipEventDestroy(ev1);
    if (ev_fork) (void)hipEventDestroy(ev_fork);
    if (ev_join) (void)hipEventDestroy(ev_join);
    if (ev_chol) (void)hipEventDestroy(ev_chol);
    if (ev_fill1) (void)hipEventDestroy(ev_fill1);
    if (ev_p0) (void)hipEventDestroy(ev_p0);
    if (ev_p1) (void)hipEventDestroy(ev_p1);
    if (ev_t0) (void)hipEventDestroy(ev_t0);
    if (ev_t1) (void)hipEventDestroy(ev_t1);
    if (pin6) (void)hipHostFree(pin6);
    if (pinB) (void)hipHostFree(pinB);
    if (pinG) (void)hipHostFree(pinG);
    if (ev_ov_a) (void)hipEventDestroy(ev_ov_a);
    if (ev_ov_x) (void)hipEventDestroy(ev_ov_x);
    if (comm_stream) (void)hipStreamDestroy(comm_stream);
    if (side2) (void)hipStreamDestroy(side2);
    if (side_cu) (void)hipStreamDestroy(side_cu);
    if (side) (void)hipStreamDestroy(side);
    if (stream) (void)hipStreamDestroy(stream);
  }
};

namespace {

int staging(pl_context *c, double **out) {
  const size_t n6 = (size_t)c->N * 6;
  if (!c->pin6 || c->pin6_n < n6) {
    if (c->pin6) (void)hipHostFree(c->pin6);
    c->pin6 = nullptr;
    void *p = nullptr;
    PL_HIP(hipHostMalloc(&p, n6 * sizeof(double), hipHostMallocDefault));
    c->pin6 = static_cast<double *>(p);
    c->pin6_n = n6;
  }
  *out = c->pin6;
  return PL_OK;
}

int stagingB(pl_context *c, double **out) {
  if (!c->pinB) {
    void *p = nullptr;
    PL_HIP(hipHostMalloc(&p, (size_t)std::max<int64_t>(c->B, 1) * sizeof(double), hipHostMallocDefault));
    c->pinB = static_cast<double *>(p);
  }
  *out = c->pinB;
  return PL_OK;
}

int upload6(pl_context *c, const double *host, double *dev, std::vector<double> &) {
  const size_t n6 = (size_t)c->N * 6;
  double *st = nullptr;
  int rc = staging(c, &st);
  if (rc) return rc;
  if (!c->reordered) {
    pl::parallel_for((int64_t)n6, [&](int64_t b, int64_t e, unsigned) { std::memcpy(st + b, host + b, (e - b) * sizeof(double)); },
                     1 << 18);
  } else {
    pl::parallel_for(c->N, [&](int64_t b, int64_t e, unsigned) {
      for (int64_t i = b; i < e; ++i) std::memcpy(st + 6 * i, host + 6 * (size_t)c->perm[i], 6 * sizeof(double));
    }, 1 << 15);
  }
  PL_HIP(hipMemcpyAsync(dev, st, n6 * sizeof(double), hipMemcpyHostToDevice, c->stream));
  PL_HIP(hipStreamSynchronize(c->stream));
  return PL_OK;
}

int download6(pl_context *c, const double *dev, double *host) {
  const size_t n6 = (size_t)c->N * 6;
  double *st = nullptr;
  int rc = staging(c, &st);
  if (rc) return rc;
  PL_HIP(hipMemcpyAsync(st, dev, n6 * sizeof(double), hipMemcpyDeviceToHost, c->stream));
  PL_HIP(hipStreamSynchronize(c->stream));
  if (!c->reordered) {
    pl::parallel_for((int64_t)n6, [&](int64_t b, int64_t e, unsigned) { std::memcpy(host + b, st + b, (e - b) * sizeof(double)); },
                     1 << 18);
  } else {
    pl::parallel_for(c->N, [&](int64_t b, int64_t e, unsigned) {
      for (int64_t i = b; i < e; ++i) std::memcpy(host + 6 * (size_t)c->perm[i], st + 6 * i, 6 * sizeof(double));
    }, 1 << 15);
  }
  return PL_OK;
}

void struts_to_caller(const pl_context *c, const double *stg, double *host, int width = 1) {
  const size_t w = (size_t)width;
  pl::parallel_for(c->B, [&](int64_t b0, int64_t b1, unsigned) {
    for (int64_t b = b0; b < b1; ++b)
      for (size_t k = 0; k < w; ++k) host[w * (size_t)c->bperm[b] + k] = stg[w * (size_t)b + k];
  }, width == 1 ? 1 << 16 : 1 << 14);
}

int download_struts(pl_context *c, const double *dev, double *host, int width = 1) {
  const size_t w = (size_t)width;
  std::vector<double> wide;
  double *stg = nullptr;
  if (width == 1) {
    if (int rc = stagingB(c, &stg)) return rc;
  } else {
    wide.resize((size_t)c->B * w);
    stg = wide.data();
  }
  PL_HIP(hipMemcpyAsync(stg, dev, (size_t)c->B * w * sizeof(double), hipMemcpyDeviceToHost, c->stream));
  PL_HIP(hipStreamSynchronize(c->stream));
  struts_to_caller(c, stg, host, width);
  return PL_OK;
}

int state_on_device(pl_context *c, const char *who, const double *u, const double **u_dev) {
  if (!u && !(c->usol.p && c->usol_valid))
    return fail(PL_ERR_STATE, std::string(who) + ": u = NULL needs a pl_solve on this handle first");
  PL_HIP(hipSetDevice(c->opt.device));
  *u_dev = c->usol.p;
  if (u) {
    std::vector<double> stage;
    if (int rc = upload6(c, u, c->tmp.p, stage)) return rc;
    *u_dev = c->tmp.p;
  }
  return PL_OK;
}

}
```

Baseline: 256.4 million.

## Compress tile strain blocks by runs of identical beam records and rework cross-coupling assembly

Adds a k_tile_runs kernel that groups consecutive interior beams of each tile with bit-identical records into runs. It computes each run's strain-block contribution once, weighted by the run's count, so k_tile_blocks_strain can skip free interior beams and add the precomputed sums. The k_coarse_cross12 kernel is rewritten to use wave-level shuffle reductions and per-block merging of identical aggregate pairs, which cuts the number of atomic adds into the coarse matrix. It also runs on its own stream (side_cu) with an extra event. The trade-offs are an extra kernel launch, scratch buffers, and a fallback path for tiles with more than 64 runs.

```diff
diff --git a/include/pylattice_hip.h b/include/pylattice_hip.h
--- a/include/pylattice_hip.h
+++ b/include/pylattice_hip.h
@@ -236,6 +236,8 @@
 int pl_time_kernel(pl_handle h, int which, int reps, double *avg_ms);
 int pl_algorithmic_bytes(pl_handle h, double *out3);
 int pl_node_words_info(pl_handle h, int *classes_on, int *n_classes, int *bytes_on, int *byte_exp);
+int pl_tile_runs_info(pl_handle h, int *tiles_by_runs, int *tiles_fallback, int *max_runs);
+int pl_debug_tile_blocks(pl_handle h, double *raw, int64_t cap);
 int pl_forget_history(pl_handle h);
 
 int pl_debug_spd_solve(int device, int32_t n, const double *A, const double *b, double *x, double *quad,
diff --git a/pylatticedso_amd/_capi.py b/pylatticedso_amd/_capi.py
--- a/pylatticedso_amd/_capi.py
+++ b/pylatticedso_amd/_capi.py
@@ -20,7 +20,7 @@
            "pl_spmv_multi", "pl_solve_multi", "pl_schur_block", "pl_geom_spmv_multi", "pl_buckling_modes", "pl_buckling_modes_sens",
            "pl_set_mass", "pl_mass_spmv_multi", "pl_vibration_modes", "pl_vibration_modes_sens",
            "pl_dyn_spmv_multi", "pl_transient", "pl_transient_sens",
-           "pl_schur_cells", "pl_cells_recover", "pl_get_records", "pl_debug_partition", "pl_time_kernel", "pl_algorithmic_bytes", "pl_node_words_info", "pl_forget_history", "pl_debug_spd_solve", "pl_dist_unique_id_bytes",
+           "pl_schur_cells", "pl_cells_recover", "pl_get_records", "pl_debug_partition", "pl_time_kernel", "pl_algorithmic_bytes", "pl_node_words_info", "pl_tile_runs_info", "pl_debug_tile_blocks", "pl_forget_history", "pl_debug_spd_solve", "pl_dist_unique_id_bytes",
            "pl_dist_unique_id", "pl_dist_loopback_id", "pl_dist_abort", "pl_dist_init", "pl_dist_set_peers", "pl_generate_lattice", "pl_lattice_fetch",
            "pl_lattice_free", "pl_penalize", "pl_boundary_index", "pl_boundary_index_rows"]
 
@@ -103,7 +103,7 @@
            "pl_schur_cells": [V, I32, I32, I32, V, I32, V, V, V, V, V, V, V],
            "pl_cells_recover": [V, I32, I32, I32, V, I32, V, V, V, V, V, V, V, V, V, V, V],
            "pl_get_records": [V, V], "pl_debug_partition": [V, V, V, V, V], "pl_time_kernel": [V, I32, I32, V],
-           "pl_algorithmic_bytes": [V, V], "pl_node_words_info": [V, V, V, V, V], "pl_forget_history": [V], "pl_debug_spd_solve": [I32, I32, V, V, V, V, I32], "pl_dist_unique_id_bytes": [], "pl_dist_unique_id": [V], "pl_dist_loopback_id": [V], "pl_dist_abort": [V],
+           "pl_algorithmic_bytes": [V, V], "pl_node_words_info": [V, V, V, V, V], "pl_tile_runs_info": [V, V, V, V], "pl_debug_tile_blocks": [V, V, I64], "pl_forget_history": [V], "pl_debug_spd_solve": [I32, I32, V, V, V, V, I32], "pl_dist_unique_id_bytes": [], "pl_dist_unique_id": [V], "pl_dist_loopback_id": [V], "pl_dist_abort": [V],
            "pl_dist_init": [V, I32, I32, V, V, V, I32, I32], "pl_dist_set_peers": [V, V],
            "pl_generate_lattice": [I64, V, V, V, I32, I32, V, V, V, V], "pl_lattice_fetch": [V] * 12,
            "pl_lattice_free": [V], "pl_penalize": [I64, V, V, V, D, V, V, V],
@@ -936,6 +936,17 @@
         _check(self._lib, self._lib.pl_node_words_info(self._h, *[C.byref(x) for x in v]))
         return {"classes": bool(v[0].value), "n_classes": v[1].value, "bytes": bool(v[2].value), "byte_exp": v[3].value}
 
+    def tile_runs_info(self):
+        v = [C.c_int() for _ in range(3)]
+        _check(self._lib, self._lib.pl_tile_runs_info(self._h, *[C.byref(x) for x in v]))
+        return {"by_runs": v[0].value, "fallback": v[1].value, "max_runs": v[2].value}
+
+    def debug_tile_blocks(self):
+        n_tiles = int(self.partition()["tile"].max()) + 1
+        buf = np.zeros(n_tiles * 147)
+        _check(self._lib, self._lib.pl_debug_tile_blocks(self._h, _ptr(buf), buf.size))
+        return buf[:n_tiles * 144].reshape(n_tiles, 12, 12).copy(), buf[n_tiles * 144:].reshape(n_tiles, 3).copy()
+
     def algorithmic_bytes(self):
         out = (C.c_double * 3)()
         _check(self._lib, self._lib.pl_algorithmic_bytes(self._h, out))
diff --git a/pylatticedso_amd/csrc/pl_api.hip b/pylatticedso_amd/csrc/pl_api.hip
--- a/pylatticedso_amd/csrc/pl_api.hip
+++ b/pylatticedso_amd/csrc/pl_api.hip
@@ -200,6 +200,7 @@
   PL_HIPC(hipEventCreateWithFlags(&c->ev_chol, hipEventDisableTiming));
   PL_HIPC(hipEventCreateWithFlags(&c->ev_t0, hipEventDisableTiming));
   PL_HIPC(hipEventCreateWithFlags(&c->ev_t1, hipEventDisableTiming));
+  PL_HIPC(hipEventCreateWithFlags(&c->ev_t2, hipEventDisableTiming));
   PL_HIPC(hipEventCreateWithFlags(&c->ev_p0, hipEventDisableTiming));
   PL_HIPC(hipEventCreateWithFlags(&c->ev_p1, hipEventDisableTiming));
   PL_HIPC(hipEventCreateWithFlags(&c->ev_fill1, hipEventDisableTiming));
@@ -570,6 +571,7 @@
   PL_HIPC(hipEventCreateWithFlags(&c->ev_chol, hipEventDisableTiming));
   PL_HIPC(hipEventCreateWithFlags(&c->ev_t0, hipEventDisableTiming));
   PL_HIPC(hipEventCreateWithFlags(&c->ev_t1, hipEventDisableTiming));
+  PL_HIPC(hipEventCreateWithFlags(&c->ev_t2, hipEventDisableTiming));
   PL_HIPC(hipStreamCreateWithFlags(&c->side2, hipStreamNonBlocking));
   c->perm.resize(n_nodes);
   std::iota(c->perm.begin(), c->perm.end(), 0);
@@ -3018,6 +3020,48 @@
   return PL_OK;
 }
 
+int pl_tile_runs_info(pl_handle h, int *tiles_by_runs, int *tiles_fallback, int *max_runs) {
+  if (!valid(h)) return fail(PL_ERR_ARG, "pl_tile_runs_info: null handle");
+  int by_runs = 0, fallback = 0, longest = 0;
+  const pl::Coarse &cs = h->coarse;
+  if (h->assembled && cs.runs_valid && cs.tile_runs && cs.n_tiles > 0) {
+    PL_HIP(hipSetDevice(h->opt.device));
+    std::vector<int32_t> runs((size_t)cs.n_tiles);
+    PL_HIP(hipDeviceSynchronize());
+    PL_HIP(hipMemcpy(runs.data(), cs.tile_runs, runs.size() * sizeof(int32_t), hipMemcpyDeviceToHost));
+    for (int32_t r : runs) {
+      if (r < 0) ++fallback;
+      else ++by_runs;
+      longest = std::max(longest, (int)r);
+    }
+  }
+  if (tiles_by_runs) *tiles_by_runs = by_runs;
+  if (tiles_fallback) *tiles_fallback = fallback;
+  if (max_runs) *max_runs = longest;
+  return PL_OK;
+}
+
+int pl_debug_tile_blocks(pl_handle h, double *raw, int64_t cap) {
+  if (!valid(h) || !raw) return fail(PL_ERR_ARG, "pl_debug_tile_blocks: null argument");
+  const pl::Coarse &cs = h->coarse;
+  if (h->opkind != 0 || !h->assembled || !h->have_bc || !cs.enabled || !cs.tile_level || tile_modes_now(h) != 12 || !cs.Bt_raw)
+    return fail(PL_ERR_STATE, "pl_debug_tile_blocks: no assembled 12-mode tile level on this handle");
+  const int64_t T = cs.n_tiles;
+  if (cap < T * 144) return fail(PL_ERR_ARG, "pl_debug_tile_blocks: cap is below n_tiles * 144");
+  PL_HIP(hipSetDevice(h->opt.device));
+  PL_HIP(hipDeviceSynchronize());
+  PL_HIP(hipMemcpy(raw, cs.Bt_raw, (size_t)T * 144 * sizeof(double), hipMemcpyDeviceToHost));
+  if (cap >= T * 147) {
+    std::vector<int32_t> agg((size_t)T);
+    std::vector<double> cen((size_t)cs.n_agg * 3);
+    PL_HIP(hipMemcpy(agg.data(), cs.agg_of_tile.p, agg.size() * sizeof(int32_t), hipMemcpyDeviceToHost));
+    PL_HIP(hipMemcpy(cen.data(), cs.cen.p, cen.size() * sizeof(double), hipMemcpyDeviceToHost));
+    for (int64_t t = 0; t < T; ++t)
+      for (int k = 0; k < 3; ++k) raw[T * 144 + 3 * t + k] = cen[3 * (size_t)agg[(size_t)t] + k];
+  }
+  return PL_OK;
+}
+
 int pl_debug_spd_solve(int device, int32_t n, const double *A, const double *b, double *x, double *quad,
                        int32_t fp32_factor) {
   return fp32_factor ? debug_spd_solve_t<float>(device, n, A, b, x, quad)
diff --git a/pylatticedso_amd/csrc/pl_assembly.h b/pylatticedso_amd/csrc/pl_assembly.h
--- a/pylatticedso_amd/csrc/pl_assembly.h
+++ b/pylatticedso_amd/csrc/pl_assembly.h
@@ -234,6 +234,28 @@
   return (c->coarse.tile_level && c->coarse.tile_modes == 12 && !c->coarseL.enabled) ? 12 : 6;
 }
 
+struct TileRunArgs {
+  const pl::TileDesc *tdesc = nullptr;
+  const double *ss_int = nullptr;
+  const int32_t *tile_runs = nullptr;
+};
+int launch_tile_runs(pl_context *c, pl::Coarse &cs, const uint8_t *mask, hipStream_t st, TileRunArgs &a) {
+  a = TileRunArgs{};
+  cs.runs_valid = false;
+  if (!cs.runs_on || !c->tile.vis_ready || cs.n_tiles <= 0 || cs.n_tiles != c->tile.n_tiles) return PL_OK;
+  if (!cs.ss_int && hipMalloc((void **)&cs.ss_int, (size_t)cs.n_tiles * 21 * sizeof(double)) != hipSuccess)
+    return fail(PL_ERR_HIP, "pl_assemble: out of device memory for the tile runs");
+  if (!cs.tile_runs && hipMalloc((void **)&cs.tile_runs, (size_t)cs.n_tiles * sizeof(int32_t)) != hipSuccess)
+    return fail(PL_ERR_HIP, "pl_assemble: out of device memory for the tile runs");
+  hipLaunchKernelGGL(pl::k_tile_runs, dim3((unsigned)cs.n_tiles), dim3(pl::kBlock), 0, st, c->tile.tdesc.p,
+                     reinterpret_cast<const int2 *>(c->conn.p), c->rec.p, mask, cs.ss_int, cs.tile_runs);
+  a.tdesc = c->tile.tdesc.p;
+  a.ss_int = cs.ss_int;
+  a.tile_runs = cs.tile_runs;
+  cs.runs_valid = true;
+  return PL_OK;
+}
+
 int launch_tile_blocks(pl_context *c, hipStream_t st) {
   pl::Coarse &cs = c->coarse;
   if (!cs.enabled || !c->have_bc || !cs.tile_level) return PL_OK;
@@ -250,10 +272,12 @@
                        c->tile.tile_start.p, c->tile.home_ptr.p, c->tile.foreign_ptr.p, c->tile.foreign_idx.p,
                        reinterpret_cast<const int2 *>(c->conn.p), c->rec.p, cs.agg_of_tile.p, cs.cen.p, c->xyz.p, fb,
                        cs.Bt_raw);
+    TileRunArgs ra;
+    if (int rc = launch_tile_runs(c, cs, fb, st, ra)) return rc;
     hipLaunchKernelGGL(pl::k_tile_blocks_strain<false>, dim3((unsigned)cs.n_tiles), dim3(pl::kBlock), 0, st,
                        c->tile.tile_start.p, c->tile.home_ptr.p, c->tile.foreign_ptr.p, c->tile.foreign_idx.p,
                        reinterpret_cast<const int2 *>(c->conn.p), c->rec.p, cs.agg_of_tile.p, cs.cen.p, c->xyz.p, fb,
-                       cs.Bt_raw);
+                       cs.Bt_raw, ra.tdesc, ra.ss_int, ra.tile_runs);
     hipLaunchKernelGGL(pl::k_tile_invert12, dim3((unsigned)cs.n_tiles), dim3(pl::kInv12Block), 0, st, cs.n_tiles,
                        (const double *)cs.Bt_raw, cs.Bt_inv);
   }
@@ -283,23 +307,36 @@
       hipLaunchKernelGGL(pl::k_tile_blocks_strain<true>, gt, blk, 0, c->stream, c->tile.tile_start.p, c->tile.home_ptr.p,
                          c->tile.foreign_ptr.p, c->tile.foreign_idx.p, conn2, c->rec.p, cs.agg_of_tile.p, cs.cen.p,
                          c->xyz.p, (const uint8_t *)c->maskL.p, cs.Bt_raw);
+      TileRunArgs raL;
+      if (int rc = launch_tile_runs(c, cs, c->maskL.p, c->stream, raL)) return rc;
       hipLaunchKernelGGL(pl::k_tile_blocks_strain<false>, gt, blk, 0, c->stream, c->tile.tile_start.p, c->tile.home_ptr.p,
                          c->tile.foreign_ptr.p, c->tile.foreign_idx.p, conn2, c->rec.p, cs.agg_of_tile.p, cs.cen.p,
-                         c->xyz.p, (const uint8_t *)c->maskL.p, cs.Bt_raw);
+                         c->xyz.p, (const uint8_t *)c->maskL.p, cs.Bt_raw, raL.tdesc, raL.ss_int, raL.tile_runs);
     }
     double *rawA = two_sets ? cs.Bt_rawA : cs.Bt_raw;
+    hipStream_t cross_st = c->side_cu ? c->side_cu : c->side2;
     PL_HIP(hipEventRecord(c->ev_t0, c->stream));
     PL_HIP(hipStreamWaitEvent(c->side2, c->ev_t0, 0));
+    if (cs.n_cross > 0 && cross_st != c->side2) PL_HIP(hipStreamWaitEvent(cross_st, c->ev_t0, 0));
+    TileRunArgs ra;
+    if (int rc = launch_tile_runs(c, cs, mask, c->stream, ra)) return rc;
+    hipLaunchKernelGGL(pl::k_tile_blocks_strain<false>, gt, blk, 0, c->stream, c->tile.tile_start.p, c->tile.home_ptr.p,
+                       c->tile.foreign_ptr.p, c->tile.foreign_idx.p, conn2, c->rec.p, cs.agg_of_tile.p, cs.cen.p, c->xyz.p,
+                       mask, rawA, ra.tdesc, ra.ss_int, ra.tile_runs);
     hipLaunchKernelGGL(pl::k_tile_blocks_strain<true>, gt, blk, 0, c->side2, c->tile.tile_start.p, c->tile.home_ptr.p,
                        c->tile.foreign_ptr.p, c->tile.foreign_idx.p, conn2, c->rec.p, cs.agg_of_tile.p, cs.cen.p, c->xyz.p,
                        mask, rawA);
-    if (cs.n_cross > 0)
-      hipLaunchKernelGGL(pl::k_coarse_cross12, dim3(grid_for(cs.n_cross)), blk, 0, c->side2, cs.n_cross,
+    PL_HIP(hipEventRecord(c->ev_t1, c->side2));
+    if (cs.n_cross > 0) {
+      hipLaunchKernelGGL(pl::k_coarse_cross12, dim3(grid_for(cs.n_cross)), blk, 0, cross_st, cs.n_cross,
                          cs.cross_idx.p, c->conn.p, c->rec.p, cs.agg_of_node.p, cs.cen.p, c->xyz.p, mask, n, cs.Ac);
-    PL_HIP(hipEventRecord(c->ev_t1, c->side2));
-    hipLaunchKernelGGL(pl::k_tile_blocks_strain<false>, gt, blk, 0, c->stream, c->tile.tile_start.p, c->tile.home_ptr.p,
-                       c->tile.foreign_ptr.p, c->tile.foreign_idx.p, conn2, c->rec.p, cs.agg_of_tile.p, cs.cen.p, c->xyz.p,
-                       mask, rawA);
+      if (cross_st != c->side2) {
+        PL_HIP(hipEventRecord(c->ev_t2, cross_st));
+        PL_HIP(hipStreamWaitEvent(c->stream, c->ev_t2, 0));
+      } else {
+        PL_HIP(hipEventRecord(c->ev_t1, c->side2));
+      }
+    }
     PL_HIP(hipStreamWaitEvent(c->stream, c->ev_t1, 0));
     hipLaunchKernelGGL(pl::k_agg_add_tiles, dim3(grid_for(cs.n_tiles * 144)), blk, 0, c->stream, cs.n_tiles,
                        cs.agg_of_tile.p, (const double *)rawA, n, cs.Ac);
diff --git a/pylatticedso_amd/csrc/pl_coarse.h b/pylatticedso_amd/csrc/pl_coarse.h
--- a/pylatticedso_amd/csrc/pl_coarse.h
+++ b/pylatticedso_amd/csrc/pl_coarse.h
@@ -17,6 +17,10 @@
 constexpr int kDclSlots = 4096;
 inline bool node_words_enabled() {
   const char *e = std::getenv("PL_NODE_WORDS");
+  return !(e && e[0] == '0');
+}
+inline bool tile_runs_enabled() {
+  const char *e = std::getenv("PL_TILE_RUNS");
   return !(e && e[0] == '0');
 }
 
@@ -47,6 +51,9 @@
   int tile_modes = 6;
   double *Bt_raw = nullptr;
   double *Bt_rawA = nullptr;
+  double *ss_int = nullptr;
+  int32_t *tile_runs = nullptr;
+  bool runs_on = true, runs_valid = false;
   float *dinv32 = nullptr;
   TBuf<float> rel32;
   bool rel_exact = false;
@@ -61,7 +68,7 @@
   ~Coarse() {
     for (void *q : {(void *)Ac, (void *)Lf, (void *)W, (void *)Wt, (void *)Dinv, (void *)rc, (void *)yc, (void *)tv,
                     (void *)info, (void *)Bt_inv, (void *)yt, (void *)fix_count, (void *)dinv32, (void *)bar,
-                    (void *)Bt_raw, (void *)Bt_rawA, (void *)Ainv, (void *)dcl_table})
+                    (void *)Bt_raw, (void *)Bt_rawA, (void *)Ainv, (void *)dcl_table, (void *)ss_int, (void *)tile_runs})
       if (q) (void)hipFree(q);
   }
 };
@@ -152,6 +159,7 @@
       if (hipMalloc((void **)&c.dcl_table, (size_t)kDclMax * 8 * sizeof(uint32_t)) != hipSuccess) return 2;
     }
   }
+  c.runs_on = tile_runs_enabled();
   c.n_agg = n_agg;
   c.nc = modes * n_agg;
   c.n_tiles = T;
@@ -431,6 +439,23 @@
     default: u = {-r[1], r[0], 0.0}; th = {0.0, 0.0, 1.0}; break;
   }
 }
+__device__ __forceinline__ int wave_fold12_index(int lane) { return (lane >> 2) & 15; }
+__device__ __forceinline__ double wave_fold12(const double *x , int lane) {
+  const bool b5 = lane & 32, b4 = lane & 16, b3 = lane & 8, b2 = lane & 4;
+  double y8[8], y4[4], y2[2];
+#pragma unroll
+  for (int i = 0; i < 8; ++i) {
+    const double up = i < 4 ? x[8 + i] : 0.0;
+    y8[i] = (b5 ? up : x[i]) + __shfl_xor(b5 ? x[i] : up, 32);
+  }
+#pragma unroll
+  for (int i = 0; i < 4; ++i) y4[i] = (b4 ? y8[4 + i] : y8[i]) + __shfl_xor(b4 ? y8[i] : y8[4 + i], 16);
+#pragma unroll
+  for (int i = 0; i < 2; ++i) y2[i] = (b3 ? y4[2 + i] : y4[i]) + __shfl_xor(b3 ? y4[i] : y4[2 + i], 8);
+  double v = (b2 ? y2[1] : y2[0]) + __shfl_xor(b2 ? y2[0] : y2[1], 4);
+  v += __shfl_xor(v, 1);
+  return v + __shfl_xor(v, 2);
+}
 __global__ __launch_bounds__(kBlock) void k_coarse_cross12(int64_t n_cross, const int32_t *__restrict__ list,
                                                            const int32_t *__restrict__ conn,
                                                            const Record *__restrict__ rec,
@@ -439,43 +464,65 @@
                                                            const double *__restrict__ xyz,
                                                            const uint8_t *__restrict__ fixedbits, int nc,
                                                            double *__restrict__ Ac) {
+  __shared__ double part[kBlock / kWave][144];
+  __shared__ int pairI[kBlock / kWave], pairJ[kBlock / kWave];
   const int64_t q = (int64_t)blockIdx.x * kBlock + threadIdx.x;
-  if ((q & ~(int64_t)(kWave - 1)) >= n_cross) return;
-  const bool live = list[q] >= 0;
-  const int64_t b = live ? list[q] : list[q & ~(int64_t)(kWave - 1)];
-  const int ia = conn[2 * b], ib = conn[2 * b + 1];
-  const int I = agg[ia], J = agg[ib];
-  const unsigned fa = fixedbits ? fixedbits[ia] : 0u, fb = fixedbits ? fixedbits[ib] : 0u;
-  const Record r = load_record(rec, b);
-  double rela[3], relb[3];
-#pragma unroll
-  for (int k = 0; k < 3; ++k) {
-    rela[k] = xyz[3 * (int64_t)ia + k] - cen[3 * I + k];
-    relb[k] = xyz[3 * (int64_t)ib + k] - cen[3 * J + k];
-  }
-  const V3 d = {r.dx, r.dy, r.dz}, zero = {0.0, 0.0, 0.0};
-  const int lane = threadIdx.x & 63;
-  for (int n = 0; n < 12; ++n) {
-    V3 uB, tB;
-    mode_disp(n, relb, uB, tB);
-    uB = mask3(uB, fb);
-    tB = mask3(tB, fb >> 3);
-    V3 F, M;
-    tip_force(r, zero, zero, uB, tB, F, M);
-    const V3 FA = mask3((-1.0) * F, fa), MA = mask3((-1.0) * M - cross(d, F), fa >> 3);
-    double x[12] = {FA.x, FA.y, FA.z,
-                    MA.x + (rela[1] * FA.z - rela[2] * FA.y), MA.y + (rela[2] * FA.x - rela[0] * FA.z),
-                    MA.z + (rela[0] * FA.y - rela[1] * FA.x), 0, 0, 0, 0, 0, 0};
-    strain_restrict(FA, rela, x + 6, 1.0);
-#pragma unroll
-    for (int m = 0; m < 12; ++m) {
-      const double v = wave_sum(live ? x[m] : 0.0);
-      if (lane == 0 && v != 0.0) {
-        const size_t ri = (size_t)12 * I + m, cj = (size_t)12 * J + n;
-        if (ri > cj) unsafeAtomicAdd(Ac + ri * nc + cj, v);
-        else if (cj > ri) unsafeAtomicAdd(Ac + cj * nc + ri, v);
-        else unsafeAtomicAdd(Ac + ri * nc + cj, 2.0 * v);
+  const int lane = threadIdx.x & 63, wv = threadIdx.x >> 6;
+  const bool wave_on = (q & ~(int64_t)(kWave - 1)) < n_cross;
+  if (lane == 0) pairI[wv] = -1;
+  if (wave_on) {
+    const bool live = list[q] >= 0;
+    const int64_t b = live ? list[q] : list[q & ~(int64_t)(kWave - 1)];
+    const int ia = conn[2 * b], ib = conn[2 * b + 1];
+    const int I = agg[ia], J = agg[ib];
+    const unsigned fa = fixedbits ? fixedbits[ia] : 0u, fb = fixedbits ? fixedbits[ib] : 0u;
+    const Record r = load_record(rec, b);
+    double rela[3], relb[3];
+#pragma unroll
+    for (int k = 0; k < 3; ++k) {
+      rela[k] = xyz[3 * (int64_t)ia + k] - cen[3 * I + k];
+      relb[k] = xyz[3 * (int64_t)ib + k] - cen[3 * J + k];
+    }
+    const V3 d = {r.dx, r.dy, r.dz}, zero = {0.0, 0.0, 0.0};
+    if (lane == 0) {
+      pairI[wv] = I;
+      pairJ[wv] = J;
+    }
+    const int held = wave_fold12_index(lane);
+    for (int n = 0; n < 12; ++n) {
+      V3 uB, tB;
+      mode_disp(n, relb, uB, tB);
+      uB = mask3(uB, fb);
+      tB = mask3(tB, fb >> 3);
+      V3 F, M;
+      tip_force(r, zero, zero, uB, tB, F, M);
+      const V3 FA = mask3((-1.0) * F, fa), MA = mask3((-1.0) * M - cross(d, F), fa >> 3);
+      double x[12] = {FA.x, FA.y, FA.z,
+                      MA.x + (rela[1] * FA.z - rela[2] * FA.y), MA.y + (rela[2] * FA.x - rela[0] * FA.z),
+                      MA.z + (rela[0] * FA.y - rela[1] * FA.x), 0, 0, 0, 0, 0, 0};
+      strain_restrict(FA, rela, x + 6, 1.0);
+      if (!live) {
+#pragma unroll
+        for (int m = 0; m < 12; ++m) x[m] = 0.0;
       }
+      const double v = wave_fold12(x, lane);
+      if ((lane & 3) == 0 && held < 12) part[wv][held * 12 + n] = v;
+    }
+  }
+  __syncthreads();
+  const int e = threadIdx.x;
+  if (e >= 144) return;
+  const int m = e / 12, n = e - 12 * m;
+  for (int w = 0; w < kBlock / kWave; ++w) {
+    const int I = pairI[w], J = pairJ[w];
+    if (I < 0 || (w > 0 && pairI[w - 1] == I && pairJ[w - 1] == J)) continue;
+    double v = part[w][e];
+    for (int w2 = w + 1; w2 < kBlock / kWave && pairI[w2] == I && pairJ[w2] == J; ++w2) v += part[w2][e];
+    if (v != 0.0) {
+      const size_t ri = (size_t)12 * I + m, cj = (size_t)12 * J + n;
+      if (ri > cj) unsafeAtomicAdd(Ac + ri * nc + cj, v);
+      else if (cj > ri) unsafeAtomicAdd(Ac + cj * nc + ri, v);
+      else unsafeAtomicAdd(Ac + ri * nc + cj, 2.0 * v);
     }
   }
 }
@@ -648,6 +695,109 @@
   }
 }
 
+constexpr int kTileRunsMax = 64;
+__device__ __forceinline__ bool same_record_bits(const Record *__restrict__ rec, int64_t i, int64_t j) {
+  const ulonglong2 *p = reinterpret_cast<const ulonglong2 *>(rec + i), *q = reinterpret_cast<const ulonglong2 *>(rec + j);
+  bool same = true;
+#pragma unroll
+  for (int k = 0; k < 4; ++k) {
+    const ulonglong2 a = p[k], b = q[k];
+    same = same && a.x == b.x && a.y == b.y;
+  }
+  return same;
+}
+__global__ __launch_bounds__(kBlock) void k_tile_runs(const TileDesc *__restrict__ tdesc, const int2 *__restrict__ conn2,
+                                                      const Record *__restrict__ rec,
+                                                      const uint8_t *__restrict__ fixedbits,
+                                                      double *__restrict__ ss_int, int32_t *__restrict__ tile_runs) {
+  __shared__ int head[kTileRunsMax], sorted[kTileRunsMax];
+  __shared__ unsigned cnt[kTileRunsMax];
+  __shared__ double part[kTileRunsMax][21];
+  __shared__ int n_heads;
+  const int t = blockIdx.x;
+  const TileDesc td = tdesc[t];
+  const int n_int = td.n_int;
+  if (threadIdx.x == 0) n_heads = 0;
+  if (threadIdx.x < kTileRunsMax) cnt[threadIdx.x] = 0u;
+  unsigned fx = 0u;
+  if (fixedbits)
+    for (int i = td.n0 + (int)threadIdx.x; i < td.n1; i += kBlock) fx |= fixedbits[i];
+  const bool any_fixed = __syncthreads_or((int)fx) != 0;
+  for (int k = threadIdx.x; k < n_int; k += kBlock) {
+    if (*(volatile int *)&n_heads > kTileRunsMax) break;
+    if (k == 0 || !same_record_bits(rec, td.h0 + k, td.h0 + k - 1)) {
+      const int slot = atomicAdd(&n_heads, 1);
+      if (slot < kTileRunsMax) head[slot] = k;
+    }
+  }
+  __syncthreads();
+  const int n = n_heads;
+  if (n > kTileRunsMax) {
+    if (threadIdx.x < 21) ss_int[(size_t)t * 21 + threadIdx.x] = 0.0;
+    if (threadIdx.x == 0) tile_runs[t] = -1;
+    return;
+  }
+  if ((int)threadIdx.x < n) {
+    const int mine = head[threadIdx.x];
+    int rank = 0;
+    for (int j = 0; j < n; ++j) rank += head[j] < mine;
+    sorted[rank] = mine;
+  }
+  __syncthreads();
+  if (!any_fixed) {
+    if ((int)threadIdx.x < n) cnt[threadIdx.x] = (unsigned)((threadIdx.x + 1 < (unsigned)n ? sorted[threadIdx.x + 1] : n_int) - sorted[threadIdx.x]);
+  } else {
+    const int lane = threadIdx.x & (kWave - 1);
+    for (int k0 = 0; k0 < n_int; k0 += kBlock) {
+      const int k = k0 + (int)threadIdx.x;
+      bool counted = false;
+      int run = 0;
+      if (k < n_int) {
+        const int2 cn = conn2[td.h0 + k];
+        counted = (fixedbits[cn.x] | fixedbits[cn.y]) == 0u;
+        int lo = 0, hi = n - 1;
+        while (lo < hi) {
+          const int mid = (lo + hi + 1) >> 1;
+          if (sorted[mid] <= k) lo = mid;
+          else hi = mid - 1;
+        }
+        run = lo;
+      }
+      unsigned long long todo = __ballot(counted);
+      while (todo) {
+        const int leader = __ffsll((long long)todo) - 1;
+        const int r = __shfl(run, leader);
+        const unsigned long long m = __ballot(counted && run == r);
+        if (lane == leader) atomicAdd(&cnt[r], (unsigned)__popcll(m));
+        todo &= ~m;
+      }
+    }
+  }
+  __syncthreads();
+  for (int item = threadIdx.x; item < 6 * n; item += kBlock) {
+    const int i = item / 6, q = item - 6 * i;
+    const Record r = load_record(rec, td.h0 + sorted[i]);
+    const double d[3] = {r.dx, r.dy, r.dz}, none[3] = {0.0, 0.0, 0.0};
+    const V3 zero = {0.0, 0.0, 0.0};
+    V3 F, M;
+    tip_force(r, strain_disp(q, none), zero, strain_disp(q, d), zero, F, M);
+    double s6[6] = {0, 0, 0, 0, 0, 0};
+    strain_restrict(F, d, s6, 1.0);
+    strain_restrict((-1.0) * F, none, s6, 1.0);
+    const double w = (double)cnt[i];
+#pragma unroll
+    for (int p = 0; p < 6; ++p)
+      if (p <= q) part[i][q * (q + 1) / 2 + p] = w * s6[p];
+  }
+  __syncthreads();
+  if (threadIdx.x < 21) {
+    double v = 0.0;
+    for (int i = 0; i < n; ++i) v += part[i][threadIdx.x];
+    ss_int[(size_t)t * 21 + threadIdx.x] = v;
+  }
+  if (threadIdx.x == 0) tile_runs[t] = n;
+}
+
 template <bool RIGID>
 __global__ __launch_bounds__(kBlock) void k_tile_blocks_strain(const int32_t *__restrict__ tile_start,
                                                                const int64_t *__restrict__ home_ptr,
@@ -659,7 +809,10 @@
                                                                const double *__restrict__ cen,
                                                                const double *__restrict__ xyz,
                                                                const uint8_t *__restrict__ fixedbits,
-                                                               double *__restrict__ raw) {
+                                                               double *__restrict__ raw,
+                                                               const TileDesc *__restrict__ tdesc = nullptr,
+                                                               const double *__restrict__ ss_int = nullptr,
+                                                               const int32_t *__restrict__ tile_runs = nullptr) {
   __shared__ double red[57][kBlock / kWave];
   const int t = blockIdx.x;
   const int n0 = tile_start[t], n1 = tile_start[t + 1];
@@ -675,14 +828,22 @@
   for (int e = 0; e < (RIGID ? 1 : 36); ++e) RS[e] = 0.0;
   const int64_t h0 = home_ptr[t], h1 = home_ptr[t + 1], f0 = foreign_ptr[t], f1 = foreign_ptr[t + 1];
   const int64_t total = (h1 - h0) + (f1 - f0);
-  for (int64_t v = threadIdx.x; v < total; v += kBlock) {
+  const bool by_runs = !RIGID && tile_runs && tile_runs[t] >= 0;
+  int64_t first = 0;
+  if (by_runs) {
+    unsigned fx = 0u;
+    if (fixedbits)
+      for (int i = n0 + (int)threadIdx.x; i < n1; i += kBlock) fx |= fixedbits[i];
+    if (!__syncthreads_or((int)fx)) first = tdesc[t].n_int;
+  }
+  for (int64_t v = first + threadIdx.x; v < total; v += kBlock) {
     const int64_t b = v < (h1 - h0) ? h0 + v : (int64_t)foreign_idx[f0 + (v - (h1 - h0))];
     const int2 cn = conn2[b];
     const bool ina = cn.x >= n0 && cn.x < n1, inb = cn.y >= n0 && cn.y < n1;
     if (!ina && !inb) continue;
     const unsigned fa = fixedbits ? fixedbits[cn.x] : 0u, fb = fixedbits ? fixedbits[cn.y] : 0u;
     const bool free_inside = ina && inb && fa == 0u && fb == 0u;
-    if (RIGID && free_inside) continue;
+    if ((RIGID || by_runs) && free_inside) continue;
     const Record r = load_record(rec, b);
     const double rela[3] = {xyz[3 * (int64_t)cn.x] - c0, xyz[3 * (int64_t)cn.x + 1] - c1, xyz[3 * (int64_t)cn.x + 2] - c2};
     const double relb[3] = {xyz[3 * (int64_t)cn.y] - c0, xyz[3 * (int64_t)cn.y + 1] - c1, xyz[3 * (int64_t)cn.y + 2] - c2};
@@ -795,6 +956,7 @@
 #pragma unroll
     for (int q = 0; q < kBlock / kWave; ++q) v += red[threadIdx.x][q];
     if (threadIdx.x < 21) {
+      if (by_runs) v += ss_int[(size_t)t * 21 + threadIdx.x];
       int q = 0;
       while ((q + 1) * (q + 2) / 2 <= (int)threadIdx.x) ++q;
       const int p = (int)threadIdx.x - q * (q + 1) / 2;
diff --git a/pylatticedso_amd/csrc/pl_context.h b/pylatticedso_amd/csrc/pl_context.h
--- a/pylatticedso_amd/csrc/pl_context.h
+++ b/pylatticedso_amd/csrc/pl_context.h
@@ -80,6 +80,7 @@
   hipEvent_t ev_p0 = nullptr, ev_p1 = nullptr;
   hipEvent_t ev_fill1 = nullptr;
   hipStream_t side2 = nullptr;
+  hipEvent_t ev_t2 = nullptr;
   hipStream_t side_cu = nullptr;
   bool assembled = false, have_bc = false, have_bsr = false;
   int pal_fallback_flags[2] = {1, 0};
@@ -253,6 +254,7 @@
     if (ev_p1) (void)hipEventDestroy(ev_p1);
     if (ev_t0) (void)hipEventDestroy(ev_t0);
     if (ev_t1) (void)hipEventDestroy(ev_t1);
+    if (ev_t2) (void)hipEventDestroy(ev_t2);
     if (pin6) (void)hipHostFree(pin6);
     if (pinB) (void)hipHostFree(pinB);
     if (pinG) (void)hipHostFree(pinG);
```

New measurement: 257.2 million, median of 6. No clear change (+0.3%).
